# alshai/Big-BWT

Hardware: NVIDIA B200
Metric: pfp_parse_throughput (higher is better)
Workload: dtype u8/u32/u64 integer

## Files before the change

big-bwt_b200/csrc/pfp_api.cu:

```cuda
#include "pfp_common.cuh"
#include "pfp_stages.cuh"
#include <errno.h>
#include <fcntl.h>
#include <stdlib.h>
#include <sys/stat.h>
#include <time.h>
#include <unistd.h>

extern "C" {
int pfp_io_read_file(const char *path, int gz_ok, uint8_t **buf, uint64_t *n, char *err, size_t errlen);
int pfp_io_write_outputs(const char *path, const pfpb200_opts *opts, const pfpb200_outputs *o,
                         char *err, size_t errlen);
}

static double wall_sec() {
    struct timespec ts;
    clock_gettime(CLOCK_MONOTONIC, &ts);
    return (double)ts.tv_sec + 1e-9 * (double)ts.tv_nsec;
}

__global__ void set_u64_k(u64 *p, u64 v) { *p = v; }

__global__ void __launch_bounds__(256) first_invalid_k(const u8 *__restrict__ t, u64 n,
                                                       unsigned long long *__restrict__ first) {
    const u64 stride = (u64)gridDim.x * blockDim.x * 16;
    for (u64 i = ((u64)blockIdx.x * blockDim.x + threadIdx.x) * 16; i < n; i += stride) {
        bool hit = false;
        if (i + 16 <= n && (((uintptr_t)(t + i)) & 15) == 0) {
            uint4 v = __ldg(reinterpret_cast<const uint4 *>(t + i));
            u32 w[4] = {v.x, v.y, v.z, v.w};
#pragma unroll
            for (int k = 0; k < 4; k++) hit |= ((w[k] - 0x03030303u) & ~w[k] & 0x80808080u) != 0;
        } else hit = true;
        if (hit) {
            u64 e = i + 16 < n ? i + 16 : n;
            for (u64 j = i; j < e; j++)
                if (t[j] <= PFP_DOLLAR) { atomicMin(first, (unsigned long long)j); break; }
        }
    }
}

int pfp_first_invalid(pfpb200_ctx *ctx, const u8 *d_text, u64 n, u64 *d_first) {
    if (n == 0) return PFPB200_OK;
    first_invalid_k<<<ctx->sm_count * 8, 256, 0, ctx->stream>>>(d_text, n,
                                                               reinterpret_cast<unsigned long long *>(d_first));
    PFP_LAUNCHED(ctx);
    return PFPB200_OK;
}

extern "C" int pfpb200_abi_version(void) { return PFPB200_ABI_VERSION; }

extern "C" const char *pfpb200_strerror(int code) {
    switch (code) {
        case PFPB200_OK: return "ok";
        case PFPB200_E_ARG: return "invalid argument";
        case PFPB200_E_IO: return "file I/O error";
        case PFPB200_E_CUDA: return "CUDA error (no usable GPU or kernel failure)";
        case PFPB200_E_NOMEM: return "out of memory";
        case PFPB200_E_LIMIT: return "algorithm limit exceeded";
        case PFPB200_E_COLLISION: return "fingerprint collision";
        case PFPB200_E_INTERNAL: return "internal error";
        default: return "unknown error";
    }
}

extern "C" uint32_t pfpb200_launch_count(const pfpb200_ctx *ctx) { return ctx ? ctx->launches : 0; }

extern "C" const char *pfpb200_last_error(const pfpb200_ctx *ctx) { return ctx ? ctx->err : ""; }

static u64 splitmix64(u64 &s) {
    u64 z = (s += 0x9E3779B97F4A7C15ULL);
    z = (z ^ (z >> 30)) * 0xBF58476D1CE4E5B9ULL;
    z = (z ^ (z >> 27)) * 0x94D049BB133111EBULL;
    return z ^ (z >> 31);
}

extern "C" int pfpb200_create(int device, pfpb200_ctx **out) {
    if (!out) return PFPB200_E_ARG;
    *out = nullptr;
    int ndev = 0;
    if (cudaGetDeviceCount(&ndev) != cudaSuccess || device < 0 || device >= ndev) {
        cudaGetLastError();
        return PFPB200_E_CUDA;
    }
    pfpb200_ctx *ctx = new (std::nothrow) pfpb200_ctx();
    if (!ctx) return PFPB200_E_NOMEM;
    ctx->device = device;
    { const char *ev = getenv("PFPB200_LEGACY_K2"); ctx->legacy_k2 = ev && atoi(ev) != 0; }
    { const char *ev = getenv("PFPB200_K1"); ctx->k1_mode = (ev && strcmp(ev, "rolling") == 0) ? 1 : (ev && strcmp(ev, "table") == 0) ? 2 : 0; }
    { const char *ev = getenv("PFPB200_TEST_WEAK_FP"); ctx->weak_fp = (ev && atoi(ev) != 0) ? 1u : 0u; }
    { const char *ev = getenv("PFPB200_NO_SCAN_ALPHA"); ctx->no_scan_alpha = ev && atoi(ev) != 0; }
    { const char *ev = getenv("PFPB200_RANK_FULL_SORT"); ctx->rank_full_sort = ev && atoi(ev) != 0; }
    { const char *ev = getenv("PFPB200_RANK_CHUNK_PASSES"); ctx->rank_chunk_passes = ev && atoi(ev) != 0; }
    { const char *ev = getenv("PFPB200_RANK_WARP_PASSES"); ctx->rank_warp_passes = ev && atoi(ev) != 0; }
    { const char *ev = getenv("PFPB200_POOL_BY_WORD"); ctx->pool_by_word = ev && atoi(ev) != 0; }
    { const char *ev = getenv("PFPB200_FUSE_K3"); ctx->fuse_k3 = ev && atoi(ev) != 0; }
    { const char *ev = getenv("PFPB200_TABLE_SCALE"); if (ev && atof(ev) >= 1.2) ctx->table_scale = atof(ev); }
    { const char *ev = getenv("PFPB200_K1_MIX"); ctx->k1_mix = ev ? atoi(ev) : 0; }
    { const char *ev = getenv("PFPB200_K2_WINDOW"); ctx->k2_window = ev ? atoi(ev) : 0; }
    auto bail = [&](int code) { pfpb200_destroy(ctx); return code; };
    if (cudaSetDevice(device) != cudaSuccess) return bail(PFPB200_E_CUDA);
    cudaDeviceProp prop;
    if (cudaGetDeviceProperties(&prop, device) != cudaSuccess) return bail(PFPB200_E_CUDA);
    ctx->sm_count = prop.multiProcessorCount;
    if (cudaStreamCreateWithFlags(&ctx->own_stream, cudaStreamNonBlocking) != cudaSuccess)
        return bail(PFPB200_E_CUDA);
    ctx->stream = ctx->own_stream;
    if (cudaMalloc(&ctx->d_flags, PFP_FLAG_SLOTS * sizeof(u64)) != cudaSuccess ||
        cudaMallocHost(&ctx->h_flags, PFP_FLAG_SLOTS * sizeof(u64)) != cudaSuccess ||
        cudaMalloc(&ctx->d_keys, NH_KEY_WORDS * sizeof(u32)) != cudaSuccess ||
        cudaMalloc(&ctx->d_alpha, 8 * sizeof(u32)) != cudaSuccess)
        return bail(PFPB200_E_NOMEM);
    u32 hk[NH_KEY_WORDS];
    u64 seed = 0x5bd1e9955bd1e995ULL;
    for (u32 i = 0; i < NH_KEY_WORDS; i++) hk[i] = (u32)(splitmix64(seed) >> 32);
    if (cudaMemcpy(ctx->d_keys, hk, sizeof(hk), cudaMemcpyHostToDevice) != cudaSuccess ||
        cudaMemset(ctx->d_flags, 0, PFP_FLAG_SLOTS * sizeof(u64)) != cudaSuccess)
        return bail(PFPB200_E_CUDA);
    set_u64_k<<<1, 1, 0, ctx->stream>>>(&ctx->d_flags[15], 1);
    if (cudaGetLastError() != cudaSuccess || cudaStreamSynchronize(ctx->stream) != cudaSuccess)
        return bail(PFPB200_E_CUDA);
    if (cudaStreamCreateWithFlags(&ctx->aux_stream, cudaStreamNonBlocking) != cudaSuccess ||
        cudaEventCreateWithFlags(&ctx->ev_aux0, cudaEventDisableTiming) != cudaSuccess ||
        cudaEventCreateWithFlags(&ctx->ev_aux1, cudaEventDisableTiming) != cudaSuccess)
        return bail(PFPB200_E_CUDA);
    if (pfp_scan_init(ctx) || pfp_stream_init(ctx) || pfp_phrase_init(ctx) || pfp_prims_init(ctx) ||
        pfp_rank_init(ctx))
        return bail(PFPB200_E_CUDA);
    *out = ctx;
    return PFPB200_OK;
}

extern "C" void pfpb200_destroy(pfpb200_ctx *ctx) {
    if (!ctx) return;
    cudaSetDevice(ctx->device);
    if (ctx->stream) cudaStreamSynchronize(ctx->stream);
    pfp_release_scratch(ctx);
    pfp_release_held(ctx);
    pfp_arena_destroy(ctx);
    if (ctx->own_stream) { cudaStreamSynchronize(ctx->own_stream); cudaStreamDestroy(ctx->own_stream); }
    if (ctx->d_flags) cudaFree(ctx->d_flags);
    if (ctx->h_flags) cudaFreeHost(ctx->h_flags);
    if (ctx->d_keys) cudaFree(ctx->d_keys);
    if (ctx->dna_table) cudaFree(ctx->dna_table);
    if (ctx->iv_etab) cudaFree(ctx->iv_etab);
    if (ctx->iv_xtab) cudaFree(ctx->iv_xtab);
    if (ctx->d_alpha) cudaFree(ctx->d_alpha);
    pfp_io_destroy(ctx);
    for (int i = 0; i < 5; i++)
        if (ctx->pin_buf[i]) cudaFreeHost(ctx->pin_buf[i]);
    if (ctx->copy_stream) { cudaStreamSynchronize(ctx->copy_stream); cudaStreamDestroy(ctx->copy_stream); }
    if (ctx->aux_stream) { cudaStreamSynchronize(ctx->aux_stream); cudaStreamDestroy(ctx->aux_stream); }
    if (ctx->ev_aux0) cudaEventDestroy(ctx->ev_aux0);
    if (ctx->ev_aux1) cudaEventDestroy(ctx->ev_aux1);
    if (ctx->ev_k2) cudaEventDestroy(ctx->ev_k2);
    if (ctx->ev_copy) cudaEventDestroy(ctx->ev_copy);
    delete ctx;
}

extern "C" int pfpb200_set_stream(pfpb200_ctx *ctx, void *cuda_stream) {
    if (!ctx) return PFPB200_E_ARG;
    cudaStreamSynchronize(ctx->stream);
    pfp_release_scratch(ctx);
    pfp_release_held(ctx);
    ctx->stream = cuda_stream ? (cudaStream_t)cuda_stream : ctx->own_stream;
    return PFPB200_OK;
}

static int check_opts(pfpb200_ctx *ctx, const pfpb200_opts *o) {
    if (!ctx) return PFPB200_E_ARG;
    if (!o) return pfp_fail(ctx, PFPB200_E_ARG, "null options");
    if (o->w < 4) return pfp_fail(ctx, PFPB200_E_ARG, "Windows size must be at least 4");
    if (o->p < 10) return pfp_fail(ctx, PFPB200_E_ARG, "Modulus must be at least 10");
    if (o->w > 65536) return pfp_fail(ctx, PFPB200_E_ARG, "window size too large");
    if (o->nseg < 0) return pfp_fail(ctx, PFPB200_E_ARG, "Number of threads cannot be negative");
    return PFPB200_OK;
}

static int begin_call(pfpb200_ctx *ctx) {
    PFP_CUDA(ctx, cudaSetDevice(ctx->device));
    pfp_release_scratch(ctx);
    pfp_release_held(ctx);
    PFP_TRY(pfp_arena_consolidate(ctx));
    ctx->launches = 0;
    ctx->err[0] = 0;
    PFP_CUDA(ctx, cudaMemsetAsync(ctx->d_flags, 0, PFP_FLAG_SLOTS * sizeof(u64), ctx->stream));
    return PFPB200_OK;
}

struct StageTimer {
    cudaEvent_t ev[10] = {nullptr};
    int n = 0;
    int init() {
        for (int i = 0; i < 10; i++)
            if (cudaEventCreate(&ev[i]) != cudaSuccess) { ev[i] = nullptr; return -1; }
        return 0;
    }
    void mark(cudaStream_t s) { cudaEventRecord(ev[n++], s); }
    float ms(int a, int b) { float t = 0; cudaEventElapsedTime(&t, ev[a], ev[b]); return t; }
    ~StageTimer() {
        for (int i = 0; i < 10; i++)
            if (ev[i]) cudaEventDestroy(ev[i]);
    }
};

static int pfp_pin(pfpb200_ctx *ctx, int slot, void **h, size_t bytes) {
    if (bytes > ctx->pin_cap[slot]) {
        if (ctx->pin_buf[slot]) cudaFreeHost(ctx->pin_buf[slot]);
        ctx->pin_buf[slot] = nullptr;
        ctx->pin_cap[slot] = 0;
        size_t cap = bytes + bytes / 8 + 4096;
        if (cudaMallocHost(&ctx->pin_buf[slot], cap) != cudaSuccess) {
            cudaGetLastError();
            return pfp_fail(ctx, PFPB200_E_NOMEM, "pinned host allocation of %zu bytes failed", cap);
        }
        ctx->pin_cap[slot] = cap;
    }
    *h = ctx->pin_buf[slot];
    return PFPB200_OK;
}

static int parse_device_impl(pfpb200_ctx *ctx, const u8 *d_text, u64 n, const pfpb200_opts *o,
                             pfpb200_outputs *out, pfpb200_stats *st) {
    const u32 w = o->w, p = o->p;
    StageTimer tm;
    if (tm.init()) return pfp_fail(ctx, PFPB200_E_CUDA, "cudaEventCreate failed");
    int rc = PFPB200_OK;
    auto run = [&]() -> int {
        tm.mark(ctx->stream);
        ScanBits sb;
        float ms_scan = 0, ms_emit = 0;
        PFP_TRY(pfp_scan_bits(ctx, d_text, n, 0, 0, n, w, p, false, &sb, &ms_scan));
        const u64 k = sb.total;
        const u64 P = k + 1;
        if (P >= 0xFFFFFFFFull)
            return pfp_fail(ctx, PFPB200_E_LIMIT, "the parse contains %llu words, more than 2^32-2",
                            (unsigned long long)P);
        u64 *ends = nullptr;
        PFP_TRY(pfp_alloc_t(ctx, &ends, P));
        set_u64_k<<<1, 1, 0, ctx->stream>>>(ends + k, n + w - 1);
        PFP_LAUNCHED(ctx);
        tm.mark(ctx->stream);
        PhraseArrays ph{};
        ph.ends = ends;
        PFP_TRY(pfp_alloc_t(ctx, &ph.last, P, true));
        if (o->flags & PFPB200_F_SAI) PFP_TRY(pfp_alloc_t(ctx, &ph.sai, P * PFP_IBYTES, true));
        TextView tv{d_text, n, 0, (i64)n};
        DictArrays D;
        const bool stream = pfp_stream_ok(sb, w) && !ctx->legacy_k2;
        const bool fused = stream && ctx->fuse_k3;
        if (fused) {
            PFP_TRY(pfp_words_fused_stage(ctx, sb, tv, ph, P, -1, w, true, &D));
        } else {
            PFP_TRY(pfp_alloc_t(ctx, &ph.rec, P));
            if (stream) PFP_TRY(pfp_stream_stage(ctx, sb, tv, ph, P, -1, w, true));
            else {
                PFP_TRY(pfp_scan_emit(ctx, sb, ends));
                PFP_TRY(pfp_hash_stage(ctx, tv, ph, P, -1, w));
            }
        }
        PFP_TRY(pfp_scan_bits_free(ctx, &sb));
        tm.mark(ctx->stream);
        if (ctx->early_copy) {
            void *h_last = nullptr, *h_sai = nullptr;
            PFP_TRY(pfp_pin(ctx, 3, &h_last, P));
            if (ph.sai) PFP_TRY(pfp_pin(ctx, 4, &h_sai, P * PFP_IBYTES));
            if (!ctx->copy_stream) {
                PFP_CUDA(ctx, cudaStreamCreateWithFlags(&ctx->copy_stream, cudaStreamNonBlocking));
                PFP_CUDA(ctx, cudaEventCreateWithFlags(&ctx->ev_k2, cudaEventDisableTiming));
                PFP_CUDA(ctx, cudaEventCreateWithFlags(&ctx->ev_copy, cudaEventDisableTiming));
            }
            PFP_CUDA(ctx, cudaEventRecord(ctx->ev_k2, ctx->stream));
            PFP_CUDA(ctx, cudaStreamWaitEvent(ctx->copy_stream, ctx->ev_k2, 0));
            PFP_CUDA(ctx, cudaMemcpyAsync(h_last, ph.last, P, cudaMemcpyDeviceToHost, ctx->copy_stream));
            if (ph.sai)
                PFP_CUDA(ctx, cudaMemcpyAsync(h_sai, ph.sai, P * PFP_IBYTES, cudaMemcpyDeviceToHost, ctx->copy_stream));
            PFP_CUDA(ctx, cudaEventRecord(ctx->ev_copy, ctx->copy_stream));
            ctx->early_done = true;
        }
        if (!fused) {
            PFP_TRY(pfp_dedup_stage(ctx, ph, P, -1, w, &D));
            PFP_TRY(pfp_free_now(ctx, ph.rec));
            PFP_TRY(pfp_pool_stage(ctx, tv, ends, -1, w, &D));
        }
        if (o->flags & PFPB200_F_VERIFY) {
            PFP_TRY(pfp_uid_words(ctx, &D, P));
            PFP_TRY(pfp_verify_stage(ctx, tv, ends, -1, w, P, D));
        }
        tm.mark(ctx->stream);
        u32 *order = nullptr, rounds = 0;
        PFP_TRY(pfp_rank_stage(ctx, D, &order, &rounds, ctx->alpha_valid && !ctx->no_scan_alpha));
        tm.mark(ctx->stream);
        u8 *dict = nullptr;
        u32 *occ = nullptr, *rank_of_uid = nullptr;
        u64 dict_bytes = 0;
        u32 *parse = nullptr;
        PFP_TRY(pfp_alloc_t(ctx, &parse, P, true));
        PFP_TRY(pfp_dict_stage(ctx, D, order, (o->flags & PFPB200_F_COMPRESS) ? w : 0, &dict,
                               &dict_bytes, &occ, &rank_of_uid, D.uid, P, parse));
        tm.mark(ctx->stream);
        tm.mark(ctx->stream);
        PFP_CUDA(ctx, cudaMemcpyAsync(ctx->h_flags, ctx->d_flags, sizeof(u64), cudaMemcpyDeviceToHost, ctx->stream));
        PFP_CUDA(ctx, cudaStreamSynchronize(ctx->stream));
        PFP_CUDA(ctx, cudaGetLastError());
        if (ctx->h_flags[0] & PFP_ERRBIT_COLLISION)
            return pfp_fail(ctx, PFPB200_E_COLLISION, "two different phrases share a fingerprint (found by the verify pass)");
        out->dict = dict; out->dict_bytes = dict_bytes;
        out->occ = occ; out->n_distinct = D.d;
        out->parse = parse; out->n_phrases = P;
        out->last = ph.last;
        out->sai = ph.sai;
        if (st) {
            st->n_text = n; st->n_phrases = P; st->n_distinct = D.d;
            st->sum_word_len = D.sum_len; st->dict_bytes = dict_bytes;
            st->alg_bytes = n + 4 * P + P + ((o->flags & PFPB200_F_SAI) ? 5 * P : 0) + dict_bytes + 4 * D.d;
            st->rank_rounds = rounds;
            st->launches = ctx->launches;
            st->ms_total = tm.ms(0, 6);
            st->ms_scan = ms_scan; st->ms_emit = ms_emit;
            st->ms_hash = tm.ms(1, 2); st->ms_dedup = tm.ms(2, 3); st->ms_rank = tm.ms(3, 4);
            st->ms_dict = tm.ms(4, 5); st->ms_remap = tm.ms(5, 6);
        }
        return PFPB200_OK;
    };
    rc = run();
    if (rc != PFPB200_OK) cudaStreamSynchronize(ctx->stream);
    pfp_release_scratch(ctx);
    return rc;
}

extern "C" int pfpb200_parse_device(pfpb200_ctx *ctx, const uint8_t *d_text, uint64_t n_text,
                                    const pfpb200_opts *opts, pfpb200_outputs *dev_out,
                                    pfpb200_stats *stats) {
    PFP_TRY(check_opts(ctx, opts));
    if (!dev_out || (n_text && !d_text)) return pfp_fail(ctx, PFPB200_E_ARG, "null buffer");
    if (stats) memset(stats, 0, sizeof(*stats));
    memset(dev_out, 0, sizeof(*dev_out));
    PFP_TRY(begin_call(ctx));
    return parse_device_impl(ctx, d_text, n_text, opts, dev_out, stats);
}

extern "C" int pfpb200_memcpy_d2h(pfpb200_ctx *ctx, void *dst_host, const void *src_device,
                                  uint64_t bytes) {
    if (!ctx || (bytes && (!dst_host || !src_device))) return PFPB200_E_ARG;
    if (bytes == 0) return PFPB200_OK;
    PFP_CUDA(ctx, cudaSetDevice(ctx->device));
    PFP_CUDA(ctx, cudaMemcpyAsync(dst_host, src_device, bytes, cudaMemcpyDeviceToHost, ctx->stream));
    PFP_CUDA(ctx, cudaStreamSynchronize(ctx->stream));
    return PFPB200_OK;
}

extern "C" int pfpb200_parse_host(pfpb200_ctx *ctx, const uint8_t *text, uint64_t n_text,
                                  const pfpb200_opts *opts, pfpb200_outputs *host_out,
                                  pfpb200_stats *stats) {
    PFP_TRY(check_opts(ctx, opts));
    if (!host_out || (n_text && !text)) return pfp_fail(ctx, PFPB200_E_ARG, "null buffer");
    if (stats) memset(stats, 0, sizeof(*stats));
    memset(host_out, 0, sizeof(*host_out));
    PFP_TRY(begin_call(ctx));
    PfpEvents evs(4);
    if (!evs.ok) return pfp_fail(ctx, PFPB200_E_CUDA, "cudaEventCreate failed");
    const cudaEvent_t e0 = evs[0], e1 = evs[1], e2 = evs[2], e3 = evs[3];
    u8 *d_text = nullptr;
    PFP_TRY(pfp_alloc(ctx, (void **)&d_text, n_text, true));
    cudaEventRecord(e0, ctx->stream);
    if (n_text) PFP_CUDA(ctx, cudaMemcpyAsync(d_text, text, n_text, cudaMemcpyHostToDevice, ctx->stream));
    u64 n = n_text;
    if (n_text) {
        set_u64_k<<<1, 1, 0, ctx->stream>>>(&ctx->d_flags[14], n_text);
        PFP_LAUNCHED(ctx);
        first_invalid_k<<<ctx->sm_count * 8, 256, 0, ctx->stream>>>(
            d_text, n_text, reinterpret_cast<unsigned long long *>(&ctx->d_flags[14]));
        PFP_LAUNCHED(ctx);
        PFP_CUDA(ctx, cudaMemcpyAsync(&ctx->h_flags[14], &ctx->d_flags[14], sizeof(u64),
                                      cudaMemcpyDeviceToHost, ctx->stream));
    }
    cudaEventRecord(e1, ctx->stream);
    if (n_text) {
        PFP_CUDA(ctx, cudaStreamSynchronize(ctx->stream));
        n = ctx->h_flags[14];
    }
    if (n < n_text && (opts->flags & PFPB200_F_VERBOSE))
        fprintf(stderr, "Invalid char found in input file: no additional chars will be read\n");
    pfpb200_outputs dv;
    memset(&dv, 0, sizeof(dv));
    ctx->early_copy = true;
    ctx->early_done = false;
    int rc = parse_device_impl(ctx, d_text, n, opts, &dv, stats);
    ctx->early_copy = false;
    if (rc != PFPB200_OK) {
        if (ctx->early_done) cudaEventSynchronize(ctx->ev_copy);
        return rc;
    }
    const u64 P = dv.n_phrases, d = dv.n_distinct;
    void *h_dict = nullptr, *h_occ = nullptr, *h_parse = nullptr, *h_last = nullptr, *h_sai = nullptr;
    PFP_TRY(pfp_pin(ctx, 0, &h_dict, dv.dict_bytes));
    PFP_TRY(pfp_pin(ctx, 1, &h_occ, d * 4));
    PFP_TRY(pfp_pin(ctx, 2, &h_parse, P * 4));
    PFP_TRY(pfp_pin(ctx, 3, &h_last, P));
    if (dv.sai) PFP_TRY(pfp_pin(ctx, 4, &h_sai, P * PFP_IBYTES));
    cudaEventRecord(e2, ctx->stream);
    PFP_CUDA(ctx, cudaMemcpyAsync(h_dict, dv.dict, dv.dict_bytes, cudaMemcpyDeviceToHost, ctx->stream));
    PFP_CUDA(ctx, cudaMemcpyAsync(h_occ, dv.occ, d * 4, cudaMemcpyDeviceToHost, ctx->stream));
    PFP_CUDA(ctx, cudaMemcpyAsync(h_parse, dv.parse, P * 4, cudaMemcpyDeviceToHost, ctx->stream));
    if (ctx->early_done) {
        PFP_CUDA(ctx, cudaStreamWaitEvent(ctx->stream, ctx->ev_copy, 0));
    } else {
        PFP_CUDA(ctx, cudaMemcpyAsync(h_last, dv.last, P, cudaMemcpyDeviceToHost, ctx->stream));
        if (dv.sai)
            PFP_CUDA(ctx, cudaMemcpyAsync(h_sai, dv.sai, P * PFP_IBYTES, cudaMemcpyDeviceToHost, ctx->stream));
    }
    cudaEventRecord(e3, ctx->stream);
    PFP_CUDA(ctx, cudaStreamSynchronize(ctx->stream));
    if (stats) {
        cudaEventElapsedTime(&stats->ms_h2d, e0, e1);
        cudaEventElapsedTime(&stats->ms_d2h, e2, e3);
    }
    host_out->dict = (const u8 *)h_dict; host_out->dict_bytes = dv.dict_bytes;
    host_out->occ = (const u32 *)h_occ; host_out->n_distinct = d;
    host_out->parse = (const u32 *)h_parse; host_out->n_phrases = P;
    host_out->last = (const u8 *)h_last;
    host_out->sai = (const u8 *)h_sai;
    pfp_release_held(ctx);
    return PFPB200_OK;
}

static int write_outputs_from_device(pfpb200_ctx *ctx, const char *path, const pfpb200_opts *o,
                                     const pfpb200_outputs &dv) {
    char name[4096];
    auto put = [&](const char *ext, int seg, const void *p, u64 bytes) -> int {
        if (seg < 0) snprintf(name, sizeof(name), "%s.%s", path, ext);
        else snprintf(name, sizeof(name), "%s.%d.%s", path, seg, ext);
        return pfp_device_to_file(ctx, name, p, bytes);
    };
    const u64 P = dv.n_phrases;
    PFP_TRY(put((o->flags & PFPB200_F_COMPRESS) ? "dicz" : "dict", -1, dv.dict, dv.dict_bytes));
    PFP_TRY(put("occ", -1, dv.occ, 4 * dv.n_distinct));
    PFP_TRY(put("parse", -1, dv.parse, 4 * P));
    const int T = o->nseg;
    if (T <= 0) {
        PFP_TRY(put("last", -1, dv.last, P));
        if (dv.sai) PFP_TRY(put("sai", -1, dv.sai, PFP_IBYTES * P));
    } else {
        const u64 per = (P + (u64)T - 1) / (u64)T;
        for (int s = 0; s < T; s++) {
            u64 a = (u64)s * per, b = a + per;
            if (a > P) a = P;
            if (b > P) b = P;
            PFP_TRY(put("last", s, dv.last + a, b - a));
            if (dv.sai) PFP_TRY(put("sai", s, dv.sai + PFP_IBYTES * a, PFP_IBYTES * (b - a)));
        }
    }
    return PFPB200_OK;
}

static int cut_and_parse_device(pfpb200_ctx *ctx, const u8 *d_text, u64 n_text, const pfpb200_opts *opts,
                                pfpb200_outputs *dv, pfpb200_stats *stats) {
    u64 n = n_text;
    if (n_text) {
        set_u64_k<<<1, 1, 0, ctx->stream>>>(&ctx->d_flags[14], n_text);
        PFP_LAUNCHED(ctx);
        PFP_TRY(pfp_first_invalid(ctx, d_text, n_text, &ctx->d_flags[14]));
        PFP_CUDA(ctx, cudaMemcpyAsync(&ctx->h_flags[14], &ctx->d_flags[14], sizeof(u64), cudaMemcpyDeviceToHost,
                                      ctx->stream));
        PFP_CUDA(ctx, cudaStreamSynchronize(ctx->stream));
        n = ctx->h_flags[14];
    }
    if (n < n_text) fprintf(stderr, "Invalid char found in input file: no additional chars will be read\n");
    return parse_device_impl(ctx, d_text, n, opts, dv, stats);
}

static int parse_file_impl(pfpb200_ctx *ctx, const char *path, const pfpb200_opts *opts, pfpb200_stats *stats,
                           bool write_files, pfpb200_outputs *dv_out);

extern "C" int pfpb200_parse_file(pfpb200_ctx *ctx, const char *path, const pfpb200_opts *opts,
                                  pfpb200_stats *stats) {
    const int rc = parse_file_impl(ctx, path, opts, stats, true, nullptr);
    if (ctx && rc == PFPB200_OK) pfp_release_held(ctx);
    return rc;
}

extern "C" int pfpb200_bigbwt_file(pfpb200_ctx *ctx, const char *path, const pfpb200_opts *opts, uint32_t pfbwt_flags,
                                   int keep_files, pfpb200_stats *stats, pfpb200_bwtparse_result *bp_out,
                                   pfpb200_pfbwt_result *res) {
    if (!ctx || !opts || !res) return PFPB200_E_ARG;
    if (opts->flags & PFPB200_F_COMPRESS) return pfp_fail(ctx, PFPB200_E_ARG, "bigbwt: -c stops after the parse, use pfpb200_parse_file");
    pfpb200_opts o = *opts;
    o.flags |= PFPB200_F_SAI;
    o.nseg = 0;
    pfpb200_stats st;
    pfpb200_outputs dv;
    PFP_TRY(parse_file_impl(ctx, path, &o, &st, keep_files != 0, &dv));
    if (stats) *stats = st;
    const double t0 = wall_sec();
    pfpb200_bwtparse_result bp;
    PFP_TRY(pfpb200_bwtparse_device(ctx, dv.parse, dv.n_phrases, dv.last, dv.sai, &bp));
    if (bp_out) *bp_out = bp;
    PFP_TRY(pfpb200_pfbwt_device(ctx, dv.dict, dv.dict_bytes, dv.occ, dv.n_distinct, bp.ilist, bp.bwlast, bp.bwsai,
                                 bp.n_out, o.w, pfbwt_flags, res));
    char name[4096];
    auto put = [&](const char *ext, const void *p, u64 bytes) -> int {
        snprintf(name, sizeof(name), "%s.%s", path, ext);
        return pfp_device_to_file(ctx, name, p, bytes);
    };
    if (keep_files) {
        PFP_TRY(put("ilist", bp.ilist, bp.n_out * 4));
        PFP_TRY(put("bwlast", bp.bwlast, bp.n_out));
        PFP_TRY(put("bwsai", bp.bwsai, bp.n_out * PFP_IBYTES));
    }
    PFP_TRY(put("bwt", res->bwt, res->n_bwt));
    if (pfbwt_flags & PFPB200_PFBWT_SA) PFP_TRY(put("sa", res->sa, res->n_sa * PFP_IBYTES));
    if (pfbwt_flags & PFPB200_PFBWT_SSA) PFP_TRY(put("ssa", res->ssa, res->n_ssa * 2 * PFP_IBYTES));
    if (pfbwt_flags & PFPB200_PFBWT_ESA) PFP_TRY(put("esa", res->esa, res->n_esa * 2 * PFP_IBYTES));
    if (stats) stats->sec_write += (float)(wall_sec() - t0);
    pfp_release_scratch(ctx);
    return PFPB200_OK;
}

static int parse_file_impl(pfpb200_ctx *ctx, const char *path, const pfpb200_opts *opts, pfpb200_stats *stats,
                           bool write_files, pfpb200_outputs *dv_out) {
    PFP_TRY(check_opts(ctx, opts));
    if (!path) return pfp_fail(ctx, PFPB200_E_ARG, "null path");
    if (stats) memset(stats, 0, sizeof(*stats));
    const double t0 = wall_sec();
    const bool fasta = (opts->flags & PFPB200_F_FASTA) != 0;
    int fd = open(path, O_RDONLY);
    if (fd < 0) return pfp_fail(ctx, PFPB200_E_IO, "%s: %s", path, strerror(errno));
    struct stat sb;
    if (fstat(fd, &sb) != 0) { close(fd); return pfp_fail(ctx, PFPB200_E_IO, "%s: %s", path, strerror(errno)); }
    const u64 fsize = (u64)sb.st_size;
    bool gz = false;
    if (fasta && fsize >= 2) {
        unsigned char mg[2] = {0, 0};
        if (pread(fd, mg, 2, 0) == 2) gz = mg[0] == 0x1f && mg[1] == 0x8b;
    }
    PFP_TRY(begin_call(ctx));
    pfpb200_outputs dv;
    memset(&dv, 0, sizeof(dv));
    double t1 = t0;
    int rc = PFPB200_OK;
    auto run = [&]() -> int {
        u8 *d_text = nullptr;
        u64 n_text = 0;
        bool on_device = false;
        if (!gz) {
            u8 *d_file = nullptr;
            PFP_TRY(pfp_alloc(ctx, (void **)&d_file, fsize + 16));
            PFP_TRY(pfp_file_to_device(ctx, fd, 0, fsize, d_file));
            if (!fasta) { d_text = d_file; n_text = fsize; on_device = true; }
            else {
                int supported = 0;
                PFP_TRY(pfp_fasta_device(ctx, d_file, fsize, &d_text, &n_text, &supported, false));
                on_device = supported != 0;
                PFP_CUDA(ctx, cudaStreamSynchronize(ctx->stream));
                PFP_TRY(pfp_free_now(ctx, d_file));
            }
        }
        if (!on_device) {
            uint8_t *text = nullptr;
            uint64_t n = 0;
            int trunc = 0;
            if (pfpb200_read_input(path, opts->flags, &text, &n, &trunc) != PFPB200_OK)
                return pfp_fail(ctx, PFPB200_E_IO, "%s: cannot read", path);
            if (trunc) fprintf(stderr, "Invalid char found in input file: no additional chars will be read\n");
            int r2 = pfp_alloc(ctx, (void **)&d_text, n + 16);
            if (r2 == PFPB200_OK && n && cudaMemcpyAsync(d_text, text, n, cudaMemcpyHostToDevice, ctx->stream) != cudaSuccess)
                r2 = pfp_fail(ctx, PFPB200_E_CUDA, "host-to-device copy of the input failed");
            if (r2 == PFPB200_OK && cudaStreamSynchronize(ctx->stream) != cudaSuccess)
                r2 = pfp_fail(ctx, PFPB200_E_CUDA, "host-to-device copy of the input failed");
            pfpb200_free_host(text);
            PFP_TRY(r2);
            n_text = n;
        }
        PFP_CUDA(ctx, cudaStreamSynchronize(ctx->stream));
        t1 = wall_sec();
        PFP_TRY(cut_and_parse_device(ctx, d_text, n_text, opts, &dv, stats));
        return PFPB200_OK;
    };
    rc = run();
    close(fd);
    if (rc != PFPB200_OK) { pfp_release_scratch(ctx); return rc; }
    const double t2 = wall_sec();
    if (write_files) PFP_TRY(write_outputs_from_device(ctx, path, opts, dv));
    if (stats) {
        stats->sec_read = (float)(t1 - t0);
        stats->sec_write = (float)(wall_sec() - t2);
    }
    pfp_release_scratch(ctx);
    if (dv_out) *dv_out = dv;
    return PFPB200_OK;
}

extern "C" int pfpb200_fasta_extract_device(pfpb200_ctx *ctx, const uint8_t *d_file, uint64_t n,
                                            const uint8_t **d_text, uint64_t *n_text, int *supported) {
    if (!ctx || !d_text || !n_text || !supported || (n && !d_file)) return PFPB200_E_ARG;
    PFP_TRY(begin_call(ctx));
    u8 *out = nullptr;
    int rc = pfp_fasta_device(ctx, d_file, n, &out, n_text, supported, true);
    cudaStreamSynchronize(ctx->stream);
    pfp_release_scratch(ctx);
    *d_text = out;
    return rc;
}

extern "C" int pfpb200_scan_triggers(pfpb200_ctx *ctx, const uint8_t *d_buf, uint64_t n_buf,
                                     uint64_t buf_pos0, uint64_t own_lo, uint64_t own_hi, uint32_t w,
                                     uint32_t p, const uint64_t **d_triggers, uint64_t *n_triggers,
                                     float *ms) {
    pfpb200_opts o = {w, p, 0, 0};
    PFP_TRY(check_opts(ctx, &o));
    if (!d_triggers || !n_triggers) return pfp_fail(ctx, PFPB200_E_ARG, "null output");
    PFP_TRY(begin_call(ctx));
    u64 *out = nullptr, k = 0;
    float a = 0, b = 0;
    int rc = pfp_scan_stage(ctx, d_buf, n_buf, buf_pos0, own_lo, own_hi, w, p, 0, true, &out, &k, &a, &b);
    cudaStreamSynchronize(ctx->stream);
    pfp_release_scratch(ctx);
    if (rc != PFPB200_OK) return rc;
    *d_triggers = out;
    *n_triggers = k;
    if (ms) *ms = a;
    return PFPB200_OK;
}

struct CallTimer {
    PfpEvents ev;
    cudaStream_t s;
    explicit CallTimer(cudaStream_t st) : ev(2), s(st) { if (ev.ok) cudaEventRecord(ev[0], s); }
    float stop() {
        float t = 0;
        if (!ev.ok) { cudaStreamSynchronize(s); return t; }
        cudaEventRecord(ev[1], s);
        cudaEventSynchronize(ev[1]);
        cudaEventElapsedTime(&t, ev[0], ev[1]);
        return t;
    }
};

static void promote_scratch(pfpb200_ctx *ctx) {
    for (void *p : ctx->scratch) ctx->held.push_back(p);
    ctx->scratch.clear();
}

extern "C" int pfpb200_shard_scan(pfpb200_ctx *ctx, const pfpb200_shard *shard, const pfpb200_opts *opts,
                                  uint64_t *n_triggers, uint64_t *first_trigger, uint64_t *last_trigger,
                                  float *ms) {
    PFP_TRY(check_opts(ctx, opts));
    if (!shard || !n_triggers || !first_trigger || !last_trigger) return pfp_fail(ctx, PFPB200_E_ARG, "null argument");
    if (shard->own_lo > shard->own_hi || shard->own_hi > shard->n_global)
        return pfp_fail(ctx, PFPB200_E_ARG, "bad shard range");
    PFP_TRY(begin_call(ctx));
    ctx->sh.desc = *shard;
    ctx->sh.opts = *opts;
    ctx->sh.route_perm = nullptr;
    ctx->sh.route_ooff = nullptr;
    CallTimer tm(ctx->stream);
    u64 *ends = nullptr, k = 0;
    float a = 0;
    ScanBits sb;
    int rc = pfp_scan_bits(ctx, shard->d_buf, shard->n_buf, shard->buf_pos0, shard->own_lo, shard->own_hi,
                           opts->w, opts->p, true, &sb, &a);
    if (rc == PFPB200_OK) {
        k = sb.total;
        rc = pfp_alloc_t(ctx, &ends, k + 1, true);
    }
    const bool stream_k2 = rc == PFPB200_OK && pfp_stream_ok(sb, opts->w) && !ctx->legacy_k2;
    ctx->sh.ends_emitted = !stream_k2;
    if (rc == PFPB200_OK && !stream_k2) rc = pfp_scan_emit(ctx, sb, ends);
    ctx->sh.bits = sb;
    if (rc == PFPB200_OK && k > 0) {
        if (stream_k2) {
            rc = pfp_scan_first_last(ctx, sb, &ctx->d_flags[8]);
            cudaMemcpyAsync(&ctx->h_flags[8], &ctx->d_flags[8], 2 * sizeof(u64), cudaMemcpyDeviceToHost, ctx->stream);
        } else {
            cudaMemcpyAsync(&ctx->h_flags[8], ends, sizeof(u64), cudaMemcpyDeviceToHost, ctx->stream);
            cudaMemcpyAsync(&ctx->h_flags[9], ends + (k - 1), sizeof(u64), cudaMemcpyDeviceToHost, ctx->stream);
        }
    }
    float t = tm.stop();
    pfp_release_scratch(ctx);
    if (rc != PFPB200_OK) return rc;
    PFP_CUDA(ctx, cudaGetLastError());
    ctx->sh.ends = ends;
    ctx->sh.n_trig = k;
    *n_triggers = k;
    *first_trigger = k ? ctx->h_flags[8] : 0;
    *last_trigger = k ? ctx->h_flags[9] : 0;
    if (ms) *ms = t;
    return PFPB200_OK;
}

extern "C" int pfpb200_shard_words(pfpb200_ctx *ctx, int64_t first_start, pfpb200_words *out, float *ms) {
    if (!ctx || !out) return PFPB200_E_ARG;
    memset(out, 0, sizeof(*out));
    PFP_CUDA(ctx, cudaSetDevice(ctx->device));
    const pfpb200_shard &sh = ctx->sh.desc;
    const pfpb200_opts &o = ctx->sh.opts;
    const u32 w = o.w;
    const u64 k = ctx->sh.n_trig;
    const u64 P = k + (sh.is_last ? 1 : 0);
    ctx->sh.P = P;
    ctx->sh.d = 0;
    ctx->sh.uid = nullptr;
    if (ms) *ms = 0;
    if (P == 0) return PFPB200_OK;
    if (P >= 0xFFFFFFFFull) return pfp_fail(ctx, PFPB200_E_LIMIT, "the shard's parse has more than 2^32-2 words");
    CallTimer tm(ctx->stream);
    auto run = [&]() -> int {
        u64 *ends = ctx->sh.ends;
        if (sh.is_last) {
            set_u64_k<<<1, 1, 0, ctx->stream>>>(ends + k, sh.n_global + w - 1);
            PFP_LAUNCHED(ctx);
        }
        PhraseArrays ph{};
        ph.ends = ends;
        PFP_TRY(pfp_alloc_t(ctx, &ph.rec, P));
        PFP_TRY(pfp_alloc_t(ctx, &ph.last, P, true));
        if (o.flags & PFPB200_F_SAI) PFP_TRY(pfp_alloc_t(ctx, &ph.sai, P * PFP_IBYTES, true));
        TextView tv{sh.d_buf, sh.n_buf, (i64)sh.buf_pos0, (i64)sh.n_global};
        DictArrays D;
        const bool stream = pfp_stream_ok(ctx->sh.bits, w) && !ctx->legacy_k2;
        const bool fused = stream && ctx->fuse_k3;
        if (fused) {
            PFP_TRY(pfp_words_fused_stage(ctx, ctx->sh.bits, tv, ph, P, first_start, w, !ctx->sh.ends_emitted, &D));
        } else {
            if (stream) PFP_TRY(pfp_stream_stage(ctx, ctx->sh.bits, tv, ph, P, first_start, w, !ctx->sh.ends_emitted));
            else PFP_TRY(pfp_hash_stage(ctx, tv, ph, P, first_start, w));
            PFP_TRY(pfp_dedup_stage(ctx, ph, P, first_start, w, &D));
            PFP_TRY(pfp_uid_words(ctx, &D, P));
        }
        u64 *wfpa = nullptr, *wfpb = nullptr;
        PFP_TRY(pfp_alloc_t(ctx, &wfpa, D.d));
        PFP_TRY(pfp_alloc_t(ctx, &wfpb, D.d));
        PFP_TRY(pfp_gather_word_fp(ctx, D, ph, wfpa, wfpb));
        PFP_TRY(pfp_free_now(ctx, ph.rec));
        if (!fused) PFP_TRY(pfp_pool_stage(ctx, tv, ends, first_start, w, &D));
        PFP_TRY(pfp_free_now(ctx, D.rep));
        if (o.flags & PFPB200_F_VERIFY) PFP_TRY(pfp_verify_stage(ctx, tv, ends, first_start, w, P, D));
        PFP_CUDA(ctx, cudaMemcpyAsync(ctx->h_flags, ctx->d_flags, sizeof(u64), cudaMemcpyDeviceToHost, ctx->stream));
        PFP_CUDA(ctx, cudaStreamSynchronize(ctx->stream));
        PFP_CUDA(ctx, cudaGetLastError());
        if (ctx->h_flags[0] & PFP_ERRBIT_COLLISION)
            return pfp_fail(ctx, PFPB200_E_COLLISION, "two different phrases share a fingerprint (found by the verify pass)");
        ctx->sh.d = D.d;
        ctx->sh.uid = D.uid;
        ctx->sh.wfpa = wfpa; ctx->sh.wfpb = wfpb; ctx->sh.pool = D.pool; ctx->sh.uoff = D.uoff;
        ctx->sh.pool_words = D.pool_words;
        ctx->sh.ulen = D.ulen; ctx->sh.count = D.count; ctx->sh.uwords = D.uwords;
        out->n_words = D.d; out->n_phrases = P; out->pool_words = D.pool_words;
        out->fpa = wfpa; out->fpb = wfpb; out->len = D.ulen; out->count = D.count;
        out->uwords = D.uwords; out->pool = D.pool; out->last = ph.last; out->sai = ph.sai;
        return PFPB200_OK;
    };
    int rc = run();
    float t = tm.stop();
    if (rc != PFPB200_OK) { pfp_release_scratch(ctx); return rc; }
    promote_scratch(ctx);
    if (ms) *ms = t;
    return PFPB200_OK;
}

extern "C" int pfpb200_dict_merge(pfpb200_ctx *ctx, uint64_t n_in, const uint64_t *fpa, const uint64_t *fpb,
                                  const uint32_t *len, const uint32_t *count, const uint32_t *uwords,
                                  const uint64_t *pool, uint64_t pool_words, uint32_t w, uint32_t flags,
                                  pfpb200_merged *out, float *ms) {
    if (!ctx || !out) return PFPB200_E_ARG;
    memset(out, 0, sizeof(*out));
    PFP_CUDA(ctx, cudaSetDevice(ctx->device));
    PFP_CUDA(ctx, cudaMemsetAsync(ctx->d_flags, 0, PFP_FLAG_SLOTS * sizeof(u64), ctx->stream));
    CallTimer tm(ctx->stream);
    auto run = [&]() -> int {
        if (n_in == 0) {
            u8 *dict = nullptr;
            PFP_TRY(pfp_alloc_t(ctx, &dict, 1, true));
            PFP_CUDA(ctx, cudaMemsetAsync(dict, 0, 1, ctx->stream));
            out->dict = dict; out->dict_bytes = 1;
            return PFPB200_OK;
        }
        DictArrays D;
        u32 *uid_of_entry = nullptr;
        StageTimer tm;
        const bool trace = getenv("PFPB200_TRACE") != nullptr && tm.init() == 0;
        if (trace) tm.mark(ctx->stream);
        PFP_TRY(pfp_merge_stage(ctx, n_in, fpa, fpb, len, count, uwords, pool, pool_words,
                                (flags & PFPB200_F_VERIFY) != 0, &D, &uid_of_entry));
        if (trace) tm.mark(ctx->stream);
        u32 *order = nullptr, rounds = 0;
        PFP_TRY(pfp_rank_stage(ctx, D, &order, &rounds));
        if (trace) tm.mark(ctx->stream);
        u8 *dict = nullptr;
        u32 *occ = nullptr, *rank_of_uid = nullptr, *rank_of_entry = nullptr;
        u64 dict_bytes = 0;
        PFP_TRY(pfp_dict_stage(ctx, D, order, (flags & PFPB200_F_COMPRESS) ? w : 0, &dict, &dict_bytes, &occ,
                               &rank_of_uid));
        PFP_TRY(pfp_alloc_t(ctx, &rank_of_entry, n_in, true));
        PFP_TRY(pfp_remap_stage(ctx, uid_of_entry, rank_of_uid, n_in, rank_of_entry));
        if (trace) tm.mark(ctx->stream);
        PFP_CUDA(ctx, cudaStreamSynchronize(ctx->stream));
        PFP_CUDA(ctx, cudaGetLastError());
        if (trace) {
            fprintf(stderr, "[pfpb200 merge] n_in %llu -> d %llu: dedup %.3f ms, rank %.3f ms (%u rounds), dict+remap %.3f ms\n",
                    (unsigned long long)n_in, (unsigned long long)D.d, tm.ms(0, 1), tm.ms(1, 2), rounds, tm.ms(2, 3));
        }
        out->n_distinct = D.d; out->dict_bytes = dict_bytes; out->sum_word_len = D.sum_len;
        out->dict = dict; out->occ = occ; out->rank_of_entry = rank_of_entry;
        return PFPB200_OK;
    };
    int rc = run();
    float t = tm.stop();
    pfp_release_scratch(ctx);
    if (ms) *ms = t;
    return rc;
}

extern "C" int pfp_unpack_words(pfpb200_ctx *ctx, const pfpb200_word *in, u64 n, u64 *fpa, u64 *fpb,
                                u32 *len, u32 *count, u32 *uwords);

extern "C" int pfpb200_dict_merge_begin(pfpb200_ctx *ctx, uint64_t n_in, const pfpb200_word *words, float *ms) {
    if (!ctx || (n_in && !words)) return PFPB200_E_ARG;
    if (ms) *ms = 0;
    PFP_CUDA(ctx, cudaSetDevice(ctx->device));
    PFP_CUDA(ctx, cudaMemsetAsync(ctx->d_flags, 0, PFP_FLAG_SLOTS * sizeof(u64), ctx->stream));
    ctx->mg.n_in = n_in;
    ctx->mg.d = 0;
    if (n_in == 0) return PFPB200_OK;
    CallTimer tm(ctx->stream);
    auto run = [&]() -> int {
        u64 *fpa = nullptr, *fpb = nullptr;
        u32 *len = nullptr, *count = nullptr, *uwords = nullptr;
        PFP_TRY(pfp_alloc_t(ctx, &fpa, n_in));
        PFP_TRY(pfp_alloc_t(ctx, &fpb, n_in));
        PFP_TRY(pfp_alloc_t(ctx, &len, n_in));
        PFP_TRY(pfp_alloc_t(ctx, &count, n_in));
        PFP_TRY(pfp_alloc_t(ctx, &uwords, n_in));
        PFP_TRY(pfp_unpack_words(ctx, words, n_in, fpa, fpb, len, count, uwords));
        DictArrays D;
        u32 *uid_of_entry = nullptr;
        PFP_TRY(pfp_merge_stage(ctx, n_in, fpa, fpb, len, count, uwords, nullptr, 0, false, &D, &uid_of_entry));
        PFP_TRY(pfp_free_now(ctx, fpa));
        PFP_TRY(pfp_free_now(ctx, fpb));
        PFP_TRY(pfp_free_now(ctx, count));
        ctx->mg.d = D.d; ctx->mg.sum_len = D.sum_len; ctx->mg.max_len = D.max_len;
        ctx->mg.uid_of_entry = uid_of_entry; ctx->mg.rep = D.rep; ctx->mg.count = D.count;
        ctx->mg.ulen = D.ulen; ctx->mg.uwords = D.uwords; ctx->mg.uoff = D.uoff;
        ctx->mg.len_in = len; ctx->mg.uwords_in = uwords;
        return PFPB200_OK;
    };
    int rc = run();
    float t = tm.stop();
    if (rc != PFPB200_OK) { pfp_release_scratch(ctx); ctx->mg.n_in = 0; return rc; }
    promote_scratch(ctx);
    if (ms) *ms = t;
    return PFPB200_OK;
}

extern "C" int pfpb200_dict_merge_finish(pfpb200_ctx *ctx, const uint64_t *pool, uint64_t pool_words, uint32_t w,
                                         uint32_t flags, pfpb200_merged *out, float *ms) {
    if (!ctx || !out) return PFPB200_E_ARG;
    memset(out, 0, sizeof(*out));
    if (ms) *ms = 0;
    PFP_CUDA(ctx, cudaSetDevice(ctx->device));
    CallTimer tm(ctx->stream);
    const u64 n_in = ctx->mg.n_in;
    auto run = [&]() -> int {
        if (n_in == 0) {
            u8 *dict = nullptr;
            PFP_TRY(pfp_alloc_t(ctx, &dict, 1, true));
            PFP_CUDA(ctx, cudaMemsetAsync(dict, 0, 1, ctx->stream));
            out->dict = dict; out->dict_bytes = 1;
            return PFPB200_OK;
        }
        if (!pool) return pfp_fail(ctx, PFPB200_E_ARG, "dict_merge_finish: null pool");
        DictArrays D;
        D.d = ctx->mg.d; D.sum_len = ctx->mg.sum_len; D.max_len = ctx->mg.max_len;
        D.uid = ctx->mg.uid_of_entry; D.rep = ctx->mg.rep; D.count = ctx->mg.count; D.ulen = ctx->mg.ulen;
        D.uwords = ctx->mg.uwords; D.uoff = ctx->mg.uoff;
        D.pool = const_cast<u64 *>(pool); D.pool_words = pool_words;
        if (flags & PFPB200_F_VERIFY)
            PFP_TRY(pfp_merge_verify(ctx, n_in, ctx->mg.uid_of_entry, D.rep, ctx->mg.len_in, ctx->mg.uwords_in, pool));
        u32 *order = nullptr, rounds = 0;
        PFP_TRY(pfp_rank_stage(ctx, D, &order, &rounds));
        u8 *dict = nullptr;
        u32 *occ = nullptr, *rank_of_uid = nullptr, *rank_of_entry = nullptr;
        u64 dict_bytes = 0;
        PFP_TRY(pfp_alloc_t(ctx, &rank_of_entry, n_in, true));
        PFP_TRY(pfp_dict_stage(ctx, D, order, (flags & PFPB200_F_COMPRESS) ? w : 0, &dict, &dict_bytes, &occ,
                               &rank_of_uid, ctx->mg.uid_of_entry, n_in, rank_of_entry));
        PFP_CUDA(ctx, cudaStreamSynchronize(ctx->stream));
        PFP_CUDA(ctx, cudaGetLastError());
        out->n_distinct = D.d; out->dict_bytes = dict_bytes; out->sum_word_len = D.sum_len;
        out->dict = dict; out->occ = occ; out->rank_of_entry = rank_of_entry;
        return PFPB200_OK;
    };
    int rc = run();
    float t = tm.stop();
    pfp_release_scratch(ctx);
    ctx->mg.n_in = 0;
    if (ms) *ms = t;
    return rc;
}

extern "C" int pfpb200_dict_merge_words(pfpb200_ctx *ctx, uint64_t n_in, const pfpb200_word *words,
                                        const uint64_t *pool, uint64_t pool_words, uint32_t w,
                                        uint32_t flags, pfpb200_merged *out, float *ms) {
    if (!ctx || !out || (n_in && !words)) return PFPB200_E_ARG;
    float a = 0, b = 0;
    PFP_TRY(pfpb200_dict_merge_begin(ctx, n_in, words, &a));
    int rc = pfpb200_dict_merge_finish(ctx, pool, pool_words, w, flags, out, &b);
    if (ms) *ms = a + b;
    return rc;
}

extern "C" int pfpb200_shard_remap(pfpb200_ctx *ctx, const uint32_t *d_rank_of_word, const uint32_t **d_parse,
                                   float *ms) {
    if (!ctx || !d_parse) return PFPB200_E_ARG;
    *d_parse = nullptr;
    if (ms) *ms = 0;
    const u64 P = ctx->sh.P;
    if (P == 0) return PFPB200_OK;
    if (!d_rank_of_word || !ctx->sh.uid) return pfp_fail(ctx, PFPB200_E_ARG, "shard_remap before shard_words");
    PFP_CUDA(ctx, cudaSetDevice(ctx->device));
    CallTimer tm(ctx->stream);
    u32 *parse = nullptr;
    PFP_TRY(pfp_alloc_t(ctx, &parse, P, true));
    PFP_TRY(pfp_remap_stage(ctx, ctx->sh.uid, d_rank_of_word, P, parse));
    float t = tm.stop();
    PFP_CUDA(ctx, cudaGetLastError());
    *d_parse = parse;
    if (ms) *ms = t;
    return PFPB200_OK;
}

struct Splitters { u64 s[PFPB200_MAX_RANKS]; u32 n; };

extern "C" int pfp_route_impl(pfpb200_ctx *ctx, const Splitters &sp, u32 n_ranks, pfpb200_routed *out);
extern "C" int pfp_first_keys_impl(pfpb200_ctx *ctx, u64 **keys);

extern "C" int pfpb200_shard_first_keys(pfpb200_ctx *ctx, const uint64_t **d_keys) {
    if (!ctx || !d_keys) return PFPB200_E_ARG;
    *d_keys = nullptr;
    if (ctx->sh.d == 0) return PFPB200_OK;
    PFP_CUDA(ctx, cudaSetDevice(ctx->device));
    u64 *keys = nullptr;
    int rc = pfp_first_keys_impl(ctx, &keys);
    if (rc != PFPB200_OK) return rc;
    PFP_CUDA(ctx, cudaStreamSynchronize(ctx->stream));
    *d_keys = keys;
    return PFPB200_OK;
}

extern "C" int pfpb200_shard_route(pfpb200_ctx *ctx, const uint64_t *splitters, uint32_t n_ranks,
                                   pfpb200_routed *out, float *ms) {
    if (!ctx || !out || n_ranks < 1 || n_ranks > PFPB200_MAX_RANKS || (n_ranks > 1 && !splitters))
        return PFPB200_E_ARG;
    memset(out, 0, sizeof(*out));
    if (ms) *ms = 0;
    if (ctx->sh.d == 0) return PFPB200_OK;
    PFP_CUDA(ctx, cudaSetDevice(ctx->device));
    Splitters sp;
    sp.n = n_ranks - 1;
    for (u32 i = 0; i < sp.n; i++) {
        sp.s[i] = splitters[i];
        if (i && sp.s[i] < sp.s[i - 1]) return pfp_fail(ctx, PFPB200_E_ARG, "splitters not ascending");
    }
    CallTimer tm(ctx->stream);
    int rc = pfp_route_impl(ctx, sp, n_ranks, out);
    float t = tm.stop();
    if (rc != PFPB200_OK) { pfp_release_scratch(ctx); return rc; }
    promote_scratch(ctx);
    if (ms) *ms = t;
    return PFPB200_OK;
}

extern "C" int pfp_route_plan_impl(pfpb200_ctx *ctx, const Splitters &sp, u32 n_ranks, u64 *words_to, u64 *pool_to,
                                   const u32 **perm_out);
extern "C" int pfp_route_push_impl(pfpb200_ctx *ctx, u32 n_ranks, const u64 *word_dst, const u64 *pool_dst);

extern "C" int pfpb200_shard_route_plan(pfpb200_ctx *ctx, const uint64_t *splitters, uint32_t n_ranks,
                                        uint64_t *words_to, uint64_t *pool_to, const uint32_t **d_perm,
                                        float *ms) {
    if (!ctx || !words_to || !pool_to || !d_perm || n_ranks < 1 || n_ranks > PFPB200_MAX_RANKS ||
        (n_ranks > 1 && !splitters))
        return PFPB200_E_ARG;
    for (u32 q = 0; q < PFPB200_MAX_RANKS; q++) words_to[q] = pool_to[q] = 0;
    *d_perm = nullptr;
    if (ms) *ms = 0;
    if (ctx->sh.d == 0) return PFPB200_OK;
    PFP_CUDA(ctx, cudaSetDevice(ctx->device));
    Splitters sp;
    sp.n = n_ranks - 1;
    for (u32 i = 0; i < sp.n; i++) {
        sp.s[i] = splitters[i];
        if (i && sp.s[i] < sp.s[i - 1]) return pfp_fail(ctx, PFPB200_E_ARG, "splitters not ascending");
    }
    CallTimer tm(ctx->stream);
    int rc = pfp_route_plan_impl(ctx, sp, n_ranks, words_to, pool_to, d_perm);
    float t = tm.stop();
    if (rc != PFPB200_OK) { pfp_release_scratch(ctx); return rc; }
    promote_scratch(ctx);
    if (ms) *ms = t;
    return PFPB200_OK;
}

extern "C" int pfpb200_shard_route_push(pfpb200_ctx *ctx, uint32_t n_ranks, const uint64_t *word_dst,
                                        const uint64_t *pool_dst, float *ms) {
    if (!ctx || !word_dst || !pool_dst || n_ranks < 1 || n_ranks > PFPB200_MAX_RANKS) return PFPB200_E_ARG;
    if (ms) *ms = 0;
    if (ctx->sh.d == 0) return PFPB200_OK;
    if (!ctx->sh.route_perm) return pfp_fail(ctx, PFPB200_E_ARG, "shard_route_push before shard_route_plan");
    PFP_CUDA(ctx, cudaSetDevice(ctx->device));
    CallTimer tm(ctx->stream);
    int rc = pfp_route_push_impl(ctx, n_ranks, word_dst, pool_dst);
    float t = tm.stop();
    if (ms) *ms = t;
    return rc;
}
```

big-bwt_b200/csrc/pfp_common.cuh:

```cuda
#pragma once
#include <cuda_runtime.h>
#include <stdint.h>
#include <stdio.h>
#include <string.h>
#include <vector>
#include "pfp_arith.h"
#include "../../include/pfpb200.h"

typedef uint64_t u64;
typedef uint32_t u32;
typedef uint16_t u16;
typedef uint8_t u8;
typedef int64_t i64;

struct PfpBlock { char *p; size_t n; };
struct PfpArena {
    std::vector<PfpBlock> slabs;
    std::vector<PfpBlock> free_list;
    std::vector<PfpBlock> used;
    size_t in_use = 0, peak = 0, total = 0;
};

constexpr int PFP_TILE_T = 256;
constexpr int PFP_TILE_RUN = 128;
constexpr int PFP_TILE = PFP_TILE_T * PFP_TILE_RUN;
struct ScanBits {
    const uint4 *A;
    u64 q_end;
    u64 pos_bias;
    u32 ntiles;
    uint4 *mask;
    u32 *tile_cnt;
    u64 *tile_off;
    u64 total;
    u32 max_tile_cnt;
};

constexpr int PFP_IO_THREADS = 4;
constexpr size_t PFP_IO_CHUNK = (size_t)8 << 20;
struct PfpIo {
    bool ready = false;
    void *slot[PFP_IO_THREADS][2] = {{nullptr}};
    cudaEvent_t ev[PFP_IO_THREADS][2] = {{nullptr}};
    cudaStream_t stream[PFP_IO_THREADS] = {nullptr};
};

struct pfpb200_ctx {
    int device = 0;
    PfpIo io;
    PfpArena arena;
    int sm_count = 148;
    cudaStream_t own_stream = nullptr;
    cudaStream_t stream = nullptr;
    u32 launches = 0;
    int k1_mode = 0;
    u32 *d_alpha = nullptr;
    bool alpha_valid = false;
    u32 *dna_table = nullptr;
    u32 dna_w = 0, dna_p = 0;
    void *iv_etab = nullptr;
    void *iv_xtab = nullptr;
    u32 iv_w = 0, iv_p = 0, iv_cthr = 0;
    int iv_skip = 0;
    bool no_scan_alpha = false;
    bool rank_full_sort = false;
    bool rank_chunk_passes = false;
    bool rank_warp_passes = false;
    bool pool_by_word = false;
    bool fuse_k3 = false;
    double pool_ratio = 0.0;
    bool legacy_k2 = false;
    double table_scale = 2.0;
    u32 weak_fp = 0;
    int k1_mix = 0;
    int k2_window = 0;
    double dedup_ratio = 0.0;
    char err[512] = {0};
    std::vector<void *> scratch;
    std::vector<void *> held;
    void *bp_out[3] = {nullptr, nullptr, nullptr};
    void *up_out = nullptr;
    void *pb_out[4] = {nullptr, nullptr, nullptr, nullptr};
    void *pin_buf[5] = {nullptr, nullptr, nullptr, nullptr, nullptr};
    size_t pin_cap[5] = {0, 0, 0, 0, 0};
    cudaStream_t aux_stream = nullptr;
    cudaEvent_t ev_aux0 = nullptr, ev_aux1 = nullptr;
    cudaStream_t copy_stream = nullptr;
    cudaEvent_t ev_k2 = nullptr, ev_copy = nullptr;
    bool early_copy = false;
    bool early_done = false;
    u32 *d_keys = nullptr;
    u64 *d_flags = nullptr;
    u64 *h_flags = nullptr;
    struct {
        u64 n_in = 0, d = 0, sum_len = 0;
        u32 max_len = 0;
        u32 *uid_of_entry = nullptr, *rep = nullptr, *count = nullptr, *ulen = nullptr, *uwords = nullptr;
        u64 *uoff = nullptr;
        const u32 *len_in = nullptr, *uwords_in = nullptr;
    } mg;
    struct {
        pfpb200_shard desc;
        pfpb200_opts opts;
        u64 *ends = nullptr;
        bool ends_emitted = true;
        ScanBits bits;
        u64 n_trig = 0, P = 0, d = 0;
        u32 *uid = nullptr;
        u64 *wfpa = nullptr, *wfpb = nullptr, *pool = nullptr, *uoff = nullptr, pool_words = 0;
        u32 *ulen = nullptr, *count = nullptr, *uwords = nullptr;
        u32 *route_perm = nullptr;
        u64 *route_ooff = nullptr;
        u64 route_words_to[PFPB200_MAX_RANKS] = {0}, route_pool_to[PFPB200_MAX_RANKS] = {0};
    } sh;
};

#define PFP_FLAG_SLOTS 16
#define PFP_ERRBIT_COLLISION 1ull
#define PFP_ERRBIT_LIMIT 2ull
#define PFP_ERRBIT_INTERNAL 4ull
#define PFP_ERRBIT_TABLE_FULL 8ull
#define PFP_ERRBIT_POOL_FULL 16ull

int pfp_fail(pfpb200_ctx *ctx, int code, const char *fmt, ...);

#define PFP_CUDA(ctx, call)                                                                 \
    do {                                                                                    \
        cudaError_t e_ = (call);                                                            \
        if (e_ != cudaSuccess)                                                              \
            return pfp_fail((ctx), e_ == cudaErrorMemoryAllocation ? PFPB200_E_NOMEM        \
                                                                   : PFPB200_E_CUDA,        \
                            "%s:%d %s: %s", __FILE__, __LINE__, #call, cudaGetErrorString(e_)); \
    } while (0)

#define PFP_TRY(expr)                 \
    do {                              \
        int rc_ = (expr);             \
        if (rc_ != PFPB200_OK) return rc_; \
    } while (0)

#define PFP_LAUNCHED(ctx)                                                                   \
    do {                                                                                    \
        (ctx)->launches++;                                                                  \
        cudaError_t e_ = cudaGetLastError();                                                \
        if (e_ != cudaSuccess)                                                              \
            return pfp_fail((ctx), PFPB200_E_CUDA, "%s:%d launch: %s", __FILE__, __LINE__,  \
                            cudaGetErrorString(e_));                                        \
    } while (0)

int pfp_alloc(pfpb200_ctx *ctx, void **p, size_t bytes, bool held = false);
int pfp_free_now(pfpb200_ctx *ctx, void *p);
void pfp_release_scratch(pfpb200_ctx *ctx);
void pfp_release_held(pfpb200_ctx *ctx);
void pfp_arena_destroy(pfpb200_ctx *ctx);
int pfp_arena_consolidate(pfpb200_ctx *ctx);
void pfp_arena_reserve(pfpb200_ctx *ctx, size_t bytes);

template <typename T>
static inline int pfp_alloc_t(pfpb200_ctx *ctx, T **p, size_t count, bool held = false) {
    return pfp_alloc(ctx, (void **)p, (count ? count : 1) * sizeof(T), held);
}

int pfp_scan_init(pfpb200_ctx *ctx);
int pfp_stream_init(pfpb200_ctx *ctx);
int pfp_phrase_init(pfpb200_ctx *ctx);
int pfp_prims_init(pfpb200_ctx *ctx);
int pfp_rank_init(pfpb200_ctx *ctx);

struct PfpEvents {
    cudaEvent_t ev[4] = {nullptr, nullptr, nullptr, nullptr};
    bool ok = true;
    explicit PfpEvents(int n) {
        for (int i = 0; i < n && i < 4; i++)
            if (cudaEventCreate(&ev[i]) != cudaSuccess) { ev[i] = nullptr; ok = false; }
    }
    ~PfpEvents() {
        for (int i = 0; i < 4; i++)
            if (ev[i]) cudaEventDestroy(ev[i]);
    }
    PfpEvents(const PfpEvents &) = delete;
    PfpEvents &operator=(const PfpEvents &) = delete;
    cudaEvent_t operator[](int i) const { return ev[i]; }
};

static inline u32 pfp_blocks(u64 n, u32 per_block) { return (u32)((n + per_block - 1) / per_block); }

int pfp_exclusive_scan_u32(pfpb200_ctx *ctx, const u32 *in, u32 *out, u64 n, u32 *d_total);
int pfp_exclusive_scan_u32_u64(pfpb200_ctx *ctx, const u32 *in, u64 *out, u64 n, u64 *d_total);
int pfp_exclusive_scan_u8_u32(pfpb200_ctx *ctx, const u8 *in, u32 *out, u64 n, u32 *d_total);

int pfp_radix_sort_pairs(pfpb200_ctx *ctx, u64 *k0, u32 *v0, u64 *k1, u32 *v1, u64 n,
                         int begin_bit, int end_bit, u64 **res_k, u32 **res_v);

__device__ __forceinline__ u32 lane_id() { return threadIdx.x & 31; }
__device__ __forceinline__ u32 lanemask_lt() {
    u32 m;
    asm("mov.u32 %0, %%lanemask_lt;" : "=r"(m));
    return m;
}
__device__ __forceinline__ u32 warp_incl_scan(u32 v) {
#pragma unroll
    for (int o = 1; o < 32; o <<= 1) {
        u32 t = __shfl_up_sync(0xffffffffu, v, o);
        if (lane_id() >= (u32)o) v += t;
    }
    return v;
}
__device__ __forceinline__ u32 block_excl_scan_256(u32 v, u32 *total, u32 *sm ) {
    u32 inc = warp_incl_scan(v);
    u32 w = threadIdx.x >> 5;
    __syncthreads();
    if (lane_id() == 31) sm[w] = inc;
    __syncthreads();
    if (threadIdx.x < 32) {
        u32 x = threadIdx.x < 8 ? sm[threadIdx.x] : 0;
        u32 xi = warp_incl_scan(x);
        if (threadIdx.x < 8) sm[threadIdx.x] = xi - x;
        if (threadIdx.x == 7) sm[8] = xi;
    }
    __syncthreads();
    *total = sm[8];
    return inc - v + sm[w];
}
```

big-bwt_b200/csrc/pfp_phrase.cu:

```cuda
#include "pfp_common.cuh"
#include "pfp_stages.cuh"
#include "pfp_fp.cuh"
#include "pfp_table.cuh"
#include <stdlib.h>

__device__ __forceinline__ void load_chunk(const TextView &tv, i64 s0, u64 len, u64 o, bool special,
                                           u32 x[4]) {
    const u32 nbv = (u32)((len - o) < 16 ? (len - o) : 16);
    if (!special) {
        const i64 loc = s0 + (i64)o - tv.pos0;
        const u8 *p = tv.T + loc;
        const u32 bs = (u32)((uintptr_t)p & 3);
        const u32 *p4 = reinterpret_cast<const u32 *>(p - bs);
        u32 W[5];
        if ((u64)loc + 20 <= tv.n_buf) {
#pragma unroll
            for (int j = 0; j < 5; j++) W[j] = __ldg(p4 + j);
        } else {
            const u32 need = bs + nbv;
#pragma unroll
            for (int j = 0; j < 5; j++) W[j] = (4u * j < need) ? __ldg(p4 + j) : 0u;
        }
#pragma unroll
        for (int j = 0; j < 4; j++) x[j] = __funnelshift_r(W[j], W[j + 1], 8 * bs);
    } else {
#pragma unroll
        for (int j = 0; j < 4; j++) {
            u32 v = 0;
            for (int b = 0; b < 4; b++) {
                u32 k = 4 * j + b;
                if (k < nbv) v |= (u32)tv_byte(tv, s0 + (i64)o + k) << (8 * b);
            }
            x[j] = v;
        }
    }
    if (nbv < 16) {
#pragma unroll
        for (int j = 0; j < 4; j++) {
            u32 lo = 4u * j;
            u32 nb = nbv > lo ? nbv - lo : 0;
            if (nb < 4) x[j] &= (nb == 0) ? 0u : ((1u << (8 * nb)) - 1u);
        }
    }
}

struct ChunkRaw { u32 W[5]; u32 bs; };

__device__ __forceinline__ void chunk_fetch(const u8 *p, ChunkRaw &r) {
    r.bs = (u32)((uintptr_t)p & 3);
    const u32 *p4 = reinterpret_cast<const u32 *>(p - r.bs);
#pragma unroll
    for (int j = 0; j < 5; j++) r.W[j] = __ldg(p4 + j);
}

__device__ __forceinline__ void chunk_finish(const ChunkRaw &r, u32 rem, u32 x[4]) {
#pragma unroll
    for (int j = 0; j < 4; j++) {
        u32 v = __funnelshift_r(r.W[j], r.W[j + 1], 8 * r.bs);
        int nb = (int)rem - 4 * j;
        nb = nb < 0 ? 0 : (nb > 4 ? 4 : nb);
        x[j] = v & __funnelshift_rc(0xFFFFFFFFu, 0u, 8u * (4u - (u32)nb));
    }
}

__device__ __forceinline__ void nh_chunk(const u32 *__restrict__ sk, u32 c, const u32 x[4], u64 &pa,
                                         u64 &pb) {
    const uint4 k0 = *reinterpret_cast<const uint4 *>(sk + 4 * c);
    const uint4 k1 = *reinterpret_cast<const uint4 *>(sk + 4 * c + 4);
    pa += (u64)(x[0] + k0.x) * (u64)(x[1] + k0.y) + (u64)(x[2] + k0.z) * (u64)(x[3] + k0.w);
    pb += (u64)(x[0] + k1.x) * (u64)(x[1] + k1.y) + (u64)(x[2] + k1.z) * (u64)(x[3] + k1.w);
}

__global__ void phrase_records_k(TextView tv, const u64 *__restrict__ ends, u64 j0, u64 P, u32 w,
                                 u8 *__restrict__ last, u8 *__restrict__ sai) {
    u64 j = j0 + (u64)blockIdx.x * blockDim.x + threadIdx.x;
    if (j >= P) return;
    i64 e = (i64)ends[j];
    last[j] = tv_byte(tv, e - (i64)w);
    if (sai) {
        u64 pos = (u64)(e + 1);
        u8 *d = sai + j * PFP_IBYTES;
#pragma unroll
        for (int b = 0; b < PFP_IBYTES; b++) d[b] = (u8)(pos >> (8 * b));
    }
}

constexpr int PH_T = 256;
constexpr int PH_WARPS = PH_T / 32;
constexpr int PH_PER_BLOCK = PH_T;
constexpr int PH_WIN = 6144;


__global__ void __launch_bounds__(PH_T) phrase_hash_k(TextView tv, PhraseArrays ph, u64 P,
                                                      i64 first_start, u32 w,
                                                      const u32 *__restrict__ keytab,
                                                      u32 *__restrict__ long_list,
                                                      u32 *__restrict__ long_count, u32 long_cap,
                                                      u64 *__restrict__ flags, int use_window) {
    __shared__ __align__(16) u32 sk[NH_KEY_WORDS];
    __shared__ const u8 *s_ptr[PH_WARPS][32];
    __shared__ u32 s_len[PH_WARPS][32];
    __shared__ u32 s_pre[PH_WARPS][33];
    __shared__ unsigned long long s_acc[PH_WARPS][32][2];
    extern __shared__ __align__(16) unsigned char ph_win[];
    for (int i = threadIdx.x; i < NH_KEY_WORDS; i += PH_T) sk[i] = keytab[i];
    __syncthreads();
    const u32 lane = threadIdx.x & 31, wp = threadIdx.x >> 5;
    unsigned char *win = ph_win + wp * PH_WIN;
    const u8 *gend = tv.T + tv.n_buf;
    for (u64 j0 = ((u64)blockIdx.x * PH_WARPS + wp) * 32; j0 < P; j0 += (u64)gridDim.x * PH_PER_BLOCK) {
        const u64 j = j0 + lane;
        const bool valid = j < P;
        i64 e = valid ? (i64)ph.ends[j] : 0;
        i64 prev = __shfl_up_sync(0xffffffffu, e, 1);
        if (lane == 0) prev = (j0 > 0) ? (i64)ph.ends[j0 - 1] : 0;
        const i64 s0 = (j == 0) ? first_start : prev - (i64)w + 1;
        const u64 len = valid ? (u64)(e - s0 + 1) : 0;
        const bool slow = valid && (len > NH_SEG_BYTES || s0 < tv.pos0 || e >= tv.n_global ||
                                    (u64)(e - tv.pos0) + 24 > tv.n_buf);
        if (slow) {
            if (len > 0xFFFFFFFFull) atomicOr((unsigned long long *)&flags[0], PFP_ERRBIT_LIMIT);
            else {
                const u32 li = atomicAdd(long_count, 1u);
                if (li < long_cap) long_list[li] = (u32)j;
                else atomicOr((unsigned long long *)&flags[0], PFP_ERRBIT_INTERNAL);
            }
        }
        const u32 mylen = slow ? 0u : (u32)len;
        const u32 nch = (mylen + 15) >> 4;
        const u32 incl = warp_incl_scan(nch);
        const u32 T = __shfl_sync(0xffffffffu, incl, 31);
        i64 wlo = mylen ? s0 - tv.pos0 : (i64)0x7fffffffffffffffLL;
        i64 whi = mylen ? e - tv.pos0 + 1 : -1;
#pragma unroll
        for (int o = 16; o > 0; o >>= 1) {
            wlo = min(wlo, __shfl_xor_sync(0xffffffffu, wlo, o));
            whi = max(whi, __shfl_xor_sync(0xffffffffu, whi, o));
        }
        const u8 *myptr = tv.T + (s0 - tv.pos0);
        if (use_window && whi > wlo) {
            const u8 *gbase = reinterpret_cast<const u8 *>(reinterpret_cast<uintptr_t>(tv.T + wlo) & ~(uintptr_t)15);
            const u64 wbytes = (u64)((tv.T + whi) - gbase) + 24;
            if (wbytes <= PH_WIN) {
                for (u32 o = lane * 16; o < wbytes; o += 512) {
                    uint4 v = make_uint4(0u, 0u, 0u, 0u);
                    if (gbase + o < gend) v = __ldg(reinterpret_cast<const uint4 *>(gbase + o));
                    *reinterpret_cast<uint4 *>(win + o) = v;
                }
                myptr = win + (myptr - gbase);
            }
        }
        s_ptr[wp][lane] = myptr;
        s_len[wp][lane] = mylen;
        s_pre[wp][lane] = incl - nch;
        if (lane == 31) s_pre[wp][32] = T;
        s_acc[wp][lane][0] = 0ull;
        s_acc[wp][lane][1] = 0ull;
        __syncwarp();
        const u32 K = (T + 31) >> 5;
        u32 g = lane * K;
        const u32 g1 = (g + K < T) ? g + K : T;
        u64 head_a = 0, head_b = 0, tail_a = 0, tail_b = 0;
        u32 head_q = 0xFFFFFFFFu;
        bool pass = false;
        if (g < g1) {
            u32 lo = 0, hi = 32;
#pragma unroll
            for (int it = 0; it < 5; it++) {
                u32 mid = (lo + hi) >> 1;
                if (s_pre[wp][mid] <= g) lo = mid; else hi = mid;
            }
            u32 q = lo;
            u32 c = g - s_pre[wp][q];
            bool cont = c != 0;
            const u8 *qp = s_ptr[wp][q];
            u32 qlen = s_len[wp][q];
            u32 qnch = (qlen + 15) >> 4;
            u64 pa = 0, pb = 0;
            ChunkRaw cur;
            chunk_fetch(qp + 16u * c, cur);
            for (; g < g1; g++) {
                u32 nq = q, nc = c + 1, nlen = qlen, nnch = qnch;
                const u8 *np = qp;
                const bool ends = nc == qnch;
                if (ends) {
                    nc = 0;
                    do { nq++; } while (nq < 31 && s_len[wp][nq] == 0);
                    np = s_ptr[wp][nq & 31];
                    nlen = s_len[wp][nq & 31];
                    nnch = (nlen + 15) >> 4;
                }
                ChunkRaw nxt;
                if (g + 1 < g1) chunk_fetch(np + 16u * nc, nxt);
                u32 x[4];
                chunk_finish(cur, qlen - 16u * c, x);
                nh_chunk(sk, c, x, pa, pb);
                if (ends) {
                    if (cont) { head_a = pa; head_b = pb; head_q = q; cont = false; }
                    else { s_acc[wp][q][0] = pa; s_acc[wp][q][1] = pb; }
                    pa = pb = 0;
                }
                q = nq; c = nc; qp = np; qlen = nlen; qnch = nnch;
                cur = nxt;
            }
            if (c != 0) { tail_a = pa; tail_b = pb; pass = cont; }
        }
#pragma unroll
        for (int o = 1; o < 32; o <<= 1) {
            u64 ta = __shfl_up_sync(0xffffffffu, tail_a, o);
            u64 tb = __shfl_up_sync(0xffffffffu, tail_b, o);
            int tp = __shfl_up_sync(0xffffffffu, (int)pass, o);
            if (lane >= (u32)o && pass) { tail_a += ta; tail_b += tb; pass = tp != 0; }
        }
        u64 ca = __shfl_up_sync(0xffffffffu, tail_a, 1);
        u64 cb = __shfl_up_sync(0xffffffffu, tail_b, 1);
        if (head_q != 0xFFFFFFFFu) {
            s_acc[wp][head_q][0] = head_a + (lane ? ca : 0ull);
            s_acc[wp][head_q][1] = head_b + (lane ? cb : 0ull);
        }
        __syncwarp();
        if (valid && !slow) store_rec(ph.rec, j, s_acc[wp][lane][0], s_acc[wp][lane][1]);
        __syncwarp();
    }
}

__global__ void __launch_bounds__(PH_T) phrase_hash_long_k(TextView tv, PhraseArrays ph,
                                                           i64 first_start, u32 w,
                                                           const u32 *__restrict__ keytab,
                                                           const u32 *__restrict__ long_list,
                                                           const u32 *__restrict__ long_count, u32 long_cap,
                                                           u64 *__restrict__ flags,
                                                           PhraseFp *__restrict__ rec_compact ) {
    __shared__ __align__(16) u32 sk[NH_KEY_WORDS];
    for (int i = threadIdx.x; i < NH_KEY_WORDS; i += PH_T) sk[i] = keytab[i];
    __syncthreads();
    const u32 lane = threadIdx.x & 31;
    const u32 nlong = min(*long_count, long_cap);
    for (u32 q = blockIdx.x * PH_WARPS + (threadIdx.x >> 5); q < nlong; q += gridDim.x * PH_WARPS) {
        const u64 j = long_list[q];
        const i64 e = (i64)ph.ends[j];
        const i64 s0 = (j == 0) ? first_start : (i64)ph.ends[j - 1] - (i64)w + 1;
        const u64 len = (u64)(e - s0 + 1);
        const bool special = (s0 < 0) || (e >= tv.n_global);
        const u64 nch = (len + 15) >> 4;
        u64 fa = 0, fb = 0, pa = 0, pb = 0, wa = 1, wb = 1;
        u64 seg = 0;
        for (u64 c = lane; c < nch; c += 32) {
            const u64 sg = c >> 9;
            if (sg != seg) {
                fa += wa * pa; fb += wb * pb;
                pa = pb = 0;
                for (; seg < sg; seg++) { wa *= NH_FOLD_A; wb *= NH_FOLD_B; }
            }
            u32 x[4];
            load_chunk(tv, s0, len, 16ull * c, special, x);
            nh_chunk(sk, (u32)(c & 511u), x, pa, pb);
        }
        fa += wa * pa; fb += wb * pb;
#pragma unroll
        for (int o = 16; o > 0; o >>= 1) {
            fa += __shfl_xor_sync(0xffffffffu, fa, o);
            fb += __shfl_xor_sync(0xffffffffu, fb, o);
        }
        if (lane == 0) {
            if (len > 0xFFFFFFFFull) atomicOr((unsigned long long *)&flags[0], PFP_ERRBIT_LIMIT);
            if (rec_compact) store_rec(rec_compact, q, fa, fb);
            else store_rec(ph.rec, j, fa, fb);
        }
    }
}

__global__ void table_init_k(DictSlot *__restrict__ tab, u64 cap) {
    u64 i = (u64)blockIdx.x * blockDim.x + threadIdx.x;
    if (i < cap) *reinterpret_cast<uint4 *>(tab + i) = make_uint4(0u, 0u, 0u, 0u);
}

int pfp_table_init(pfpb200_ctx *ctx, DictSlot *tab, u64 cap) {
    table_init_k<<<pfp_blocks(cap, 256), 256, 0, ctx->stream>>>(tab, cap);
    PFP_LAUNCHED(ctx);
    return PFPB200_OK;
}

constexpr int TI_T = 256;

__global__ void __launch_bounds__(TI_T, 8) table_insert_k(const PhraseFp *__restrict__ rec, u64 P,
                                                         DictSlot *__restrict__ tab, u64 cap,
                                                         const u32 *__restrict__ weight,
                                                         u32 weak ,
                                                         u32 *__restrict__ uid, u64 *__restrict__ flags) {
    const u32 lane = threadIdx.x & 31;
    for (u64 b0 = (u64)blockIdx.x * TI_T; b0 < P; b0 += (u64)gridDim.x * TI_T) {
        const u64 j = b0 + threadIdx.x;
        PhraseFp r;
        r.fpa = 0; r.fpb = 0;
        u64 k = 0;
        if (j < P) {
            const uint4 a = __ldcs(reinterpret_cast<const uint4 *>(rec + j));
            r.fpa = ((u64)a.y << 32) | a.x; r.fpb = ((u64)a.w << 32) | a.z;
            if (weak) { r.fpa &= 3ull; r.fpb = 0; }
            k = sort_key_of(r.fpa, r.fpb);
        }
        const u32 chk = j < P ? check_of(r) : 0u;
        const u32 peers = __match_any_sync(0xffffffffu, k);
        const int leader = __ffs(peers) - 1;
        const bool lead = j < P && (int)lane == leader;
        u32 res = 0;
        if (lead) {
            const u64 s0 = __umul64hi(k, cap);
            const Probe pr = table_probe(tab, cap, s0, __ldcg(reinterpret_cast<const uint4 *>(tab + s0)), k);
            if (pr.placed) {
                res = (u32)pr.slot | (pr.creator ? UID_CREATOR : 0u);
                u32 seen = pr.seen_chk;
                if (seen == 0u) seen = atomicCAS(&tab[pr.slot].chk, 0u, chk);
                if (seen != 0u && seen != chk) atomicOr((unsigned long long *)&flags[0], PFP_ERRBIT_COLLISION);
                if (!weight) atomicAdd(&tab[pr.slot].val, (u32)__popc(peers));
            } else {
                atomicOr((unsigned long long *)&flags[0], PFP_ERRBIT_TABLE_FULL);
            }
        }
        const u32 slot = __shfl_sync(0xffffffffu, res, leader) & ~UID_CREATOR;
        const u32 lchk = __shfl_sync(0xffffffffu, chk, leader);
        if (j < P) {
            if (chk != lchk) atomicOr((unsigned long long *)&flags[0], PFP_ERRBIT_COLLISION);
            __stcs(uid + j, lead ? res : slot);
            if (weight) {
                const u32 c = weight[j];
                const u32 old = atomicAdd(&tab[slot].val, c);
                if (old + c < old) atomicOr((unsigned long long *)&flags[0], PFP_ERRBIT_LIMIT);
            }
        }
    }
}

constexpr int TC_T = 256;
constexpr int TC_I = 4;
constexpr int TC_TILE = TC_T * TC_I;

__device__ __forceinline__ void load_uids(const u32 *__restrict__ uid, u64 n, u64 j, u32 v[TC_I]) {
    if (j + TC_I <= n) {
        const uint4 a = __ldcs(reinterpret_cast<const uint4 *>(uid + j));
        v[0] = a.x; v[1] = a.y; v[2] = a.z; v[3] = a.w;
    } else {
#pragma unroll
        for (int i = 0; i < TC_I; i++) v[i] = j + i < n ? uid[j + i] : 0u;
    }
}

__global__ void __launch_bounds__(TC_T) table_creators_k(const u32 *__restrict__ uid, u64 n,
                                                         u32 *__restrict__ tile_count) {
    __shared__ u32 sm[9];
    u32 v[TC_I];
    load_uids(uid, n, (u64)blockIdx.x * TC_TILE + (u64)threadIdx.x * TC_I, v);
    u32 c = 0;
#pragma unroll
    for (int i = 0; i < TC_I; i++) c += v[i] >> 31;
    u32 total;
    block_excl_scan_256(c, &total, sm);
    if (threadIdx.x == 0) tile_count[blockIdx.x] = total;
}

__global__ void __launch_bounds__(TC_T, 6) table_compact_k(u32 *__restrict__ uid, u64 n,
                                                        const u32 *__restrict__ tile_base,
                                                        const DictSlot *__restrict__ tab,
                                                        const u32 *__restrict__ len_in,
                                                        const u64 *__restrict__ ends, i64 first_start, u32 w,
                                                        u32 *__restrict__ slot_of_word,
                                                        u32 *__restrict__ rep, u32 *__restrict__ count,
                                                        u32 *__restrict__ ulen, u32 *__restrict__ uwords,
                                                        i64 *__restrict__ ustart ,
                                                        u64 *__restrict__ flags) {
    __shared__ u32 sm[9];
    __shared__ u32 s_max;
    __shared__ unsigned long long s_sum;
    if (threadIdx.x == 0) { s_max = 0; s_sum = 0; }
    const u64 j0 = (u64)blockIdx.x * TC_TILE + (u64)threadIdx.x * TC_I;
    u32 v[TC_I];
    load_uids(uid, n, j0, v);
    u32 c = 0;
#pragma unroll
    for (int i = 0; i < TC_I; i++) c += v[i] >> 31;
    u32 cnt[TC_I], len[TC_I];
    i64 st[TC_I];
#pragma unroll
    for (int i = 0; i < TC_I; i++) {
        const u64 j = j0 + i;
        const bool cr = (v[i] & UID_CREATOR) != 0;
        cnt[i] = cr ? tab[v[i] & ~UID_CREATOR].val : 0u;
        if (len_in) {
            len[i] = cr ? len_in[j] : 0u;
            st[i] = 0;
        } else {
            st[i] = cr ? (j ? (i64)ends[j - 1] - (i64)w + 1 : first_start) : 0;
            len[i] = cr ? (u32)((i64)ends[j] - st[i] + 1) : 0u;
        }
    }
    u32 total;
    u32 u = block_excl_scan_256(c, &total, sm) + tile_base[blockIdx.x];
    u32 mx = 0;
    u64 sum = 0;
#pragma unroll
    for (int i = 0; i < TC_I; i++) {
        if (!(v[i] & UID_CREATOR)) continue;
        slot_of_word[u] = v[i] & ~UID_CREATOR;
        uid[j0 + i] = u | UID_CREATOR;
        rep[u] = (u32)(j0 + i); count[u] = cnt[i]; ulen[u] = len[i]; uwords[u] = (len[i] + 7) >> 3;
        if (ustart) ustart[u] = st[i];
        mx = max(mx, len[i]);
        sum += len[i];
        u++;
    }
    mx = __reduce_max_sync(0xffffffffu, mx);
#pragma unroll
    for (int o = 16; o > 0; o >>= 1) sum += __shfl_xor_sync(0xffffffffu, sum, o);
    if ((threadIdx.x & 31) == 0 && sum) { atomicMax(&s_max, mx); atomicAdd(&s_sum, (unsigned long long)sum); }
    __syncthreads();
    if (threadIdx.x == 0 && s_sum) {
        atomicMax((unsigned long long *)&flags[2], (unsigned long long)s_max);
        atomicAdd((unsigned long long *)&flags[3], s_sum);
    }
}

__global__ void word_of_slot_k(const u32 *__restrict__ slot_of_word, u64 d, const u64 *__restrict__ d_ptr,
                               u32 *__restrict__ word_of_slot) {
    const u64 u = (u64)blockIdx.x * blockDim.x + threadIdx.x;
    if (u < (d_ptr ? *d_ptr : d)) word_of_slot[slot_of_word[u]] = (u32)u;
}

__device__ __forceinline__ u32 word_of(u32 v, const u32 *__restrict__ word_of_slot) {
    return (v & UID_CREATOR) ? v & ~UID_CREATOR : word_of_slot[v];
}

__global__ void uid_words_k(u32 *__restrict__ uid, u64 n, const u32 *__restrict__ word_of_slot) {
    const u64 q = (u64)blockIdx.x * blockDim.x + threadIdx.x;
    const u64 j = 4 * q;
    if (j + 4 <= n) {
        uint4 v = __ldcs(reinterpret_cast<const uint4 *>(uid) + q);
        v.x = word_of(v.x, word_of_slot); v.y = word_of(v.y, word_of_slot);
        v.z = word_of(v.z, word_of_slot); v.w = word_of(v.w, word_of_slot);
        __stcs(reinterpret_cast<uint4 *>(uid) + q, v);
    } else {
        for (u64 i = j; i < n; i++) uid[i] = word_of(uid[i], word_of_slot);
    }
}

static int uid_words(pfpb200_ctx *ctx, DictArrays *D, u64 n, u64 d_max, const u64 *d_ptr) {
    if (n && d_max) {
        u32 *word_of_slot = nullptr;
        PFP_TRY(pfp_alloc_t(ctx, &word_of_slot, D->slots));
        word_of_slot_k<<<pfp_blocks(d_max, 256), 256, 0, ctx->stream>>>(D->slot_of_word, d_max, d_ptr, word_of_slot);
        PFP_LAUNCHED(ctx);
        uid_words_k<<<pfp_blocks((n + 3) / 4, 256), 256, 0, ctx->stream>>>(D->uid, n, word_of_slot);
        PFP_LAUNCHED(ctx);
        PFP_TRY(pfp_free_now(ctx, word_of_slot));
    }
    PFP_TRY(pfp_free_now(ctx, D->slot_of_word));
    D->slot_of_word = nullptr;
    return PFPB200_OK;
}

int pfp_uid_words(pfpb200_ctx *ctx, DictArrays *D, u64 n) {
    return D->slot_of_word ? uid_words(ctx, D, n, D->d, nullptr) : PFPB200_OK;
}

static int table_words(pfpb200_ctx *ctx, const PhraseFp *rec, u64 n, DictSlot *tab, u64 cap,
                       const u32 *weight, const u32 *len_in, const u64 *ends, i64 first_start, u32 w,
                       u32 *uid, const DictArrays &D) {
    table_init_k<<<pfp_blocks(cap, 256), 256, 0, ctx->stream>>>(tab, cap);
    PFP_LAUNCHED(ctx);
    PFP_CUDA(ctx, cudaMemsetAsync(&ctx->d_flags[1], 0, 3 * sizeof(u64), ctx->stream));
    if (n == 0) return PFPB200_OK;
    int per_sm = 0;
    PFP_CUDA(ctx, cudaOccupancyMaxActiveBlocksPerMultiprocessor(&per_sm, table_insert_k, TI_T, 0));
    const u64 want = (n + TI_T - 1) / TI_T;
    const u64 resident = (u64)ctx->sm_count * (per_sm > 0 ? per_sm : 1);
    table_insert_k<<<(u32)(want < resident ? want : resident), TI_T, 0, ctx->stream>>>(
        rec, n, tab, cap, weight, ctx->weak_fp, uid, ctx->d_flags);
    PFP_LAUNCHED(ctx);
    const u32 nt = pfp_blocks(n, TC_TILE);
    u32 *tile = nullptr;
    PFP_TRY(pfp_alloc_t(ctx, &tile, nt));
    table_creators_k<<<nt, TC_T, 0, ctx->stream>>>(uid, n, tile);
    PFP_LAUNCHED(ctx);
    PFP_TRY(pfp_exclusive_scan_u32(ctx, tile, tile, nt, reinterpret_cast<u32 *>(&ctx->d_flags[1])));
    table_compact_k<<<nt, TC_T, 0, ctx->stream>>>(uid, n, tile, tab, len_in, ends, first_start, w, D.slot_of_word,
                                                  D.rep, D.count, D.ulen, D.uwords, D.ustart, ctx->d_flags);
    PFP_LAUNCHED(ctx);
    PFP_TRY(pfp_free_now(ctx, tile));
    return PFPB200_OK;
}

__global__ void table_pending_k(const DictSlot *__restrict__ tab, u64 P, u32 *__restrict__ uid,
                                u32 *__restrict__ count) {
    u64 j = (u64)blockIdx.x * blockDim.x + threadIdx.x;
    if (j >= P) return;
    const u32 v = uid[j];
    if (!(v & UID_PENDING)) return;
    const u32 u = tab[v & ~UID_PENDING].val - 1;
    uid[j] = u;
    atomicAdd(&count[u], 1u);
}

constexpr int PC_GROUP = 8;
constexpr int PC_PER_BLOCK = PH_T / PC_GROUP;

__device__ __forceinline__ u64 phrase_word8(const TextView &tv, i64 s0, u64 len, u64 k, bool special) {
    const u64 o = 8 * k;
    const u32 nbv = (u32)((len - o) < 8 ? (len - o) : 8);
    u64 v = 0;
    if (!special) {
        const u8 *p = tv.T + (s0 + (i64)o - tv.pos0);
        const u32 bs = (u32)((uintptr_t)p & 7);
        const u64 *p8 = reinterpret_cast<const u64 *>(p - bs);
        const u64 lo = __ldg(p8);
        if (bs) {
            const u64 hi = (bs + nbv > 8) ? __ldg(p8 + 1) : 0ull;
            v = (lo >> (8 * bs)) | (hi << (64 - 8 * bs));
        } else v = lo;
    } else {
        for (u32 b = 0; b < nbv; b++) v |= (u64)tv_byte(tv, s0 + (i64)o + b) << (8 * b);
    }
    if (nbv < 8) v &= (1ull << (8 * nbv)) - 1ull;
    return v;
}

__global__ void __launch_bounds__(PH_T) pool_copy_k(TextView tv, const u64 *__restrict__ ends,
                                                    i64 first_start, u32 w,
                                                    const u32 *__restrict__ rep,
                                                    const u32 *__restrict__ ulen,
                                                    const u64 *__restrict__ uoff, u64 d,
                                                    u64 *__restrict__ pool,
                                                    const u32 *__restrict__ ulist ,
                                                    const u32 *__restrict__ ucount, u64 pool_cap,
                                                    const i64 *__restrict__ ustart ) {
    const u32 li = threadIdx.x & (PC_GROUP - 1);
    if (ulist) d = *ucount;
    for (u64 x = (u64)blockIdx.x * PC_PER_BLOCK + (threadIdx.x / PC_GROUP); x < d;
         x += (u64)gridDim.x * PC_PER_BLOCK) {
        const u64 u = ulist ? ulist[x] : x;
        const u64 len = ulen[u];
        i64 s0, e;
        if (ustart) {
            s0 = ustart[u];
            e = s0 + (i64)len - 1;
        } else {
            const u64 j = rep[u];
            e = (i64)ends[j];
            s0 = (j == 0) ? first_start : (i64)ends[j - 1] - (i64)w + 1;
        }
        const bool special = (s0 < 0) || (e >= tv.n_global);
        u64 nw = (len + 7) >> 3;
        if (uoff[u] + nw > pool_cap) continue;
        u64 *dst = pool + uoff[u];
        for (u64 k = li; k < nw; k += PC_GROUP) dst[k] = phrase_word8(tv, s0, len, k, special);
    }
}

__global__ void __launch_bounds__(PH_T) pool_copy_span_k(TextView tv, const i64 *__restrict__ ustart,
                                                         const u32 *__restrict__ ulen,
                                                         const u64 *__restrict__ uoff, u64 d,
                                                         u64 *__restrict__ pool) {
    const u32 lane = threadIdx.x & 31;
    for (u64 u0 = ((u64)blockIdx.x * PH_WARPS + (threadIdx.x >> 5)) * 32; u0 < d; u0 += (u64)gridDim.x * PH_WARPS * 32) {
        const u64 u = u0 + lane;
        const bool have = u < d;
        const i64 s0 = have ? ustart[u] : 0;
        const u32 len = have ? ulen[u] : 0u;
        const u64 off = have ? uoff[u] : 0ull;
        const u64 base = __shfl_sync(0xffffffffu, off, 0);
        const u32 nw = (len + 7) >> 3;
        u32 rel = have ? (u32)(off - base) : 0xFFFFFFFFu;
        const u32 endrel = have ? rel + nw : 0u;
        u32 total = endrel;
#pragma unroll
        for (int o = 16; o > 0; o >>= 1) total = max(total, __shfl_xor_sync(0xffffffffu, total, o));
        const bool special = have && (s0 < 0 || s0 + (i64)len > tv.n_global);
        for (u32 k0 = 0; k0 < total; k0 += 32) {
            const u32 k = k0 + lane;
            u32 j = 0;
#pragma unroll
            for (int step = 16; step > 0; step >>= 1) {
                const u32 t = __shfl_sync(0xffffffffu, rel, (j + step) & 31);
                if (j + step < 32 && t <= k) j += step;
            }
            const u32 rj = __shfl_sync(0xffffffffu, rel, j);
            const u32 lj = __shfl_sync(0xffffffffu, len, j);
            const i64 sj = __shfl_sync(0xffffffffu, s0, j);
            const int spj = __shfl_sync(0xffffffffu, (int)special, j);
            if (k < total) pool[base + k] = phrase_word8(tv, sj, lj, k - rj, spj != 0);
        }
    }
}

__global__ void __launch_bounds__(PH_T) verify_phrases_k(TextView tv, const u64 *__restrict__ ends,
                                                         i64 first_start, u32 w, u64 P,
                                                         const u32 *__restrict__ uid,
                                                         const u32 *__restrict__ ulen,
                                                         const u64 *__restrict__ uoff,
                                                         const u64 *__restrict__ pool,
                                                         u64 *__restrict__ flags) {
    const u32 lane = threadIdx.x & 31;
    for (u64 j = (u64)blockIdx.x * PH_WARPS + (threadIdx.x >> 5); j < P; j += (u64)gridDim.x * PH_WARPS) {
        const i64 e = (i64)ends[j];
        const i64 s0 = (j == 0) ? first_start : (i64)ends[j - 1] - (i64)w + 1;
        const u64 len = (u64)(e - s0 + 1);
        const u32 u = uid[j];
        bool bad = len != (u64)ulen[u];
        if (!bad) {
            const bool special = (s0 < 0) || (e >= tv.n_global);
            const u64 *src = pool + uoff[u];
            const u64 nw = (len + 7) >> 3;
            for (u64 k = lane; k < nw; k += 32) bad |= phrase_word8(tv, s0, len, k, special) != src[k];
        }
        if (__any_sync(0xffffffffu, bad) && lane == 0)
            atomicOr((unsigned long long *)&flags[0], PFP_ERRBIT_COLLISION);
    }
}

__global__ void __launch_bounds__(PH_T) verify_entries_k(u64 n, const u32 *__restrict__ uid_of_entry,
                                                         const u32 *__restrict__ rep,
                                                         const u32 *__restrict__ len_in,
                                                         const u64 *__restrict__ in_off,
                                                         const u64 *__restrict__ pool,
                                                         u64 *__restrict__ flags) {
    const u32 lane = threadIdx.x & 31;
    for (u64 i = (u64)blockIdx.x * PH_WARPS + (threadIdx.x >> 5); i < n; i += (u64)gridDim.x * PH_WARPS) {
        const u32 r = rep[uid_of_entry[i]];
        if (r == (u32)i) continue;
        bool bad = len_in[i] != len_in[r];
        if (!bad) {
            const u64 *a = pool + in_off[i], *b = pool + in_off[r];
            const u64 nw = ((u64)len_in[i] + 7) >> 3;
            for (u64 k = lane; k < nw; k += 32) bad |= a[k] != b[k];
        }
        if (__any_sync(0xffffffffu, bad) && lane == 0)
            atomicOr((unsigned long long *)&flags[0], PFP_ERRBIT_COLLISION);
    }
}

__global__ void table_insert_list_k(const PhraseFp *__restrict__ rec_small, const u32 *__restrict__ list,
                                    const u32 *__restrict__ list_count, u32 list_cap,
                                    DictSlot *__restrict__ tab, u64 cap, const u64 *__restrict__ ends,
                                    i64 first_start, u32 w, u32 weak, u32 *__restrict__ uid,
                                    u32 *__restrict__ rep, u32 *__restrict__ ulen, u32 *__restrict__ uwords,
                                    u32 *__restrict__ count, u64 *__restrict__ uoff,
                                    PhraseFp *__restrict__ rec_full, u32 *__restrict__ created,
                                    u32 *__restrict__ created_count, u64 *__restrict__ flags) {
    const u32 i = blockIdx.x * blockDim.x + threadIdx.x;
    if (i >= min(*list_count, list_cap)) return;
    const u64 j = list[i];
    PhraseFp r = rec_small[i];
    if (weak) { r.fpa &= 3ull; r.fpb = 0; }
    const u64 k = sort_key_of(r.fpa, r.fpb);
    const u32 chk = check_of(r);
    const u64 s0 = __umul64hi(k, cap);
    const Probe pr = table_probe(tab, cap, s0, __ldcg(reinterpret_cast<const uint4 *>(tab + s0)), k);
    if (!pr.placed) { atomicOr((unsigned long long *)&flags[0], PFP_ERRBIT_TABLE_FULL); uid[j] = 0; return; }
    u32 seen = pr.seen_chk;
    if (pr.creator) {
        const i64 st = j ? (i64)ends[j - 1] - (i64)w + 1 : first_start;
        const u32 len = (u32)((i64)ends[j] - st + 1);
        const u32 uw = (len + 7) >> 3;
        const u32 u = (u32)atomicAdd((unsigned long long *)&flags[1], 1ull);
        const u64 off = atomicAdd((unsigned long long *)&flags[7], (unsigned long long)uw);
        atomicMax((unsigned long long *)&flags[2], (unsigned long long)len);
        atomicAdd((unsigned long long *)&flags[3], (unsigned long long)len);
        rep[u] = (u32)j; ulen[u] = len; uwords[u] = uw; uoff[u] = off;
        tab[pr.slot].val = u + 1;
        uid[j] = u;
        atomicAdd(&count[u], 1u);
        created[atomicAdd(created_count, 1u)] = u;
        if (rec_full) store_rec(rec_full, j, r.fpa, r.fpb);
    } else if (pr.seen_val) {
        uid[j] = pr.seen_val - 1;
        atomicAdd(&count[pr.seen_val - 1], 1u);
    } else {
        uid[j] = UID_PENDING | (u32)pr.slot;
        atomicOr((unsigned long long *)&flags[6], 1ull);
    }
    if (seen == 0u) seen = atomicCAS(&tab[pr.slot].chk, 0u, chk);
    if (seen != 0u && seen != chk) atomicOr((unsigned long long *)&flags[0], PFP_ERRBIT_COLLISION);
}

int pfp_insert_list(pfpb200_ctx *ctx, const TextView &tv, const PhraseFp *rec_small, const u32 *list,
                    const u32 *list_count, u64 list_cap, void *tab, u64 cap, const u64 *ends, i64 first_start,
                    u32 w, const DictArrays &D, u64 pool_cap, PhraseFp *rec_full) {
    u32 *created = nullptr;
    PFP_TRY(pfp_alloc_t(ctx, &created, (size_t)list_cap + 1));
    u32 *ccount = created + list_cap;
    PFP_CUDA(ctx, cudaMemsetAsync(ccount, 0, sizeof(u32), ctx->stream));
    const u32 lc = (u32)(list_cap < 0xFFFFFFFFull ? list_cap : 0xFFFFFFFFull);
    table_insert_list_k<<<pfp_blocks(list_cap, 128), 128, 0, ctx->stream>>>(
        rec_small, list, list_count, lc, (DictSlot *)tab, cap, ends, first_start, w, ctx->weak_fp, D.uid, D.rep, D.ulen,
        D.uwords, D.count, D.uoff, rec_full, created, ccount, ctx->d_flags);
    PFP_LAUNCHED(ctx);
    u64 want = (list_cap + PC_PER_BLOCK - 1) / PC_PER_BLOCK;
    u64 maxb = (u64)ctx->sm_count * 8;
    pool_copy_k<<<(u32)(want < maxb ? (want ? want : 1) : maxb), PH_T, 0, ctx->stream>>>(
        tv, ends, first_start, w, D.rep, D.ulen, D.uoff, 0, D.pool, created, ccount, pool_cap, nullptr);
    PFP_LAUNCHED(ctx);
    PFP_TRY(pfp_free_now(ctx, created));
    return PFPB200_OK;
}

int pfp_table_pending(pfpb200_ctx *ctx, const void *tab, u64 P, u32 *uid, u32 *count) {
    table_pending_k<<<pfp_blocks(P, 256), 256, 0, ctx->stream>>>((const DictSlot *)tab, P, uid, count);
    PFP_LAUNCHED(ctx);
    return PFPB200_OK;
}

int pfp_hash_list(pfpb200_ctx *ctx, const TextView &tv, const PhraseArrays &ph, i64 first_start, u32 w,
                  const u32 *long_list, const u32 *long_count, u64 max_count, PhraseFp *rec_compact) {
    u64 want = (max_count + PH_WARPS - 1) / PH_WARPS;
    u64 maxb = (u64)ctx->sm_count * 8;
    u32 nlb = (u32)(want < maxb ? want : maxb);
    if (nlb == 0) nlb = 1;
    phrase_hash_long_k<<<nlb, PH_T, 0, ctx->stream>>>(tv, ph, first_start, w, ctx->d_keys, long_list,
                                                      long_count, (u32)(max_count < 0xFFFFFFFFull ? max_count : 0xFFFFFFFFull),
                                                      ctx->d_flags, rec_compact);
    PFP_LAUNCHED(ctx);
    return PFPB200_OK;
}

int pfp_records_range(pfpb200_ctx *ctx, const TextView &tv, const PhraseArrays &ph, u64 j0, u64 P, u32 w) {
    if (j0 >= P) return PFPB200_OK;
    phrase_records_k<<<pfp_blocks(P - j0, 256), 256, 0, ctx->stream>>>(tv, ph.ends, j0, P, w, ph.last, ph.sai);
    PFP_LAUNCHED(ctx);
    return PFPB200_OK;
}

int pfp_phrase_init(pfpb200_ctx *ctx) {
    PFP_CUDA(ctx, cudaFuncSetAttribute(phrase_hash_k, cudaFuncAttributeMaxDynamicSharedMemorySize,
                                       PH_WARPS * PH_WIN));
    return PFPB200_OK;
}

int pfp_hash_stage(pfpb200_ctx *ctx, const TextView &tv, const PhraseArrays &ph, u64 P,
                   i64 first_start, u32 w) {
    u32 *long_list = nullptr, *long_count = nullptr;
    const u64 cap = P + 8;
    PFP_TRY(pfp_alloc_t(ctx, &long_list, (size_t)cap));
    PFP_TRY(pfp_alloc_t(ctx, &long_count, 1));
    PFP_CUDA(ctx, cudaMemsetAsync(long_count, 0, sizeof(u32), ctx->stream));
    phrase_records_k<<<pfp_blocks(P, 256), 256, 0, ctx->stream>>>(tv, ph.ends, 0, P, w, ph.last, ph.sai);
    PFP_LAUNCHED(ctx);
    u64 want = (P + PH_PER_BLOCK - 1) / PH_PER_BLOCK;
    u64 maxb = (u64)ctx->sm_count * 32;
    u32 nb = (u32)(want < maxb ? want : maxb);
    if (nb == 0) nb = 1;
    const int use_window = ctx->k2_window;
    phrase_hash_k<<<nb, PH_T, use_window ? PH_WARPS * PH_WIN : 0, ctx->stream>>>(
        tv, ph, P, first_start, w, ctx->d_keys, long_list, long_count, (u32)cap, ctx->d_flags, use_window);
    PFP_LAUNCHED(ctx);
    PFP_TRY(pfp_hash_list(ctx, tv, ph, first_start, w, long_list, long_count, cap, nullptr));
    PFP_TRY(pfp_free_now(ctx, long_list));
    PFP_TRY(pfp_free_now(ctx, long_count));
    return PFPB200_OK;
}

int pfp_dedup_stage(pfpb200_ctx *ctx, const PhraseArrays &ph, u64 P, i64 first_start, u32 w, DictArrays *D) {
    if (P >= 0x7FFFFFFEull) return pfp_fail(ctx, PFPB200_E_LIMIT, "more than 2^31-2 phrases in one shard");
    DictSlot *tab = nullptr;
    u64 cap = 0, d = 0;
    PFP_TRY(pfp_alloc_t(ctx, &D->uid, P));
    for (int attempt = 0;; attempt++) {
        double want = (double)P * 1.5;
        if (attempt == 0 && ctx->dedup_ratio > 0.0) {
            double guess = ctx->dedup_ratio * (double)P * ctx->table_scale;
            if (guess < want) want = guess;
        }
        cap = (u64)want + 1024;
        if (cap >= 0x7FFFFFFFull) cap = 0x7FFFFFFEull;
        const u64 wcap = cap < P ? cap : P;
        PFP_TRY(pfp_alloc_t(ctx, &tab, cap));
        PFP_TRY(pfp_alloc_t(ctx, &D->slot_of_word, wcap));
        PFP_TRY(pfp_alloc_t(ctx, &D->rep, wcap));
        PFP_TRY(pfp_alloc_t(ctx, &D->count, wcap));
        PFP_TRY(pfp_alloc_t(ctx, &D->ulen, wcap));
        PFP_TRY(pfp_alloc_t(ctx, &D->uwords, wcap));
        PFP_TRY(pfp_alloc_t(ctx, &D->ustart, wcap));
        PFP_TRY(table_words(ctx, ph.rec, P, tab, cap, nullptr, nullptr, ph.ends, first_start, w, D->uid, *D));
        PFP_CUDA(ctx, cudaMemcpyAsync(ctx->h_flags, ctx->d_flags, 4 * sizeof(u64), cudaMemcpyDeviceToHost,
                                      ctx->stream));
        PFP_CUDA(ctx, cudaStreamSynchronize(ctx->stream));
        if (ctx->h_flags[0] & PFP_ERRBIT_LIMIT)
            return pfp_fail(ctx, PFPB200_E_LIMIT, "a phrase is longer than 2^32-1 bytes");
        d = ctx->h_flags[1];
        const bool full = (ctx->h_flags[0] & PFP_ERRBIT_TABLE_FULL) != 0 || (double)d > 0.85 * (double)cap;
        if (!full) break;
        if (attempt > 0) return pfp_fail(ctx, PFPB200_E_INTERNAL, "dictionary table overflow");
        void *fr[] = {tab, D->slot_of_word, D->rep, D->count, D->ulen, D->uwords, D->ustart};
        for (void *q : fr) PFP_TRY(pfp_free_now(ctx, q));
        ctx->dedup_ratio = 0.0;
        const u64 keep = ctx->h_flags[0] & ~(PFP_ERRBIT_TABLE_FULL | PFP_ERRBIT_COLLISION);
        PFP_CUDA(ctx, cudaMemcpyAsync(&ctx->d_flags[0], &keep, sizeof(u64), cudaMemcpyHostToDevice, ctx->stream));
        PFP_CUDA(ctx, cudaStreamSynchronize(ctx->stream));
    }
    D->slots = cap;
    ctx->dedup_ratio = (double)d / (double)P;
    if (d > 0x7FFFFFFEull)
        return pfp_fail(ctx, PFPB200_E_LIMIT, "%llu distinct words exceed the limit 2^31-2",
                        (unsigned long long)d);
    D->d = d;
    D->max_len = (u32)ctx->h_flags[2];
    D->sum_len = ctx->h_flags[3];
    PFP_TRY(pfp_free_now(ctx, tab));
    return PFPB200_OK;
}

int pfp_pool_stage(pfpb200_ctx *ctx, const TextView &tv, const u64 *ends, i64 first_start, u32 w,
                   DictArrays *D) {
    u64 d = D->d;
    PFP_TRY(pfp_alloc_t(ctx, &D->uoff, d));
    PFP_TRY(pfp_exclusive_scan_u32_u64(ctx, D->uwords, D->uoff, d, &ctx->d_flags[1]));
    PFP_CUDA(ctx, cudaMemcpyAsync(ctx->h_flags, ctx->d_flags, 4 * sizeof(u64), cudaMemcpyDeviceToHost,
                                  ctx->stream));
    PFP_CUDA(ctx, cudaStreamSynchronize(ctx->stream));
    if (ctx->h_flags[0] & PFP_ERRBIT_COLLISION)
        return pfp_fail(ctx, PFPB200_E_COLLISION, "fingerprint collision between different phrases");
    D->pool_words = ctx->h_flags[1];
    D->max_len = (u32)ctx->h_flags[2];
    D->sum_len = ctx->h_flags[3];
    PFP_TRY(pfp_alloc_t(ctx, &D->pool, (size_t)D->pool_words));
    u64 want = (d + PC_PER_BLOCK - 1) / PC_PER_BLOCK;
    u64 maxb = (u64)ctx->sm_count * 32;
    u32 nb = (u32)(want < maxb ? want : maxb);
    if (nb == 0) nb = 1;
    if (D->ustart && !ctx->pool_by_word) {
        u64 wantw = (d + 32ull * PH_WARPS - 1) / (32ull * PH_WARPS);
        pool_copy_span_k<<<(u32)(wantw < maxb ? (wantw ? wantw : 1) : maxb), PH_T, 0, ctx->stream>>>(
            tv, D->ustart, D->ulen, D->uoff, d, D->pool);
    } else {
        pool_copy_k<<<nb, PH_T, 0, ctx->stream>>>(tv, ends, first_start, w, D->rep, D->ulen, D->uoff, d,
                                                  D->pool, nullptr, nullptr, D->pool_words, D->ustart);
    }
    PFP_LAUNCHED(ctx);
    return PFPB200_OK;
}

int pfp_merge_verify(pfpb200_ctx *ctx, u64 n, const u32 *uid_of_entry, const u32 *rep, const u32 *len_in,
                     const u32 *uwords_in, const u64 *pool) {
    if (n == 0) return PFPB200_OK;
    u64 *in_off = nullptr;
    PFP_TRY(pfp_alloc_t(ctx, &in_off, n));
    PFP_TRY(pfp_exclusive_scan_u32_u64(ctx, uwords_in, in_off, n, nullptr));
    u64 want = (n + PH_WARPS - 1) / PH_WARPS;
    u64 maxb = (u64)ctx->sm_count * 32;
    verify_entries_k<<<(u32)(want < maxb ? want : maxb), PH_T, 0, ctx->stream>>>(n, uid_of_entry, rep, len_in, in_off, pool,
                                                                                ctx->d_flags);
    PFP_LAUNCHED(ctx);
    PFP_CUDA(ctx, cudaMemcpyAsync(ctx->h_flags, ctx->d_flags, sizeof(u64), cudaMemcpyDeviceToHost, ctx->stream));
    PFP_CUDA(ctx, cudaStreamSynchronize(ctx->stream));
    PFP_TRY(pfp_free_now(ctx, in_off));
    if (ctx->h_flags[0] & PFP_ERRBIT_COLLISION)
        return pfp_fail(ctx, PFPB200_E_COLLISION, "two different words share a fingerprint (found by the verify pass)");
    return PFPB200_OK;
}

int pfp_verify_stage(pfpb200_ctx *ctx, const TextView &tv, const u64 *ends, i64 first_start, u32 w, u64 P,
                     const DictArrays &D) {
    if (P == 0) return PFPB200_OK;
    u64 want = (P + PH_WARPS - 1) / PH_WARPS;
    u64 maxb = (u64)ctx->sm_count * 32;
    verify_phrases_k<<<(u32)(want < maxb ? want : maxb), PH_T, 0, ctx->stream>>>(
        tv, ends, first_start, w, P, D.uid, D.ulen, D.uoff, D.pool, ctx->d_flags);
    PFP_LAUNCHED(ctx);
    return PFPB200_OK;
}

__global__ void merge_recs_k(const u64 *__restrict__ fpa, const u64 *__restrict__ fpb, u64 n,
                             PhraseFp *__restrict__ rec) {
    u64 i = (u64)blockIdx.x * blockDim.x + threadIdx.x;
    if (i < n) store_rec(rec, i, fpa[i], fpb[i]);
}

__global__ void merge_words_k(const u32 *__restrict__ rep, const u32 *__restrict__ uwords_in,
                              const u64 *__restrict__ in_off, const u64 *__restrict__ d_ptr,
                              u32 *__restrict__ uwords, u64 *__restrict__ uoff) {
    u64 u = (u64)blockIdx.x * blockDim.x + threadIdx.x;
    if (u >= *d_ptr) return;
    const u32 r = rep[u];
    uwords[u] = uwords_in[r];
    uoff[u] = in_off[r];
}

__global__ void gather_word_fp_k(const u32 *__restrict__ rep, const PhraseFp *__restrict__ rec,
                                 u64 d, u64 *__restrict__ wfpa, u64 *__restrict__ wfpb) {
    u64 u = (u64)blockIdx.x * blockDim.x + threadIdx.x;
    if (u >= d) return;
    u32 j = rep[u];
    wfpa[u] = rec[j].fpa;
    wfpb[u] = rec[j].fpb;
}

int pfp_gather_word_fp(pfpb200_ctx *ctx, const DictArrays &D, const PhraseArrays &ph, u64 *wfpa,
                       u64 *wfpb) {
    gather_word_fp_k<<<pfp_blocks(D.d, 256), 256, 0, ctx->stream>>>(D.rep, ph.rec, D.d, wfpa, wfpb);
    PFP_LAUNCHED(ctx);
    return PFPB200_OK;
}

int pfp_merge_stage(pfpb200_ctx *ctx, u64 n, const u64 *fpa, const u64 *fpb, const u32 *len,
                    const u32 *count_in, const u32 *uwords_in, const u64 *pool, u64 pool_words,
                    bool verify, DictArrays *D, u32 **uid_of_entry) {
    const int TB = 256;
    if (n >= 0x7FFFFFFEull / 2) return pfp_fail(ctx, PFPB200_E_LIMIT, "too many words to merge");
    PhraseFp *rec = nullptr;
    DictSlot *tab = nullptr;
    u64 *in_off = nullptr;
    const u64 cap = n + n / 2 + 1024;
    PFP_TRY(pfp_alloc_t(ctx, &rec, n));
    PFP_TRY(pfp_alloc_t(ctx, &tab, cap));
    PFP_TRY(pfp_alloc_t(ctx, &D->slot_of_word, n));
    PFP_TRY(pfp_alloc_t(ctx, &in_off, n));
    PFP_TRY(pfp_alloc_t(ctx, uid_of_entry, n));
    PFP_TRY(pfp_alloc_t(ctx, &D->rep, n));
    PFP_TRY(pfp_alloc_t(ctx, &D->count, n));
    PFP_TRY(pfp_alloc_t(ctx, &D->ulen, n));
    PFP_TRY(pfp_alloc_t(ctx, &D->uwords, n));
    PFP_TRY(pfp_alloc_t(ctx, &D->uoff, n));
    D->uid = *uid_of_entry;
    merge_recs_k<<<pfp_blocks(n, TB), TB, 0, ctx->stream>>>(fpa, fpb, n, rec);
    PFP_LAUNCHED(ctx);
    PFP_TRY(table_words(ctx, rec, n, tab, cap, count_in, len, nullptr, 0, 0, *uid_of_entry, *D));
    D->slots = cap;
    PFP_TRY(uid_words(ctx, D, n, n, reinterpret_cast<const u64 *>(&ctx->d_flags[1])));
    PFP_TRY(pfp_exclusive_scan_u32_u64(ctx, uwords_in, in_off, n, nullptr));
    merge_words_k<<<pfp_blocks(n, TB), TB, 0, ctx->stream>>>(D->rep, uwords_in, in_off,
                                                             reinterpret_cast<const u64 *>(&ctx->d_flags[1]),
                                                             D->uwords, D->uoff);
    PFP_LAUNCHED(ctx);
    if (verify) {
        u64 want = (n + PH_WARPS - 1) / PH_WARPS;
        u64 maxb = (u64)ctx->sm_count * 32;
        verify_entries_k<<<(u32)(want < maxb ? want : maxb), PH_T, 0, ctx->stream>>>(
            n, *uid_of_entry, D->rep, len, in_off, pool, ctx->d_flags);
        PFP_LAUNCHED(ctx);
    }
    PFP_CUDA(ctx, cudaMemcpyAsync(ctx->h_flags, ctx->d_flags, 4 * sizeof(u64), cudaMemcpyDeviceToHost,
                                  ctx->stream));
    PFP_CUDA(ctx, cudaStreamSynchronize(ctx->stream));
    if (ctx->h_flags[0] & PFP_ERRBIT_COLLISION)
        return pfp_fail(ctx, PFPB200_E_COLLISION, "fingerprint collision between different phrases");
    if (ctx->h_flags[0] & PFP_ERRBIT_TABLE_FULL)
        return pfp_fail(ctx, PFPB200_E_INTERNAL, "dictionary table overflow in the merge");
    if (ctx->h_flags[0] & PFP_ERRBIT_LIMIT)
        return pfp_fail(ctx, PFPB200_E_LIMIT, "a word occurs more than 2^32-1 times");
    const u64 d = ctx->h_flags[1];
    if (d > 0x7FFFFFFEull)
        return pfp_fail(ctx, PFPB200_E_LIMIT, "%llu distinct words exceed the limit 2^31-2",
                        (unsigned long long)d);
    D->d = d;
    D->pool = const_cast<u64 *>(pool);
    D->pool_words = pool_words;
    D->max_len = (u32)ctx->h_flags[2];
    D->sum_len = ctx->h_flags[3];
    void *fr[] = {rec, tab, in_off};
    for (void *q : fr) PFP_TRY(pfp_free_now(ctx, q));
    return PFPB200_OK;
}
```

big-bwt_b200/csrc/pfp_stages.cuh:

```cuda
#pragma once
#include "pfp_common.cuh"

struct TextView {
    const u8 *T;
    u64 n_buf;
    i64 pos0;
    i64 n_global;
};

__device__ __forceinline__ u8 tv_byte(const TextView &tv, i64 g) {
    if (g < 0 || g >= tv.n_global) return (u8)PFP_DOLLAR;
    return tv.T[g - tv.pos0];
}

struct __align__(16) PhraseFp {
    u64 fpa;
    u64 fpb;
};

struct PhraseArrays {
    u64 *ends;
    PhraseFp *rec;
    u8 *last;
    u8 *sai;
};

struct __align__(16) WordMeta { u64 off; u32 len; u32 count; };

constexpr u32 UID_CREATOR = 0x80000000u;

struct DictArrays {
    u64 d = 0;
    WordMeta *meta = nullptr;
    u32 *uid = nullptr;
    u32 *slot_of_word = nullptr;
    u64 slots = 0;
    u32 *rep = nullptr;
    i64 *ustart = nullptr;
    u32 *count = nullptr;
    u32 *ulen = nullptr;
    u32 *uwords = nullptr;
    u64 *uoff = nullptr;
    u64 *pool = nullptr;
    u64 pool_words = 0;
    u32 max_len = 0;
    u64 sum_len = 0;
};

constexpr u32 NH_SEG_BYTES = 8192;
constexpr u32 NH_KEY_WORDS = NH_SEG_BYTES / 4 + 8;
constexpr u64 NH_FOLD_A = 0x9E3779B97F4A7C15ULL;
constexpr u64 NH_FOLD_B = 0xD6E8FEB86659FD93ULL;

int pfp_scan_stage(pfpb200_ctx *ctx, const u8 *d_buf, u64 n_buf, u64 buf_pos0, u64 own_lo,
                   u64 own_hi, u32 w, u32 p, u64 extra_slots, bool held, u64 **d_out, u64 *n_out,
                   float *ms_scan, float *ms_emit);
int pfp_scan_bits(pfpb200_ctx *ctx, const u8 *d_buf, u64 n_buf, u64 buf_pos0, u64 own_lo, u64 own_hi,
                  u32 w, u32 p, bool held, ScanBits *sb, float *ms_scan);
int pfp_scan_emit(pfpb200_ctx *ctx, const ScanBits &sb, u64 *out);
int pfp_scan_first_last(pfpb200_ctx *ctx, const ScanBits &sb, u64 *d_out2);
int pfp_scan_bits_free(pfpb200_ctx *ctx, ScanBits *sb);
int pfp_hash_stage(pfpb200_ctx *ctx, const TextView &tv, const PhraseArrays &ph, u64 P,
                   i64 first_start, u32 w);
int pfp_hash_list(pfpb200_ctx *ctx, const TextView &tv, const PhraseArrays &ph, i64 first_start, u32 w,
                  const u32 *long_list, const u32 *long_count, u64 max_count, PhraseFp *rec_compact);
int pfp_insert_list(pfpb200_ctx *ctx, const TextView &tv, const PhraseFp *rec_small, const u32 *list,
                    const u32 *list_count, u64 list_cap, void *tab, u64 cap, const u64 *ends, i64 first_start,
                    u32 w, const DictArrays &D, u64 pool_cap, PhraseFp *rec_full);
int pfp_table_pending(pfpb200_ctx *ctx, const void *tab, u64 P, u32 *uid, u32 *count);
int pfp_words_fused_stage(pfpb200_ctx *ctx, const ScanBits &sb, const TextView &tv, const PhraseArrays &ph,
                          u64 P, i64 first_start, u32 w, bool emit_ends, DictArrays *D);
int pfp_records_range(pfpb200_ctx *ctx, const TextView &tv, const PhraseArrays &ph, u64 j0, u64 P, u32 w);
bool pfp_stream_ok(const ScanBits &sb, u32 w);
int pfp_stream_stage(pfpb200_ctx *ctx, const ScanBits &sb, const TextView &tv, const PhraseArrays &ph,
                     u64 P, i64 first_start, u32 w, bool emit_ends);
int pfp_dedup_stage(pfpb200_ctx *ctx, const PhraseArrays &ph, u64 P, i64 first_start, u32 w, DictArrays *D);
int pfp_uid_words(pfpb200_ctx *ctx, DictArrays *D, u64 n);
int pfp_pool_stage(pfpb200_ctx *ctx, const TextView &tv, const u64 *ends, i64 first_start, u32 w,
                   DictArrays *D);
int pfp_rank_stage(pfpb200_ctx *ctx, DictArrays &D, u32 **order, u32 *rounds, bool alpha_from_scan = false);
int pfp_dict_stage(pfpb200_ctx *ctx, const DictArrays &D, const u32 *order, u32 strip_w,
                   u8 **dict, u64 *dict_bytes, u32 **occ, u32 **rank_of_uid,
                   const u32 *remap_uid = nullptr, u64 remap_n = 0, u32 *remap_out = nullptr);
int pfp_remap_stage(pfpb200_ctx *ctx, const u32 *uid, const u32 *rank_of_uid, u64 P, u32 *parse);

int pfp_first_invalid(pfpb200_ctx *ctx, const u8 *d_text, u64 n, u64 *d_first);

int pfp_file_to_device(pfpb200_ctx *ctx, int fd, u64 off, u64 bytes, u8 *d_dst);
int pfp_device_to_file(pfpb200_ctx *ctx, const char *name, const void *d_src, u64 bytes);
int pfp_device_to_fd(pfpb200_ctx *ctx, int fd, u64 file_off, const void *d_src, u64 bytes, const char *name);
void pfp_io_destroy(pfpb200_ctx *ctx);
int pfp_fasta_device(pfpb200_ctx *ctx, const u8 *d_file, u64 n, u8 **d_text, u64 *n_text, int *supported,
                     bool held);

int pfp_gather_word_fp(pfpb200_ctx *ctx, const DictArrays &D, const PhraseArrays &ph, u64 *wfpa,
                       u64 *wfpb);
int pfp_merge_stage(pfpb200_ctx *ctx, u64 n, const u64 *fpa, const u64 *fpb, const u32 *len,
                    const u32 *count_in, const u32 *uwords_in, const u64 *pool, u64 pool_words,
                    bool verify, DictArrays *D, u32 **uid_of_entry);
int pfp_merge_verify(pfpb200_ctx *ctx, u64 n, const u32 *uid_of_entry, const u32 *rep, const u32 *len_in,
                     const u32 *uwords_in, const u64 *pool);
int pfp_verify_stage(pfpb200_ctx *ctx, const TextView &tv, const u64 *ends, i64 first_start, u32 w, u64 P,
                     const DictArrays &D);
```

big-bwt_b200/csrc/pfp_stream.cu:

```cuda
#include "pfp_common.cuh"
#include "pfp_stages.cuh"
#include "pfp_fp.cuh"
#include "pfp_table.cuh"
#include "pfp_tma.cuh"

constexpr int K2_T = PFP_TILE_T;
constexpr int K2_TILE = PFP_TILE;
constexpr int K2_HALO = 32;
constexpr int K2_EXT = 4096;
constexpr int K2_TEXT = K2_HALO + K2_TILE + K2_EXT + 32;
constexpr int K2_MWORDS = (K2_TILE + K2_EXT) / 32;
constexpr int K2_CAP = 1024;
constexpr int K2_NBIN = 34;
constexpr int K2_LANE_MAX = 32;
constexpr int K2_OFF_M = K2_TEXT;
constexpr int K2_OFF_K = K2_OFF_M + K2_MWORDS * 4;
constexpr int K2_OFF_SE = K2_OFF_K + NH_KEY_WORDS * 4;
constexpr int K2_OFF_PERM = K2_OFF_SE + (K2_CAP + 8) * 2;
constexpr int K2_SMEM = K2_OFF_PERM + K2_CAP * 2;
constexpr int K2_OFF_CQ = K2_SMEM;
constexpr int K2_OFF_CS = K2_OFF_CQ + K2_CAP * 2;
constexpr int K2_SMEM_FUSED = K2_OFF_CS + K2_CAP * 4;
static_assert(K2_OFF_CS % 4 == 0, "alignment of the creator slots");
constexpr u32 K2_NONE = 0xFFFFu;
static_assert(K2_T == 256, "block scan below is written for 256 threads");
static_assert(K2_TEXT % 16 == 0 && K2_MWORDS % 4 == 0 && NH_KEY_WORDS % 4 == 0, "16-byte staging");
static_assert(K2_OFF_SE % 16 == 0 && K2_TILE + K2_EXT < 0xFFFF, "tile-local positions are 16 bit");

struct StreamArgs {
    const uint4 *A;
    u64 q_end;
    u64 pos_bias;
    const uint4 *mask;
    u32 ntiles;
    const u64 *tile_off;
    u32 w;
    u64 *ends_out;
    u8 *last;
    u8 *sai;
    PhraseFp *rec;
    const u32 *keytab;
    u32 *long_list, *long_count;
    u64 n_regular;
    u64 *flags;
    DictSlot *tab;
    u64 cap;
    u32 *uid, *rep, *ulen, *uwords, *count;
    u64 *uoff, *pool;
    u64 pool_cap;
    u32 weak;
};

__device__ __forceinline__ void fused_insert(const StreamArgs &a, u64 j, u32 q, u64 pa, u64 pb, u32 *s_ncre,
                                             u16 *cq, u32 *cs) {
    PhraseFp r;
    r.fpa = pa; r.fpb = pb;
    if (a.weak) { r.fpa &= 3ull; r.fpb = 0; }
    const u64 k = sort_key_of(r.fpa, r.fpb);
    const u32 chk = check_of(r);
    const u64 s0 = __umul64hi(k, a.cap);
    const Probe pr = table_probe(a.tab, a.cap, s0, __ldcg(reinterpret_cast<const uint4 *>(a.tab + s0)), k);
    if (!pr.placed) {
        atomicOr((unsigned long long *)&a.flags[0], PFP_ERRBIT_TABLE_FULL);
        return;
    }
    u32 seen = pr.seen_chk;
    if (pr.creator) {
        const u32 i = atomicAdd(s_ncre, 1u);
        cq[i] = (u16)q;
        cs[i] = (u32)pr.slot;
        if (a.rec) store_rec(a.rec, j, pa, pb);
    } else if (pr.seen_val) {
        __stcs(a.uid + j, pr.seen_val - 1);
        atomicAdd(&a.count[pr.seen_val - 1], 1u);
    } else {
        __stcs(a.uid + j, UID_PENDING | (u32)pr.slot);
        atomicOr((unsigned long long *)&a.flags[6], 1ull);
    }
    if (seen == 0u) seen = atomicCAS(&a.tab[pr.slot].chk, 0u, chk);
    if (seen != 0u && seen != chk) atomicOr((unsigned long long *)&a.flags[0], PFP_ERRBIT_COLLISION);
}

__device__ __noinline__ uint4 k2_partial_chunk(const unsigned char *b, int nb) {
    u32 wds[4] = {0, 0, 0, 0};
    for (int i = 0; i < nb; i++) wds[i >> 2] |= (u32)b[i] << ((i & 3) * 8);
    return make_uint4(wds[0], wds[1], wds[2], wds[3]);
}

__device__ __forceinline__ void mask_tail(u32 &x0, u32 &x1, u32 &x2, u32 &x3, int rem) {
    const int t = 8 * rem;
    x0 &= ~__funnelshift_lc(0u, 0xFFFFFFFFu, (u32)t);
    x1 &= ~__funnelshift_lc(0u, 0xFFFFFFFFu, (u32)max(t - 32, 0));
    x2 &= ~__funnelshift_lc(0u, 0xFFFFFFFFu, (u32)max(t - 64, 0));
    x3 &= ~__funnelshift_lc(0u, 0xFFFFFFFFu, (u32)max(t - 96, 0));
}

__device__ __forceinline__ void nh_add(u64 &pa, u64 &pb, u32 x0, u32 x1, u32 x2, u32 x3, const uint4 &k0,
                                       const uint4 &k1) {
    pa += (u64)(x0 + k0.x) * (u64)(x1 + k0.y);
    pa += (u64)(x2 + k0.z) * (u64)(x3 + k0.w);
    pb += (u64)(x0 + k1.x) * (u64)(x1 + k1.y);
    pb += (u64)(x2 + k1.z) * (u64)(x3 + k1.w);
}

template <bool FUSED>
__global__ void __launch_bounds__(K2_T, 4) phrase_stream_k(const StreamArgs a) {
    extern __shared__ __align__(16) unsigned char smem[];
    u16 *cq = reinterpret_cast<u16 *>(smem + K2_OFF_CQ);
    u32 *cs = reinterpret_cast<u32 *>(smem + K2_OFF_CS);
    __shared__ u32 s_ncre, s_max;
    __shared__ unsigned long long s_sum, s_base_id, s_base_pool;
    u8 *sT = smem;
    u32 *sM = reinterpret_cast<u32 *>(smem + K2_OFF_M);
    u32 *sk = reinterpret_cast<u32 *>(smem + K2_OFF_K);
    u16 *se = reinterpret_cast<u16 *>(smem + K2_OFF_SE);
    u16 *perm = reinterpret_cast<u16 *>(smem + K2_OFF_PERM);
    __shared__ u32 s_scan[9];
    __shared__ u32 s_hist[K2_NBIN], s_cur[K2_NBIN];
    const u32 t = threadIdx.x, lane = t & 31, wp = t >> 5;
    const u64 tile = blockIdx.x;
    const i64 q0 = (i64)(tile * (u64)K2_TILE);
    const u32 w = a.w;

    __shared__ __align__(8) u64 s_bar;
    const i64 qs = q0 - K2_HALO;
    const bool bulk = qs >= 0 && (u64)qs + K2_TEXT <= (a.q_end & ~(u64)15) &&
                      (tile * (u64)K2_T + K2_MWORDS / 4) <= (u64)a.ntiles * K2_T;
    if (bulk) {
        if (t == 0) { mbar_init(&s_bar, 1); mbar_init_fence(); }
        __syncthreads();
        if (t == 0) {
            mbar_expect_tx(&s_bar, (u32)(K2_TEXT + K2_MWORDS * 4 + NH_KEY_WORDS * 4));
            bulk_copy_g2s(sT, a.A + (qs >> 4), K2_TEXT, &s_bar);
            bulk_copy_g2s(sM, a.mask + tile * (u64)K2_T, K2_MWORDS * 4, &s_bar);
            bulk_copy_g2s(sk, a.keytab, NH_KEY_WORDS * 4, &s_bar);
        }
        if (t < K2_NBIN) { s_hist[t] = 0; }
        if (t == 0) { s_ncre = 0; s_max = 0; s_sum = 0; }
        mbar_wait(&s_bar, 0);
    } else {
        for (int i = t; i < NH_KEY_WORDS / 4; i += K2_T)
            reinterpret_cast<uint4 *>(sk)[i] = __ldg(reinterpret_cast<const uint4 *>(a.keytab) + i);
        for (int c = t; c < K2_TEXT / 16; c += K2_T) {
            const i64 qc = qs + 16 * (i64)c;
            uint4 v = make_uint4(0, 0, 0, 0);
            if (qc >= 0 && (u64)qc + 16 <= a.q_end) v = __ldg(a.A + (qc >> 4));
            else if (qc >= 0 && (u64)qc < a.q_end)
                v = k2_partial_chunk(reinterpret_cast<const unsigned char *>(a.A) + qc, (int)(a.q_end - (u64)qc));
            reinterpret_cast<uint4 *>(sT)[c] = v;
        }
        for (int i = t; i < K2_MWORDS / 4; i += K2_T) {
            const u64 gi = tile * (u64)K2_T + (u64)i;
            uint4 v = make_uint4(0, 0, 0, 0);
            if (gi < (u64)a.ntiles * K2_T) v = __ldg(a.mask + gi);
            reinterpret_cast<uint4 *>(sM)[i] = v;
        }
        if (t < K2_NBIN) { s_hist[t] = 0; }
        if (t == 0) { s_ncre = 0; s_max = 0; s_sum = 0; }
    }
    __syncthreads();

    const uint4 mv = reinterpret_cast<const uint4 *>(sM)[t];
    u32 tot;
    const u32 ex = block_excl_scan_256(__popc(mv.x) + __popc(mv.y) + __popc(mv.z) + __popc(mv.w), &tot, s_scan);
    if (tot == 0) return;
    if (tot > (u32)K2_CAP) {
        if (t == 0) atomicOr((unsigned long long *)&a.flags[0], PFP_ERRBIT_INTERNAL);
        return;
    }
    {
        u32 o = ex;
        const u32 mw[4] = {mv.x, mv.y, mv.z, mv.w};
#pragma unroll
        for (int k = 0; k < 4; k++) {
            u32 x = mw[k];
            while (x) {
                const int b = __ffs(x) - 1;
                x &= x - 1;
                se[o++] = (u16)(t * 128 + k * 32 + b);
            }
        }
    }
    if (wp == 0) {
        u32 found = K2_NONE;
        for (int b0 = 0; b0 < K2_EXT / 32 && found == K2_NONE; b0 += 32) {
            const u32 x = sM[K2_TILE / 32 + b0 + lane];
            const u32 nz = __ballot_sync(0xffffffffu, x != 0);
            if (nz) {
                const int fl = __ffs(nz) - 1;
                const u32 xf = __shfl_sync(0xffffffffu, x, fl);
                found = (u32)(K2_TILE + 32 * (b0 + fl) + __ffs(xf) - 1);
            }
        }
        if (lane == 0) se[tot] = (u16)found;
    }
    __syncthreads();

    const u64 tile_first = a.tile_off[tile];
    for (u32 li = t; li < tot; li += K2_T) {
        const int e = se[li];
        const u64 idx = tile_first + li;
        const u64 g = (u64)(q0 + e) + a.pos_bias;
        if (a.ends_out) a.ends_out[idx] = g;
        a.last[idx] = (g < (u64)w) ? (u8)PFP_DOLLAR : sT[K2_HALO + e - (int)w];
        if (a.sai) {
            const u64 pos = g + 1;
            u8 *d = a.sai + idx * PFP_IBYTES;
#pragma unroll
            for (int k = 0; k < PFP_IBYTES; k++) d[k] = (u8)(pos >> (8 * k));
        }
    }

    u32 mybin[K2_CAP / K2_T];
#pragma unroll
    for (int r = 0; r < K2_CAP / K2_T; r++) {
        const u32 q = t + 1 + r * K2_T;
        u32 bin = 0;
        if (q <= tot && tile_first + q < a.n_regular) {
            const u32 e = se[q];
            const u32 len = e - se[q - 1] + w;
            const u32 nch = (len + 15) >> 4;
            if (e == K2_NONE || nch > NH_SEG_BYTES / 16) {
                a.long_list[atomicAdd(a.long_count, 1u)] = (u32)(tile_first + q);
            } else {
                bin = nch > (u32)K2_LANE_MAX ? (u32)K2_NBIN - 1 : nch;
                atomicAdd(&s_hist[bin], 1u);
            }
        }
        mybin[r] = bin;
    }
    __syncthreads();
    if (wp == 0) {
        const u32 rb = K2_NBIN - 1 - lane;
        const u32 h = s_hist[rb];
        const u32 inc = warp_incl_scan(h);
        s_cur[rb] = inc - h;
        const u32 above1 = __shfl_sync(0xffffffffu, inc, 31);
        if (lane == 0) { s_cur[1] = above1; s_scan[0] = above1 + s_hist[1]; }
    }
    __syncthreads();
#pragma unroll
    for (int r = 0; r < K2_CAP / K2_T; r++) {
        if (mybin[r]) perm[atomicAdd(&s_cur[mybin[r]], 1u)] = (u16)(t + 1 + r * K2_T);
    }
    const u32 nvalid = s_scan[0];
    const u32 nwarp = s_hist[K2_NBIN - 1];
    __syncthreads();

    for (u32 i = wp; i < nwarp; i += K2_T / 32) {
        const u32 q = perm[i];
        const int s = (int)se[q - 1] - (int)w + 1;
        const u32 len = (u32)se[q] - (u32)se[q - 1] + w;
        const u32 nch = (len + 15) >> 4;
        u64 pa = 0, pb = 0;
        for (u32 c = lane; c < nch; c += 32) {
            const int ad = s + K2_HALO + 16 * (int)c;
            const u32 *p4 = reinterpret_cast<const u32 *>(sT + (ad & ~3));
            const u32 sh = (u32)(ad & 3) * 8u;
            const u32 W0 = p4[0], W1 = p4[1], W2 = p4[2], W3 = p4[3], W4 = p4[4];
            u32 x0 = __funnelshift_r(W0, W1, sh), x1 = __funnelshift_r(W1, W2, sh);
            u32 x2 = __funnelshift_r(W2, W3, sh), x3 = __funnelshift_r(W3, W4, sh);
            if (c == nch - 1) mask_tail(x0, x1, x2, x3, (int)(len - 16 * c));
            const uint4 k0 = *reinterpret_cast<const uint4 *>(sk + 4 * c);
            const uint4 k1 = *reinterpret_cast<const uint4 *>(sk + 4 * c + 4);
            nh_add(pa, pb, x0, x1, x2, x3, k0, k1);
        }
#pragma unroll
        for (int o = 16; o > 0; o >>= 1) {
            pa += __shfl_xor_sync(0xffffffffu, pa, o);
            pb += __shfl_xor_sync(0xffffffffu, pb, o);
        }
        if (lane == 0) {
            if (FUSED) fused_insert(a, tile_first + q, q, pa, pb, &s_ncre, cq, cs);
            else store_rec(a.rec, tile_first + q, pa, pb);
        }
    }

    for (u32 i = nwarp + t; i < nvalid; i += K2_T) {
        const u32 q = perm[i];
        const int s = (int)se[q - 1] - (int)w + 1;
        const u32 len = (u32)se[q] - (u32)se[q - 1] + w;
        const u32 nch = (len + 15) >> 4;
        const int ad = s + K2_HALO;
        const u32 *p4 = reinterpret_cast<const u32 *>(sT + (ad & ~3));
        const u32 sh = (u32)(ad & 3) * 8u;
        const u32 *kp = sk;
        uint4 k0 = *reinterpret_cast<const uint4 *>(kp);
        u32 W0 = p4[0];
        u64 pa = 0, pb = 0;
        for (u32 c = 1; c < nch; c++) {
            const u32 W1 = p4[1], W2 = p4[2], W3 = p4[3], W4 = p4[4];
            const uint4 k1 = *reinterpret_cast<const uint4 *>(kp + 4);
            nh_add(pa, pb, __funnelshift_r(W0, W1, sh), __funnelshift_r(W1, W2, sh),
                   __funnelshift_r(W2, W3, sh), __funnelshift_r(W3, W4, sh), k0, k1);
            W0 = W4;
            k0 = k1;
            p4 += 4;
            kp += 4;
        }
        {
            const u32 W1 = p4[1], W2 = p4[2], W3 = p4[3], W4 = p4[4];
            const uint4 k1 = *reinterpret_cast<const uint4 *>(kp + 4);
            u32 x0 = __funnelshift_r(W0, W1, sh), x1 = __funnelshift_r(W1, W2, sh);
            u32 x2 = __funnelshift_r(W2, W3, sh), x3 = __funnelshift_r(W3, W4, sh);
            mask_tail(x0, x1, x2, x3, (int)(len - 16 * (nch - 1)));
            nh_add(pa, pb, x0, x1, x2, x3, k0, k1);
        }
        if (FUSED) fused_insert(a, tile_first + q, q, pa, pb, &s_ncre, cq, cs);
        else store_rec(a.rec, tile_first + q, pa, pb);
    }
    if (!FUSED) return;

    __syncthreads();
    const u32 ncre = s_ncre;
    if (ncre == 0) return;
    u32 my_off[K2_CAP / K2_T], my_len[K2_CAP / K2_T];
    u32 run_uw = 0;
    {
        u32 mx = 0, sl = 0;
#pragma unroll
        for (int r = 0; r < K2_CAP / K2_T; r++) {
            my_off[r] = 0; my_len[r] = 0;
            if ((u32)r * K2_T < ncre) {
                const u32 k = t + r * K2_T;
                u32 uw = 0;
                if (k < ncre) {
                    const u32 q = cq[k];
                    const u32 len = (u32)se[q] - (u32)se[q - 1] + w;
                    my_len[r] = len;
                    uw = (len + 7) >> 3;
                    mx = max(mx, len);
                    sl += len;
                }
                u32 tot2;
                const u32 ex2 = block_excl_scan_256(uw, &tot2, s_scan);
                my_off[r] = run_uw + ex2;
                run_uw += tot2;
            }
        }
        if (mx) { atomicMax(&s_max, mx); atomicAdd(&s_sum, (unsigned long long)sl); }
    }
    __syncthreads();
    if (t == 0) {
        s_base_id = atomicAdd((unsigned long long *)&a.flags[1], (unsigned long long)ncre);
        s_base_pool = atomicAdd((unsigned long long *)&a.flags[7], (unsigned long long)run_uw);
        atomicMax((unsigned long long *)&a.flags[2], (unsigned long long)s_max);
        atomicAdd((unsigned long long *)&a.flags[3], s_sum);
    }
    __syncthreads();
    const u32 base_id = (u32)s_base_id;
    const u64 base_pool = s_base_pool;
#pragma unroll
    for (int r = 0; r < K2_CAP / K2_T; r++) {
        const u32 k = t + r * K2_T;
        if (k < ncre) {
            const u32 q = cq[k];
            const u32 u = base_id + k;
            const u64 j = tile_first + q;
            a.rep[u] = (u32)j;
            a.ulen[u] = my_len[r];
            a.uwords[u] = (my_len[r] + 7) >> 3;
            a.uoff[u] = base_pool + my_off[r];
            a.tab[cs[k]].val = u + 1;
            __stcs(a.uid + j, u);
            atomicAdd(&a.count[u], 1u);
            cs[k] = my_off[r];
        }
    }
    __syncthreads();
    if (base_pool + run_uw > a.pool_cap) {
        if (t == 0) atomicOr((unsigned long long *)&a.flags[0], PFP_ERRBIT_POOL_FULL);
        return;
    }
    for (u32 k = wp; k < ncre; k += K2_T / 32) {
        const u32 q = cq[k];
        const int s = (int)se[q - 1] - (int)w + 1 + K2_HALO;
        const u32 len = (u32)se[q] - (u32)se[q - 1] + w;
        const u32 nw = (len + 7) >> 3;
        u64 *dst = a.pool + base_pool + cs[k];
        for (u32 i = lane; i < nw; i += 32) {
            const int ad = s + 8 * (int)i;
            const u32 *p4 = reinterpret_cast<const u32 *>(sT + (ad & ~3));
            const u32 sh = (u32)(ad & 3) * 8u;
            const u32 W0 = p4[0], W1 = p4[1], W2 = p4[2];
            u32 lo = __funnelshift_r(W0, W1, sh), hi = __funnelshift_r(W1, W2, sh);
            const int rem = (int)len - 8 * (int)i;
            if (rem < 8) {
                lo &= ~__funnelshift_lc(0u, 0xFFFFFFFFu, (u32)(8 * rem));
                hi &= ~__funnelshift_lc(0u, 0xFFFFFFFFu, (u32)max(8 * rem - 32, 0));
            }
            dst[i] = ((u64)hi << 32) | lo;
        }
    }
}

__global__ void special_list_k(u32 *list, u32 *count, u64 P, u64 total) {
    u32 n = *count;
    if (P > 0) list[n++] = 0u;
    if (P > total && total > 0) list[n++] = (u32)total;
    *count = n;
}

int pfp_stream_stage(pfpb200_ctx *ctx, const ScanBits &sb, const TextView &tv, const PhraseArrays &ph,
                     u64 P, i64 first_start, u32 w, bool emit_ends) {
    if (!pfp_stream_ok(sb, w)) return pfp_fail(ctx, PFPB200_E_INTERNAL, "stream stage: unsupported shape");
    u32 *list = nullptr;
    const u64 cap = 8ull * sb.ntiles + 8;
    PFP_TRY(pfp_alloc_t(ctx, &list, cap + 1));
    u32 *count = list + cap;
    PFP_CUDA(ctx, cudaMemsetAsync(count, 0, sizeof(u32), ctx->stream));
    if (sb.ntiles > 0 && sb.total > 0) {
        StreamArgs a{};
        a.A = sb.A; a.q_end = sb.q_end; a.pos_bias = sb.pos_bias;
        a.mask = sb.mask; a.ntiles = sb.ntiles; a.tile_off = sb.tile_off;
        a.w = w;
        a.ends_out = emit_ends ? ph.ends : nullptr;
        a.last = ph.last; a.sai = ph.sai; a.rec = ph.rec;
        a.keytab = ctx->d_keys; a.flags = ctx->d_flags;
        a.long_list = list; a.long_count = count;
        a.n_regular = sb.total;
        phrase_stream_k<false><<<sb.ntiles, K2_T, K2_SMEM, ctx->stream>>>(a);
        PFP_LAUNCHED(ctx);
    }
    special_list_k<<<1, 1, 0, ctx->stream>>>(list, count, P, sb.total);
    PFP_LAUNCHED(ctx);
    PFP_TRY(pfp_hash_list(ctx, tv, ph, first_start, w, list, count, cap, nullptr));
    PFP_TRY(pfp_records_range(ctx, tv, ph, sb.total, P, w));
    PFP_TRY(pfp_free_now(ctx, list));
    return PFPB200_OK;
}

int pfp_words_fused_stage(pfpb200_ctx *ctx, const ScanBits &sb, const TextView &tv, const PhraseArrays &ph,
                          u64 P, i64 first_start, u32 w, bool emit_ends, DictArrays *D) {
    if (!pfp_stream_ok(sb, w)) return pfp_fail(ctx, PFPB200_E_INTERNAL, "stream stage: unsupported shape");
    if (P >= 0x7FFFFFFEull) return pfp_fail(ctx, PFPB200_E_LIMIT, "more than 2^31-2 phrases in one shard");
    u32 *list = nullptr;
    const u64 lcap = 8ull * sb.ntiles + 8;
    PFP_TRY(pfp_alloc_t(ctx, &list, lcap + 1));
    u32 *lcount = list + lcap;
    PhraseFp *rec_small = nullptr;
    PFP_TRY(pfp_alloc_t(ctx, &rec_small, lcap));
    PFP_TRY(pfp_alloc_t(ctx, &D->uid, P));
    const u64 text_words = tv.n_buf / 8 + P * ((u64)w / 8 + 2) + 1024;
    u64 need_pool = 0;
    bool safe_table = false;
    for (int attempt = 0;; attempt++) {
        double want = (double)P * 1.5;
        if (!safe_table && ctx->dedup_ratio > 0.0) {
            const double guess = ctx->dedup_ratio * (double)P * ctx->table_scale;
            if (guess < want) want = guess;
        }
        u64 cap = (u64)want + 1024;
        if (cap >= 0x7FFFFFFFull) cap = 0x7FFFFFFEull;
        const u64 wcap = cap < P ? cap : P;
        u64 pool_cap = text_words;
        if (need_pool) pool_cap = need_pool + 1024;
        else if (ctx->pool_ratio > 0.0) pool_cap = (u64)(ctx->pool_ratio * 1.25 * (double)tv.n_buf / 8.0) + (1u << 16);
        else pool_cap = tv.n_buf / 24 + (1u << 16);
        if (pool_cap > text_words) pool_cap = text_words;
        DictSlot *tab = nullptr;
        PFP_TRY(pfp_alloc_t(ctx, &tab, cap));
        PFP_TRY(pfp_alloc_t(ctx, &D->rep, wcap));
        PFP_TRY(pfp_alloc_t(ctx, &D->count, wcap));
        PFP_TRY(pfp_alloc_t(ctx, &D->ulen, wcap));
        PFP_TRY(pfp_alloc_t(ctx, &D->uwords, wcap));
        PFP_TRY(pfp_alloc_t(ctx, &D->uoff, wcap));
        PFP_TRY(pfp_alloc_t(ctx, &D->pool, (size_t)pool_cap));
        PFP_TRY(pfp_table_init(ctx, tab, cap));
        PFP_CUDA(ctx, cudaMemsetAsync(D->count, 0, wcap * sizeof(u32), ctx->stream));
        PFP_CUDA(ctx, cudaMemsetAsync(&ctx->d_flags[1], 0, 3 * sizeof(u64), ctx->stream));
        PFP_CUDA(ctx, cudaMemsetAsync(&ctx->d_flags[6], 0, 2 * sizeof(u64), ctx->stream));
        PFP_CUDA(ctx, cudaMemsetAsync(lcount, 0, sizeof(u32), ctx->stream));
        if (sb.ntiles > 0 && sb.total > 0) {
            StreamArgs a{};
            a.A = sb.A; a.q_end = sb.q_end; a.pos_bias = sb.pos_bias;
            a.mask = sb.mask; a.ntiles = sb.ntiles; a.tile_off = sb.tile_off;
            a.w = w;
            a.ends_out = emit_ends ? ph.ends : nullptr;
            a.last = ph.last; a.sai = ph.sai; a.rec = ph.rec;
            a.keytab = ctx->d_keys; a.flags = ctx->d_flags;
            a.long_list = list; a.long_count = lcount;
            a.n_regular = sb.total;
            a.tab = tab; a.cap = cap;
            a.uid = D->uid; a.rep = D->rep; a.ulen = D->ulen; a.uwords = D->uwords; a.count = D->count;
            a.uoff = D->uoff; a.pool = D->pool; a.pool_cap = pool_cap; a.weak = ctx->weak_fp;
            phrase_stream_k<true><<<sb.ntiles, K2_T, K2_SMEM_FUSED, ctx->stream>>>(a);
            PFP_LAUNCHED(ctx);
        }
        special_list_k<<<1, 1, 0, ctx->stream>>>(list, lcount, P, sb.total);
        PFP_LAUNCHED(ctx);
        PFP_TRY(pfp_hash_list(ctx, tv, ph, first_start, w, list, lcount, lcap, rec_small));
        D->pool_words = pool_cap;
        PFP_TRY(pfp_insert_list(ctx, tv, rec_small, list, lcount, lcap, tab, cap, ph.ends, first_start, w, *D, pool_cap,
                                ph.rec));
        if (attempt == 0) PFP_TRY(pfp_records_range(ctx, tv, ph, sb.total, P, w));
        PFP_CUDA(ctx, cudaMemcpyAsync(ctx->h_flags, ctx->d_flags, 8 * sizeof(u64), cudaMemcpyDeviceToHost, ctx->stream));
        PFP_CUDA(ctx, cudaStreamSynchronize(ctx->stream));
        const u64 fl = ctx->h_flags[0];
        if (fl & PFP_ERRBIT_LIMIT) return pfp_fail(ctx, PFPB200_E_LIMIT, "a phrase is longer than 2^32-1 bytes");
        if (fl & PFP_ERRBIT_INTERNAL) return pfp_fail(ctx, PFPB200_E_INTERNAL, "stream stage: a tile exceeded its trigger capacity");
        const u64 d = ctx->h_flags[1];
        const bool table_full = (fl & PFP_ERRBIT_TABLE_FULL) != 0 || (double)d > 0.85 * (double)cap;
        const bool pool_full = (fl & PFP_ERRBIT_POOL_FULL) != 0 || ctx->h_flags[7] > pool_cap;
        if (!table_full && !pool_full) {
            if (fl & PFP_ERRBIT_COLLISION)
                return pfp_fail(ctx, PFPB200_E_COLLISION, "fingerprint collision between different phrases");
            if (ctx->h_flags[6]) PFP_TRY(pfp_table_pending(ctx, tab, P, D->uid, D->count));
            PFP_TRY(pfp_free_now(ctx, tab));
            ctx->dedup_ratio = (double)d / (double)P;
            ctx->pool_ratio = tv.n_buf ? 8.0 * (double)ctx->h_flags[7] / (double)tv.n_buf : 0.0;
            if (d > 0x7FFFFFFEull)
                return pfp_fail(ctx, PFPB200_E_LIMIT, "%llu distinct words exceed the limit 2^31-2", (unsigned long long)d);
            D->d = d;
            D->pool_words = ctx->h_flags[7];
            D->max_len = (u32)ctx->h_flags[2];
            D->sum_len = ctx->h_flags[3];
            break;
        }
        if (attempt >= 2) return pfp_fail(ctx, PFPB200_E_INTERNAL, "dictionary table / pool overflow after resizing");
        if (table_full) { safe_table = true; need_pool = (ctx->h_flags[7] > pool_cap ? ctx->h_flags[7] : pool_cap) * 3 / 2; }
        else need_pool = ctx->h_flags[7];
        void *fr[] = {tab, D->rep, D->count, D->ulen, D->uwords, D->uoff, D->pool};
        for (void *q : fr) PFP_TRY(pfp_free_now(ctx, q));
        ctx->dedup_ratio = 0.0;
        const u64 keep = fl & ~(PFP_ERRBIT_TABLE_FULL | PFP_ERRBIT_POOL_FULL | PFP_ERRBIT_COLLISION);
        PFP_CUDA(ctx, cudaMemcpyAsync(&ctx->d_flags[0], &keep, sizeof(u64), cudaMemcpyHostToDevice, ctx->stream));
        PFP_CUDA(ctx, cudaStreamSynchronize(ctx->stream));
    }
    PFP_TRY(pfp_free_now(ctx, list));
    PFP_TRY(pfp_free_now(ctx, rec_small));
    return PFPB200_OK;
}

int pfp_stream_init(pfpb200_ctx *ctx) {
    PFP_CUDA(ctx, cudaFuncSetAttribute(phrase_stream_k<false>, cudaFuncAttributeMaxDynamicSharedMemorySize, K2_SMEM));
    PFP_CUDA(ctx, cudaFuncSetAttribute(phrase_stream_k<true>, cudaFuncAttributeMaxDynamicSharedMemorySize, K2_SMEM_FUSED));
    return PFPB200_OK;
}

bool pfp_stream_ok(const ScanBits &sb, u32 w) {
    return w <= (u32)K2_HALO && sb.max_tile_cnt <= (u32)K2_CAP;
}
```

big-bwt_b200/csrc/pfp_table.cuh:

```cuda
#pragma once
#include "pfp_common.cuh"
#include "pfp_stages.cuh"
#include "pfp_fp.cuh"

struct __align__(16) DictSlot { u64 key; u32 val; u32 chk; };
constexpr u32 TABLE_MAX_PROBES = 2048;
constexpr u32 UID_PENDING = 0x80000000u;

__device__ __forceinline__ u32 check_of(const PhraseFp &r) {
    u64 x = (r.fpa + 0x632BE59BD9B4E019ULL) * 0xD1342543DE82EF95ULL;
    x ^= (rotl64(r.fpb, 23) + 0x2545F4914F6CDD1DULL) * 0xAF251AF3B0F025B5ULL;
    x ^= x >> 29;
    u32 c = (u32)(x ^ (x >> 32));
    return c ? c : 1u;
}

int pfp_table_init(pfpb200_ctx *ctx, DictSlot *tab, u64 cap);

struct Probe { u64 slot; bool placed; bool creator; u32 seen_chk; u32 seen_val; };

__device__ __forceinline__ Probe table_probe(DictSlot *__restrict__ tab, u64 cap, u64 slot, uint4 sv, u64 k) {
    Probe r{slot, false, false, 0u, 0u};
    u32 probes = 0;
    for (;;) {
        const u64 key = ((u64)sv.y << 32) | sv.x;
        if (key == k) { r.placed = true; r.seen_val = sv.z; r.seen_chk = sv.w; break; }
        if (key == 0ull) {
            const u64 prev = atomicCAS((unsigned long long *)&tab[r.slot].key, 0ull, (unsigned long long)k);
            if (prev == 0ull) { r.placed = true; r.creator = true; break; }
            if (prev == k) { r.placed = true; break; }
        }
        if (++probes > TABLE_MAX_PROBES) break;
        r.slot = (r.slot + 1 == cap) ? 0 : r.slot + 1;
        sv = __ldcg(reinterpret_cast<const uint4 *>(tab + r.slot));
    }
    return r;
}
```

big-bwt_b200/csrc/pfp_tma.cuh:

```cuda
#pragma once
#include "pfp_common.cuh"

__device__ __forceinline__ u32 smem_addr_u32(const void *p) { return (u32)__cvta_generic_to_shared(p); }

__device__ __forceinline__ void mbar_init(u64 *bar, u32 arrivals) {
    asm volatile("mbarrier.init.shared::cta.b64 [%0], %1;" ::"r"(smem_addr_u32(bar)), "r"(arrivals) : "memory");
}
__device__ __forceinline__ void mbar_init_fence() {
    asm volatile("fence.mbarrier_init.release.cluster;" ::: "memory");
}
__device__ __forceinline__ void mbar_expect_tx(u64 *bar, u32 bytes) {
    asm volatile("mbarrier.arrive.expect_tx.shared::cta.b64 _, [%0], %1;" ::"r"(smem_addr_u32(bar)), "r"(bytes) : "memory");
}
__device__ __forceinline__ void bulk_copy_g2s(void *dst, const void *src, u32 bytes, u64 *bar) {
    asm volatile("cp.async.bulk.shared::cluster.global.mbarrier::complete_tx::bytes [%0], [%1], %2, [%3];"
                 ::"r"(smem_addr_u32(dst)), "l"(src), "r"(bytes), "r"(smem_addr_u32(bar)) : "memory");
}
__device__ __forceinline__ void mbar_wait(u64 *bar, u32 parity) {
    u32 ok;
    do {
        asm volatile("{\n\t.reg .pred p;\n\tmbarrier.try_wait.parity.shared::cta.b64 p, [%1], %2;\n\tselp.u32 %0, 1, 0, p;\n\t}"
                     : "=r"(ok) : "r"(smem_addr_u32(bar)), "r"(parity) : "memory");
    } while (!ok);
}
```

Before: 530.6.

## Make phrase stream kernel persistent with TMA staging and drop fused insert path

Removes the opt-in fused K3 path, which did dictionary table insertion inside the stream kernel, along with its helper kernels. The phrase stream kernel becomes a persistent, templated kernel launched on an occupancy-sized grid. Each block loops over tiles and stages text and trigger masks through bulk async copies into a stage buffer. This is meant to cut per-tile launch and setup overhead and to allow overlap and L2 prefetch, but it adds sequential tile loops per block and more barrier synchronisation.

```diff
diff --git a/big-bwt_b200/csrc/pfp_api.cu b/big-bwt_b200/csrc/pfp_api.cu
--- a/big-bwt_b200/csrc/pfp_api.cu
+++ b/big-bwt_b200/csrc/pfp_api.cu
@@ -94,7 +94,6 @@
     { const char *ev = getenv("PFPB200_RANK_CHUNK_PASSES"); ctx->rank_chunk_passes = ev && atoi(ev) != 0; }
     { const char *ev = getenv("PFPB200_RANK_WARP_PASSES"); ctx->rank_warp_passes = ev && atoi(ev) != 0; }
     { const char *ev = getenv("PFPB200_POOL_BY_WORD"); ctx->pool_by_word = ev && atoi(ev) != 0; }
-    { const char *ev = getenv("PFPB200_FUSE_K3"); ctx->fuse_k3 = ev && atoi(ev) != 0; }
     { const char *ev = getenv("PFPB200_TABLE_SCALE"); if (ev && atof(ev) >= 1.2) ctx->table_scale = atof(ev); }
     { const char *ev = getenv("PFPB200_K1_MIX"); ctx->k1_mix = ev ? atoi(ev) : 0; }
     { const char *ev = getenv("PFPB200_K2_WINDOW"); ctx->k2_window = ev ? atoi(ev) : 0; }
@@ -248,16 +247,11 @@
         TextView tv{d_text, n, 0, (i64)n};
         DictArrays D;
         const bool stream = pfp_stream_ok(sb, w) && !ctx->legacy_k2;
-        const bool fused = stream && ctx->fuse_k3;
-        if (fused) {
-            PFP_TRY(pfp_words_fused_stage(ctx, sb, tv, ph, P, -1, w, true, &D));
-        } else {
-            PFP_TRY(pfp_alloc_t(ctx, &ph.rec, P));
-            if (stream) PFP_TRY(pfp_stream_stage(ctx, sb, tv, ph, P, -1, w, true));
-            else {
-                PFP_TRY(pfp_scan_emit(ctx, sb, ends));
-                PFP_TRY(pfp_hash_stage(ctx, tv, ph, P, -1, w));
-            }
+        PFP_TRY(pfp_alloc_t(ctx, &ph.rec, P));
+        if (stream) PFP_TRY(pfp_stream_stage(ctx, sb, tv, ph, P, -1, w, true));
+        else {
+            PFP_TRY(pfp_scan_emit(ctx, sb, ends));
+            PFP_TRY(pfp_hash_stage(ctx, tv, ph, P, -1, w));
         }
         PFP_TRY(pfp_scan_bits_free(ctx, &sb));
         tm.mark(ctx->stream);
@@ -278,11 +272,9 @@
             PFP_CUDA(ctx, cudaEventRecord(ctx->ev_copy, ctx->copy_stream));
             ctx->early_done = true;
         }
-        if (!fused) {
-            PFP_TRY(pfp_dedup_stage(ctx, ph, P, -1, w, &D));
-            PFP_TRY(pfp_free_now(ctx, ph.rec));
-            PFP_TRY(pfp_pool_stage(ctx, tv, ends, -1, w, &D));
-        }
+        PFP_TRY(pfp_dedup_stage(ctx, ph, P, -1, w, &D));
+        PFP_TRY(pfp_free_now(ctx, ph.rec));
+        PFP_TRY(pfp_pool_stage(ctx, tv, ends, -1, w, &D));
         if (o->flags & PFPB200_F_VERIFY) {
             PFP_TRY(pfp_uid_words(ctx, &D, P));
             PFP_TRY(pfp_verify_stage(ctx, tv, ends, -1, w, P, D));
@@ -720,21 +712,16 @@
         TextView tv{sh.d_buf, sh.n_buf, (i64)sh.buf_pos0, (i64)sh.n_global};
         DictArrays D;
         const bool stream = pfp_stream_ok(ctx->sh.bits, w) && !ctx->legacy_k2;
-        const bool fused = stream && ctx->fuse_k3;
-        if (fused) {
-            PFP_TRY(pfp_words_fused_stage(ctx, ctx->sh.bits, tv, ph, P, first_start, w, !ctx->sh.ends_emitted, &D));
-        } else {
-            if (stream) PFP_TRY(pfp_stream_stage(ctx, ctx->sh.bits, tv, ph, P, first_start, w, !ctx->sh.ends_emitted));
-            else PFP_TRY(pfp_hash_stage(ctx, tv, ph, P, first_start, w));
-            PFP_TRY(pfp_dedup_stage(ctx, ph, P, first_start, w, &D));
-            PFP_TRY(pfp_uid_words(ctx, &D, P));
-        }
+        if (stream) PFP_TRY(pfp_stream_stage(ctx, ctx->sh.bits, tv, ph, P, first_start, w, !ctx->sh.ends_emitted));
+        else PFP_TRY(pfp_hash_stage(ctx, tv, ph, P, first_start, w));
+        PFP_TRY(pfp_dedup_stage(ctx, ph, P, first_start, w, &D));
+        PFP_TRY(pfp_uid_words(ctx, &D, P));
         u64 *wfpa = nullptr, *wfpb = nullptr;
         PFP_TRY(pfp_alloc_t(ctx, &wfpa, D.d));
         PFP_TRY(pfp_alloc_t(ctx, &wfpb, D.d));
         PFP_TRY(pfp_gather_word_fp(ctx, D, ph, wfpa, wfpb));
         PFP_TRY(pfp_free_now(ctx, ph.rec));
-        if (!fused) PFP_TRY(pfp_pool_stage(ctx, tv, ends, first_start, w, &D));
+        PFP_TRY(pfp_pool_stage(ctx, tv, ends, first_start, w, &D));
         PFP_TRY(pfp_free_now(ctx, D.rep));
         if (o.flags & PFPB200_F_VERIFY) PFP_TRY(pfp_verify_stage(ctx, tv, ends, first_start, w, P, D));
         PFP_CUDA(ctx, cudaMemcpyAsync(ctx->h_flags, ctx->d_flags, sizeof(u64), cudaMemcpyDeviceToHost, ctx->stream));
diff --git a/big-bwt_b200/csrc/pfp_common.cuh b/big-bwt_b200/csrc/pfp_common.cuh
--- a/big-bwt_b200/csrc/pfp_common.cuh
+++ b/big-bwt_b200/csrc/pfp_common.cuh
@@ -67,9 +67,8 @@
     bool rank_chunk_passes = false;
     bool rank_warp_passes = false;
     bool pool_by_word = false;
-    bool fuse_k3 = false;
-    double pool_ratio = 0.0;
     bool legacy_k2 = false;
+    u32 k2_grid = 0;
     double table_scale = 2.0;
     u32 weak_fp = 0;
     int k1_mix = 0;
diff --git a/big-bwt_b200/csrc/pfp_phrase.cu b/big-bwt_b200/csrc/pfp_phrase.cu
--- a/big-bwt_b200/csrc/pfp_phrase.cu
+++ b/big-bwt_b200/csrc/pfp_phrase.cu
@@ -489,17 +489,6 @@
     return PFPB200_OK;
 }
 
-__global__ void table_pending_k(const DictSlot *__restrict__ tab, u64 P, u32 *__restrict__ uid,
-                                u32 *__restrict__ count) {
-    u64 j = (u64)blockIdx.x * blockDim.x + threadIdx.x;
-    if (j >= P) return;
-    const u32 v = uid[j];
-    if (!(v & UID_PENDING)) return;
-    const u32 u = tab[v & ~UID_PENDING].val - 1;
-    uid[j] = u;
-    atomicAdd(&count[u], 1u);
-}
-
 constexpr int PC_GROUP = 8;
 constexpr int PC_PER_BLOCK = PH_T / PC_GROUP;
 
@@ -635,77 +624,6 @@
         if (__any_sync(0xffffffffu, bad) && lane == 0)
             atomicOr((unsigned long long *)&flags[0], PFP_ERRBIT_COLLISION);
     }
-}
-
-__global__ void table_insert_list_k(const PhraseFp *__restrict__ rec_small, const u32 *__restrict__ list,
-                                    const u32 *__restrict__ list_count, u32 list_cap,
-                                    DictSlot *__restrict__ tab, u64 cap, const u64 *__restrict__ ends,
-                                    i64 first_start, u32 w, u32 weak, u32 *__restrict__ uid,
-                                    u32 *__restrict__ rep, u32 *__restrict__ ulen, u32 *__restrict__ uwords,
-                                    u32 *__restrict__ count, u64 *__restrict__ uoff,
-                                    PhraseFp *__restrict__ rec_full, u32 *__restrict__ created,
-                                    u32 *__restrict__ created_count, u64 *__restrict__ flags) {
-    const u32 i = blockIdx.x * blockDim.x + threadIdx.x;
-    if (i >= min(*list_count, list_cap)) return;
-    const u64 j = list[i];
-    PhraseFp r = rec_small[i];
-    if (weak) { r.fpa &= 3ull; r.fpb = 0; }
-    const u64 k = sort_key_of(r.fpa, r.fpb);
-    const u32 chk = check_of(r);
-    const u64 s0 = __umul64hi(k, cap);
-    const Probe pr = table_probe(tab, cap, s0, __ldcg(reinterpret_cast<const uint4 *>(tab + s0)), k);
-    if (!pr.placed) { atomicOr((unsigned long long *)&flags[0], PFP_ERRBIT_TABLE_FULL); uid[j] = 0; return; }
-    u32 seen = pr.seen_chk;
-    if (pr.creator) {
-        const i64 st = j ? (i64)ends[j - 1] - (i64)w + 1 : first_start;
-        const u32 len = (u32)((i64)ends[j] - st + 1);
-        const u32 uw = (len + 7) >> 3;
-        const u32 u = (u32)atomicAdd((unsigned long long *)&flags[1], 1ull);
-        const u64 off = atomicAdd((unsigned long long *)&flags[7], (unsigned long long)uw);
-        atomicMax((unsigned long long *)&flags[2], (unsigned long long)len);
-        atomicAdd((unsigned long long *)&flags[3], (unsigned long long)len);
-        rep[u] = (u32)j; ulen[u] = len; uwords[u] = uw; uoff[u] = off;
-        tab[pr.slot].val = u + 1;
-        uid[j] = u;
-        atomicAdd(&count[u], 1u);
-        created[atomicAdd(created_count, 1u)] = u;
-        if (rec_full) store_rec(rec_full, j, r.fpa, r.fpb);
-    } else if (pr.seen_val) {
-        uid[j] = pr.seen_val - 1;
-        atomicAdd(&count[pr.seen_val - 1], 1u);
-    } else {
-        uid[j] = UID_PENDING | (u32)pr.slot;
-        atomicOr((unsigned long long *)&flags[6], 1ull);
-    }
-    if (seen == 0u) seen = atomicCAS(&tab[pr.slot].chk, 0u, chk);
-    if (seen != 0u && seen != chk) atomicOr((unsigned long long *)&flags[0], PFP_ERRBIT_COLLISION);
-}
-
-int pfp_insert_list(pfpb200_ctx *ctx, const TextView &tv, const PhraseFp *rec_small, const u32 *list,
-                    const u32 *list_count, u64 list_cap, void *tab, u64 cap, const u64 *ends, i64 first_start,
-                    u32 w, const DictArrays &D, u64 pool_cap, PhraseFp *rec_full) {
-    u32 *created = nullptr;
-    PFP_TRY(pfp_alloc_t(ctx, &created, (size_t)list_cap + 1));
-    u32 *ccount = created + list_cap;
-    PFP_CUDA(ctx, cudaMemsetAsync(ccount, 0, sizeof(u32), ctx->stream));
-    const u32 lc = (u32)(list_cap < 0xFFFFFFFFull ? list_cap : 0xFFFFFFFFull);
-    table_insert_list_k<<<pfp_blocks(list_cap, 128), 128, 0, ctx->stream>>>(
-        rec_small, list, list_count, lc, (DictSlot *)tab, cap, ends, first_start, w, ctx->weak_fp, D.uid, D.rep, D.ulen,
-        D.uwords, D.count, D.uoff, rec_full, created, ccount, ctx->d_flags);
-    PFP_LAUNCHED(ctx);
-    u64 want = (list_cap + PC_PER_BLOCK - 1) / PC_PER_BLOCK;
-    u64 maxb = (u64)ctx->sm_count * 8;
-    pool_copy_k<<<(u32)(want < maxb ? (want ? want : 1) : maxb), PH_T, 0, ctx->stream>>>(
-        tv, ends, first_start, w, D.rep, D.ulen, D.uoff, 0, D.pool, created, ccount, pool_cap, nullptr);
-    PFP_LAUNCHED(ctx);
-    PFP_TRY(pfp_free_now(ctx, created));
-    return PFPB200_OK;
-}
-
-int pfp_table_pending(pfpb200_ctx *ctx, const void *tab, u64 P, u32 *uid, u32 *count) {
-    table_pending_k<<<pfp_blocks(P, 256), 256, 0, ctx->stream>>>((const DictSlot *)tab, P, uid, count);
-    PFP_LAUNCHED(ctx);
-    return PFPB200_OK;
 }
 
 int pfp_hash_list(pfpb200_ctx *ctx, const TextView &tv, const PhraseArrays &ph, i64 first_start, u32 w,
diff --git a/big-bwt_b200/csrc/pfp_stages.cuh b/big-bwt_b200/csrc/pfp_stages.cuh
--- a/big-bwt_b200/csrc/pfp_stages.cuh
+++ b/big-bwt_b200/csrc/pfp_stages.cuh
@@ -64,12 +64,6 @@
                    i64 first_start, u32 w);
 int pfp_hash_list(pfpb200_ctx *ctx, const TextView &tv, const PhraseArrays &ph, i64 first_start, u32 w,
                   const u32 *long_list, const u32 *long_count, u64 max_count, PhraseFp *rec_compact);
-int pfp_insert_list(pfpb200_ctx *ctx, const TextView &tv, const PhraseFp *rec_small, const u32 *list,
-                    const u32 *list_count, u64 list_cap, void *tab, u64 cap, const u64 *ends, i64 first_start,
-                    u32 w, const DictArrays &D, u64 pool_cap, PhraseFp *rec_full);
-int pfp_table_pending(pfpb200_ctx *ctx, const void *tab, u64 P, u32 *uid, u32 *count);
-int pfp_words_fused_stage(pfpb200_ctx *ctx, const ScanBits &sb, const TextView &tv, const PhraseArrays &ph,
-                          u64 P, i64 first_start, u32 w, bool emit_ends, DictArrays *D);
 int pfp_records_range(pfpb200_ctx *ctx, const TextView &tv, const PhraseArrays &ph, u64 j0, u64 P, u32 w);
 bool pfp_stream_ok(const ScanBits &sb, u32 w);
 int pfp_stream_stage(pfpb200_ctx *ctx, const ScanBits &sb, const TextView &tv, const PhraseArrays &ph,
diff --git a/big-bwt_b200/csrc/pfp_stream.cu b/big-bwt_b200/csrc/pfp_stream.cu
--- a/big-bwt_b200/csrc/pfp_stream.cu
+++ b/big-bwt_b200/csrc/pfp_stream.cu
@@ -1,31 +1,31 @@
 #include "pfp_common.cuh"
 #include "pfp_stages.cuh"
 #include "pfp_fp.cuh"
-#include "pfp_table.cuh"
 #include "pfp_tma.cuh"
 
-constexpr int K2_T = PFP_TILE_T;
 constexpr int K2_TILE = PFP_TILE;
+constexpr int K2_TILE_V4 = K2_TILE / 128;
 constexpr int K2_HALO = 32;
 constexpr int K2_EXT = 4096;
 constexpr int K2_TEXT = K2_HALO + K2_TILE + K2_EXT + 32;
 constexpr int K2_MWORDS = (K2_TILE + K2_EXT) / 32;
+constexpr int K2_STAGE = K2_TEXT + K2_MWORDS * 4;
 constexpr int K2_CAP = 1024;
 constexpr int K2_NBIN = 34;
 constexpr int K2_LANE_MAX = 32;
-constexpr int K2_OFF_M = K2_TEXT;
-constexpr int K2_OFF_K = K2_OFF_M + K2_MWORDS * 4;
+constexpr int K2_OFF_K = 0;
 constexpr int K2_OFF_SE = K2_OFF_K + NH_KEY_WORDS * 4;
 constexpr int K2_OFF_PERM = K2_OFF_SE + (K2_CAP + 8) * 2;
-constexpr int K2_SMEM = K2_OFF_PERM + K2_CAP * 2;
-constexpr int K2_OFF_CQ = K2_SMEM;
-constexpr int K2_OFF_CS = K2_OFF_CQ + K2_CAP * 2;
-constexpr int K2_SMEM_FUSED = K2_OFF_CS + K2_CAP * 4;
-static_assert(K2_OFF_CS % 4 == 0, "alignment of the creator slots");
+constexpr int K2_OFF_ST = K2_OFF_PERM + K2_CAP * 2;
 constexpr u32 K2_NONE = 0xFFFFu;
-static_assert(K2_T == 256, "block scan below is written for 256 threads");
 static_assert(K2_TEXT % 16 == 0 && K2_MWORDS % 4 == 0 && NH_KEY_WORDS % 4 == 0, "16-byte staging");
-static_assert(K2_OFF_SE % 16 == 0 && K2_TILE + K2_EXT < 0xFFFF, "tile-local positions are 16 bit");
+static_assert(K2_OFF_SE % 16 == 0 && K2_OFF_ST % 16 == 0 && K2_STAGE % 16 == 0, "16-byte staging");
+static_assert(K2_TILE + K2_EXT < 0xFFFF, "tile-local positions are 16 bit");
+static_assert(K2_TILE / 32 == 1024, "trigger-bit words of a tile");
+
+constexpr int K2_T = 256;
+constexpr int K2_NST = 1;
+constexpr int K2_SMEM = K2_OFF_ST + K2_NST * K2_STAGE;
 
 struct StreamArgs {
     const uint4 *A;
@@ -43,43 +43,7 @@
     u32 *long_list, *long_count;
     u64 n_regular;
     u64 *flags;
-    DictSlot *tab;
-    u64 cap;
-    u32 *uid, *rep, *ulen, *uwords, *count;
-    u64 *uoff, *pool;
-    u64 pool_cap;
-    u32 weak;
 };
-
-__device__ __forceinline__ void fused_insert(const StreamArgs &a, u64 j, u32 q, u64 pa, u64 pb, u32 *s_ncre,
-                                             u16 *cq, u32 *cs) {
-    PhraseFp r;
-    r.fpa = pa; r.fpb = pb;
-    if (a.weak) { r.fpa &= 3ull; r.fpb = 0; }
-    const u64 k = sort_key_of(r.fpa, r.fpb);
-    const u32 chk = check_of(r);
-    const u64 s0 = __umul64hi(k, a.cap);
-    const Probe pr = table_probe(a.tab, a.cap, s0, __ldcg(reinterpret_cast<const uint4 *>(a.tab + s0)), k);
-    if (!pr.placed) {
-        atomicOr((unsigned long long *)&a.flags[0], PFP_ERRBIT_TABLE_FULL);
-        return;
-    }
-    u32 seen = pr.seen_chk;
-    if (pr.creator) {
-        const u32 i = atomicAdd(s_ncre, 1u);
-        cq[i] = (u16)q;
-        cs[i] = (u32)pr.slot;
-        if (a.rec) store_rec(a.rec, j, pa, pb);
-    } else if (pr.seen_val) {
-        __stcs(a.uid + j, pr.seen_val - 1);
-        atomicAdd(&a.count[pr.seen_val - 1], 1u);
-    } else {
-        __stcs(a.uid + j, UID_PENDING | (u32)pr.slot);
-        atomicOr((unsigned long long *)&a.flags[6], 1ull);
-    }
-    if (seen == 0u) seen = atomicCAS(&a.tab[pr.slot].chk, 0u, chk);
-    if (seen != 0u && seen != chk) atomicOr((unsigned long long *)&a.flags[0], PFP_ERRBIT_COLLISION);
-}
 
 __device__ __noinline__ uint4 k2_partial_chunk(const unsigned char *b, int nb) {
     u32 wds[4] = {0, 0, 0, 0};
@@ -103,293 +67,258 @@
     pb += (u64)(x2 + k1.z) * (u64)(x3 + k1.w);
 }
 
-template <bool FUSED>
-__global__ void __launch_bounds__(K2_T, 4) phrase_stream_k(const StreamArgs a) {
+template <int T>
+__device__ __forceinline__ u32 k2_block_scan(u32 v, u32 *total, u32 *sm ) {
+    constexpr int NW = T / 32;
+    const u32 inc = warp_incl_scan(v);
+    const u32 w = threadIdx.x >> 5;
+    __syncthreads();
+    if (lane_id() == 31) sm[w] = inc;
+    __syncthreads();
+    if (threadIdx.x < 32) {
+        const u32 x = threadIdx.x < (u32)NW ? sm[threadIdx.x] : 0;
+        const u32 xi = warp_incl_scan(x);
+        if (threadIdx.x < (u32)NW) sm[threadIdx.x] = xi - x;
+        if (threadIdx.x == (u32)NW - 1) sm[32] = xi;
+    }
+    __syncthreads();
+    *total = sm[32];
+    return inc - v + sm[w];
+}
+
+__device__ __forceinline__ bool k2_bulk(const StreamArgs &a, u64 tile) {
+    const i64 qs = (i64)(tile * (u64)K2_TILE) - K2_HALO;
+    return qs >= 0 && (u64)qs + K2_TEXT <= (a.q_end & ~(u64)15) &&
+           (tile * (u64)K2_TILE_V4 + K2_MWORDS / 4) <= (u64)a.ntiles * K2_TILE_V4;
+}
+
+__device__ __forceinline__ void k2_issue(const StreamArgs &a, u64 tile, unsigned char *stage, u64 *bar) {
+    fence_proxy_async_smem();
+    mbar_expect_tx(bar, (u32)K2_STAGE);
+    bulk_copy_g2s(stage, a.A + ((tile * (u64)K2_TILE - K2_HALO) >> 4), K2_TEXT, bar);
+    bulk_copy_g2s(stage + K2_TEXT, a.mask + tile * (u64)K2_TILE_V4, K2_MWORDS * 4, bar);
+}
+
+template <int T, int NST>
+__global__ void __launch_bounds__(T, NST == 1 ? 4 : NST == 2 ? 2 : 1) phrase_stream_k(const StreamArgs a) {
+    constexpr int WPT = 1024 / T;
+    static_assert(WPT == 2 || WPT == 4, "256 or 512 threads");
     extern __shared__ __align__(16) unsigned char smem[];
-    u16 *cq = reinterpret_cast<u16 *>(smem + K2_OFF_CQ);
-    u32 *cs = reinterpret_cast<u32 *>(smem + K2_OFF_CS);
-    __shared__ u32 s_ncre, s_max;
-    __shared__ unsigned long long s_sum, s_base_id, s_base_pool;
-    u8 *sT = smem;
-    u32 *sM = reinterpret_cast<u32 *>(smem + K2_OFF_M);
     u32 *sk = reinterpret_cast<u32 *>(smem + K2_OFF_K);
     u16 *se = reinterpret_cast<u16 *>(smem + K2_OFF_SE);
     u16 *perm = reinterpret_cast<u16 *>(smem + K2_OFF_PERM);
-    __shared__ u32 s_scan[9];
+    __shared__ __align__(8) u64 s_bar[NST];
+    __shared__ u32 s_scan[33];
     __shared__ u32 s_hist[K2_NBIN], s_cur[K2_NBIN];
     const u32 t = threadIdx.x, lane = t & 31, wp = t >> 5;
-    const u64 tile = blockIdx.x;
-    const i64 q0 = (i64)(tile * (u64)K2_TILE);
     const u32 w = a.w;
-
-    __shared__ __align__(8) u64 s_bar;
-    const i64 qs = q0 - K2_HALO;
-    const bool bulk = qs >= 0 && (u64)qs + K2_TEXT <= (a.q_end & ~(u64)15) &&
-                      (tile * (u64)K2_T + K2_MWORDS / 4) <= (u64)a.ntiles * K2_T;
-    if (bulk) {
-        if (t == 0) { mbar_init(&s_bar, 1); mbar_init_fence(); }
+    const u64 step = gridDim.x;
+
+    if (t == 0) {
+        for (int s = 0; s < NST; s++) mbar_init(&s_bar[s], 1);
+        mbar_init_fence();
+        for (int s = 0; s < NST - 1; s++) {
+            const u64 tl = blockIdx.x + s * step;
+            if (tl < a.ntiles && k2_bulk(a, tl)) k2_issue(a, tl, smem + K2_OFF_ST + s * K2_STAGE, &s_bar[s]);
+        }
+    }
+    for (int i = t; i < NH_KEY_WORDS / 4; i += T)
+        reinterpret_cast<uint4 *>(sk)[i] = __ldg(reinterpret_cast<const uint4 *>(a.keytab) + i);
+
+    u32 parity = 0;
+    int s = 0;
+    for (u64 tile = blockIdx.x; tile < a.ntiles; tile += step, s = (s + 1 == NST) ? 0 : s + 1) {
+        unsigned char *sT = smem + K2_OFF_ST + s * K2_STAGE;
+        const u32 *sM = reinterpret_cast<const u32 *>(sT + K2_TEXT);
+        const i64 q0 = (i64)(tile * (u64)K2_TILE);
+        const i64 qs = q0 - K2_HALO;
+
         __syncthreads();
         if (t == 0) {
-            mbar_expect_tx(&s_bar, (u32)(K2_TEXT + K2_MWORDS * 4 + NH_KEY_WORDS * 4));
-            bulk_copy_g2s(sT, a.A + (qs >> 4), K2_TEXT, &s_bar);
-            bulk_copy_g2s(sM, a.mask + tile * (u64)K2_T, K2_MWORDS * 4, &s_bar);
-            bulk_copy_g2s(sk, a.keytab, NH_KEY_WORDS * 4, &s_bar);
-        }
-        if (t < K2_NBIN) { s_hist[t] = 0; }
-        if (t == 0) { s_ncre = 0; s_max = 0; s_sum = 0; }
-        mbar_wait(&s_bar, 0);
-    } else {
-        for (int i = t; i < NH_KEY_WORDS / 4; i += K2_T)
-            reinterpret_cast<uint4 *>(sk)[i] = __ldg(reinterpret_cast<const uint4 *>(a.keytab) + i);
-        for (int c = t; c < K2_TEXT / 16; c += K2_T) {
-            const i64 qc = qs + 16 * (i64)c;
-            uint4 v = make_uint4(0, 0, 0, 0);
-            if (qc >= 0 && (u64)qc + 16 <= a.q_end) v = __ldg(a.A + (qc >> 4));
-            else if (qc >= 0 && (u64)qc < a.q_end)
-                v = k2_partial_chunk(reinterpret_cast<const unsigned char *>(a.A) + qc, (int)(a.q_end - (u64)qc));
-            reinterpret_cast<uint4 *>(sT)[c] = v;
-        }
-        for (int i = t; i < K2_MWORDS / 4; i += K2_T) {
-            const u64 gi = tile * (u64)K2_T + (u64)i;
-            uint4 v = make_uint4(0, 0, 0, 0);
-            if (gi < (u64)a.ntiles * K2_T) v = __ldg(a.mask + gi);
-            reinterpret_cast<uint4 *>(sM)[i] = v;
-        }
-        if (t < K2_NBIN) { s_hist[t] = 0; }
-        if (t == 0) { s_ncre = 0; s_max = 0; s_sum = 0; }
-    }
-    __syncthreads();
-
-    const uint4 mv = reinterpret_cast<const uint4 *>(sM)[t];
-    u32 tot;
-    const u32 ex = block_excl_scan_256(__popc(mv.x) + __popc(mv.y) + __popc(mv.z) + __popc(mv.w), &tot, s_scan);
-    if (tot == 0) return;
-    if (tot > (u32)K2_CAP) {
-        if (t == 0) atomicOr((unsigned long long *)&a.flags[0], PFP_ERRBIT_INTERNAL);
-        return;
-    }
-    {
-        u32 o = ex;
-        const u32 mw[4] = {mv.x, mv.y, mv.z, mv.w};
-#pragma unroll
-        for (int k = 0; k < 4; k++) {
-            u32 x = mw[k];
-            while (x) {
-                const int b = __ffs(x) - 1;
-                x &= x - 1;
-                se[o++] = (u16)(t * 128 + k * 32 + b);
-            }
-        }
-    }
-    if (wp == 0) {
-        u32 found = K2_NONE;
-        for (int b0 = 0; b0 < K2_EXT / 32 && found == K2_NONE; b0 += 32) {
-            const u32 x = sM[K2_TILE / 32 + b0 + lane];
-            const u32 nz = __ballot_sync(0xffffffffu, x != 0);
-            if (nz) {
-                const int fl = __ffs(nz) - 1;
-                const u32 xf = __shfl_sync(0xffffffffu, x, fl);
-                found = (u32)(K2_TILE + 32 * (b0 + fl) + __ffs(xf) - 1);
-            }
-        }
-        if (lane == 0) se[tot] = (u16)found;
-    }
-    __syncthreads();
-
-    const u64 tile_first = a.tile_off[tile];
-    for (u32 li = t; li < tot; li += K2_T) {
-        const int e = se[li];
-        const u64 idx = tile_first + li;
-        const u64 g = (u64)(q0 + e) + a.pos_bias;
-        if (a.ends_out) a.ends_out[idx] = g;
-        a.last[idx] = (g < (u64)w) ? (u8)PFP_DOLLAR : sT[K2_HALO + e - (int)w];
-        if (a.sai) {
-            const u64 pos = g + 1;
-            u8 *d = a.sai + idx * PFP_IBYTES;
-#pragma unroll
-            for (int k = 0; k < PFP_IBYTES; k++) d[k] = (u8)(pos >> (8 * k));
-        }
-    }
-
-    u32 mybin[K2_CAP / K2_T];
-#pragma unroll
-    for (int r = 0; r < K2_CAP / K2_T; r++) {
-        const u32 q = t + 1 + r * K2_T;
-        u32 bin = 0;
-        if (q <= tot && tile_first + q < a.n_regular) {
-            const u32 e = se[q];
-            const u32 len = e - se[q - 1] + w;
+            const u64 nx = tile + (NST - 1) * step;
+            const int sn = (s + NST - 1) % NST;
+            if (nx < a.ntiles && k2_bulk(a, nx)) k2_issue(a, nx, smem + K2_OFF_ST + sn * K2_STAGE, &s_bar[sn]);
+            const u64 nl = nx + step;
+            if (nl < a.ntiles && k2_bulk(a, nl)) {
+                bulk_prefetch_l2(a.A + ((nl * (u64)K2_TILE - K2_HALO) >> 4), K2_TEXT);
+                bulk_prefetch_l2(a.mask + nl * (u64)K2_TILE_V4, K2_MWORDS * 4);
+            }
+        }
+        if (t < K2_NBIN) s_hist[t] = 0;
+        const u64 tile_first = a.tile_off[tile];
+        if (k2_bulk(a, tile)) {
+            if (t == 0) mbar_wait(&s_bar[s], (parity >> s) & 1u);
+            parity ^= 1u << s;
+        } else {
+            for (int c = t; c < K2_TEXT / 16; c += T) {
+                const i64 qc = qs + 16 * (i64)c;
+                uint4 v = make_uint4(0, 0, 0, 0);
+                if (qc >= 0 && (u64)qc + 16 <= a.q_end) v = __ldg(a.A + (qc >> 4));
+                else if (qc >= 0 && (u64)qc < a.q_end)
+                    v = k2_partial_chunk(reinterpret_cast<const unsigned char *>(a.A) + qc, (int)(a.q_end - (u64)qc));
+                reinterpret_cast<uint4 *>(sT)[c] = v;
+            }
+            for (int i = t; i < K2_MWORDS / 4; i += T) {
+                const u64 gi = tile * (u64)K2_TILE_V4 + (u64)i;
+                uint4 v = make_uint4(0, 0, 0, 0);
+                if (gi < (u64)a.ntiles * K2_TILE_V4) v = __ldg(a.mask + gi);
+                reinterpret_cast<uint4 *>(sT + K2_TEXT)[i] = v;
+            }
+        }
+        __syncthreads();
+
+        u32 mw[WPT];
+        if constexpr (WPT == 4) {
+            const uint4 v = reinterpret_cast<const uint4 *>(sM)[t];
+            mw[0] = v.x; mw[1] = v.y; mw[2] = v.z; mw[3] = v.w;
+        } else {
+            const uint2 v = reinterpret_cast<const uint2 *>(sM)[t];
+            mw[0] = v.x; mw[1] = v.y;
+        }
+        u32 cnt = 0;
+#pragma unroll
+        for (int k = 0; k < WPT; k++) cnt += __popc(mw[k]);
+        u32 tot;
+        const u32 ex = k2_block_scan<T>(cnt, &tot, s_scan);
+        if (tot == 0) continue;
+        if (tot > (u32)K2_CAP) {
+            if (t == 0) atomicOr((unsigned long long *)&a.flags[0], PFP_ERRBIT_INTERNAL);
+            continue;
+        }
+        {
+            u32 o = ex;
+#pragma unroll
+            for (int k = 0; k < WPT; k++) {
+                u32 x = mw[k];
+                while (x) {
+                    const int b = __ffs(x) - 1;
+                    x &= x - 1;
+                    se[o++] = (u16)((t * WPT + k) * 32 + b);
+                }
+            }
+        }
+        if (wp == 0) {
+            u32 found = K2_NONE;
+            for (int b0 = 0; b0 < K2_EXT / 32 && found == K2_NONE; b0 += 32) {
+                const u32 x = sM[K2_TILE / 32 + b0 + lane];
+                const u32 nz = __ballot_sync(0xffffffffu, x != 0);
+                if (nz) {
+                    const int fl = __ffs(nz) - 1;
+                    const u32 xf = __shfl_sync(0xffffffffu, x, fl);
+                    found = (u32)(K2_TILE + 32 * (b0 + fl) + __ffs(xf) - 1);
+                }
+            }
+            if (lane == 0) se[tot] = (u16)found;
+        }
+        __syncthreads();
+
+        for (u32 li = t; li < tot; li += T) {
+            const int e = se[li];
+            const u64 idx = tile_first + li;
+            const u64 g = (u64)(q0 + e) + a.pos_bias;
+            if (a.ends_out) a.ends_out[idx] = g;
+            a.last[idx] = (g < (u64)w) ? (u8)PFP_DOLLAR : sT[K2_HALO + e - (int)w];
+            if (a.sai) {
+                const u64 pos = g + 1;
+                u8 *d = a.sai + idx * PFP_IBYTES;
+#pragma unroll
+                for (int k = 0; k < PFP_IBYTES; k++) d[k] = (u8)(pos >> (8 * k));
+            }
+        }
+
+        u32 mybin[K2_CAP / T];
+#pragma unroll
+        for (int r = 0; r < K2_CAP / T; r++) {
+            const u32 q = t + 1 + r * T;
+            u32 bin = 0;
+            if (q <= tot && tile_first + q < a.n_regular) {
+                const u32 e = se[q];
+                const u32 len = e - se[q - 1] + w;
+                const u32 nch = (len + 15) >> 4;
+                if (e == K2_NONE || nch > NH_SEG_BYTES / 16) {
+                    a.long_list[atomicAdd(a.long_count, 1u)] = (u32)(tile_first + q);
+                } else {
+                    bin = nch > (u32)K2_LANE_MAX ? (u32)K2_NBIN - 1 : nch;
+                    atomicAdd(&s_hist[bin], 1u);
+                }
+            }
+            mybin[r] = bin;
+        }
+        __syncthreads();
+        if (wp == 0) {
+            const u32 rb = K2_NBIN - 1 - lane;
+            const u32 h = s_hist[rb];
+            const u32 inc = warp_incl_scan(h);
+            s_cur[rb] = inc - h;
+            const u32 above1 = __shfl_sync(0xffffffffu, inc, 31);
+            if (lane == 0) { s_cur[1] = above1; s_scan[0] = above1 + s_hist[1]; }
+        }
+        __syncthreads();
+#pragma unroll
+        for (int r = 0; r < K2_CAP / T; r++) {
+            if (mybin[r]) perm[atomicAdd(&s_cur[mybin[r]], 1u)] = (u16)(t + 1 + r * T);
+        }
+        const u32 nvalid = s_scan[0];
+        const u32 nwarp = s_hist[K2_NBIN - 1];
+        __syncthreads();
+
+        for (u32 i = wp; i < nwarp; i += T / 32) {
+            const u32 q = perm[i];
+            const int st = (int)se[q - 1] - (int)w + 1;
+            const u32 len = (u32)se[q] - (u32)se[q - 1] + w;
             const u32 nch = (len + 15) >> 4;
-            if (e == K2_NONE || nch > NH_SEG_BYTES / 16) {
-                a.long_list[atomicAdd(a.long_count, 1u)] = (u32)(tile_first + q);
-            } else {
-                bin = nch > (u32)K2_LANE_MAX ? (u32)K2_NBIN - 1 : nch;
-                atomicAdd(&s_hist[bin], 1u);
-            }
-        }
-        mybin[r] = bin;
-    }
-    __syncthreads();
-    if (wp == 0) {
-        const u32 rb = K2_NBIN - 1 - lane;
-        const u32 h = s_hist[rb];
-        const u32 inc = warp_incl_scan(h);
-        s_cur[rb] = inc - h;
-        const u32 above1 = __shfl_sync(0xffffffffu, inc, 31);
-        if (lane == 0) { s_cur[1] = above1; s_scan[0] = above1 + s_hist[1]; }
-    }
-    __syncthreads();
-#pragma unroll
-    for (int r = 0; r < K2_CAP / K2_T; r++) {
-        if (mybin[r]) perm[atomicAdd(&s_cur[mybin[r]], 1u)] = (u16)(t + 1 + r * K2_T);
-    }
-    const u32 nvalid = s_scan[0];
-    const u32 nwarp = s_hist[K2_NBIN - 1];
-    __syncthreads();
-
-    for (u32 i = wp; i < nwarp; i += K2_T / 32) {
-        const u32 q = perm[i];
-        const int s = (int)se[q - 1] - (int)w + 1;
-        const u32 len = (u32)se[q] - (u32)se[q - 1] + w;
-        const u32 nch = (len + 15) >> 4;
-        u64 pa = 0, pb = 0;
-        for (u32 c = lane; c < nch; c += 32) {
-            const int ad = s + K2_HALO + 16 * (int)c;
+            u64 pa = 0, pb = 0;
+            for (u32 c = lane; c < nch; c += 32) {
+                const int ad = st + K2_HALO + 16 * (int)c;
+                const u32 *p4 = reinterpret_cast<const u32 *>(sT + (ad & ~3));
+                const u32 sh = (u32)(ad & 3) * 8u;
+                const u32 W0 = p4[0], W1 = p4[1], W2 = p4[2], W3 = p4[3], W4 = p4[4];
+                u32 x0 = __funnelshift_r(W0, W1, sh), x1 = __funnelshift_r(W1, W2, sh);
+                u32 x2 = __funnelshift_r(W2, W3, sh), x3 = __funnelshift_r(W3, W4, sh);
+                if (c == nch - 1) mask_tail(x0, x1, x2, x3, (int)(len - 16 * c));
+                const uint4 k0 = *reinterpret_cast<const uint4 *>(sk + 4 * c);
+                const uint4 k1 = *reinterpret_cast<const uint4 *>(sk + 4 * c + 4);
+                nh_add(pa, pb, x0, x1, x2, x3, k0, k1);
+            }
+#pragma unroll
+            for (int o = 16; o > 0; o >>= 1) {
+                pa += __shfl_xor_sync(0xffffffffu, pa, o);
+                pb += __shfl_xor_sync(0xffffffffu, pb, o);
+            }
+            if (lane == 0) store_rec(a.rec, tile_first + q, pa, pb);
+        }
+
+        for (u32 i = nwarp + t; i < nvalid; i += T) {
+            const u32 q = perm[i];
+            const int st = (int)se[q - 1] - (int)w + 1;
+            const u32 len = (u32)se[q] - (u32)se[q - 1] + w;
+            const u32 nch = (len + 15) >> 4;
+            const int ad = st + K2_HALO;
             const u32 *p4 = reinterpret_cast<const u32 *>(sT + (ad & ~3));
             const u32 sh = (u32)(ad & 3) * 8u;
-            const u32 W0 = p4[0], W1 = p4[1], W2 = p4[2], W3 = p4[3], W4 = p4[4];
-            u32 x0 = __funnelshift_r(W0, W1, sh), x1 = __funnelshift_r(W1, W2, sh);
-            u32 x2 = __funnelshift_r(W2, W3, sh), x3 = __funnelshift_r(W3, W4, sh);
-            if (c == nch - 1) mask_tail(x0, x1, x2, x3, (int)(len - 16 * c));
-            const uint4 k0 = *reinterpret_cast<const uint4 *>(sk + 4 * c);
-            const uint4 k1 = *reinterpret_cast<const uint4 *>(sk + 4 * c + 4);
-            nh_add(pa, pb, x0, x1, x2, x3, k0, k1);
-        }
-#pragma unroll
-        for (int o = 16; o > 0; o >>= 1) {
-            pa += __shfl_xor_sync(0xffffffffu, pa, o);
-            pb += __shfl_xor_sync(0xffffffffu, pb, o);
-        }
-        if (lane == 0) {
-            if (FUSED) fused_insert(a, tile_first + q, q, pa, pb, &s_ncre, cq, cs);
-            else store_rec(a.rec, tile_first + q, pa, pb);
-        }
-    }
-
-    for (u32 i = nwarp + t; i < nvalid; i += K2_T) {
-        const u32 q = perm[i];
-        const int s = (int)se[q - 1] - (int)w + 1;
-        const u32 len = (u32)se[q] - (u32)se[q - 1] + w;
-        const u32 nch = (len + 15) >> 4;
-        const int ad = s + K2_HALO;
-        const u32 *p4 = reinterpret_cast<const u32 *>(sT + (ad & ~3));
-        const u32 sh = (u32)(ad & 3) * 8u;
-        const u32 *kp = sk;
-        uint4 k0 = *reinterpret_cast<const uint4 *>(kp);
-        u32 W0 = p4[0];
-        u64 pa = 0, pb = 0;
-        for (u32 c = 1; c < nch; c++) {
-            const u32 W1 = p4[1], W2 = p4[2], W3 = p4[3], W4 = p4[4];
-            const uint4 k1 = *reinterpret_cast<const uint4 *>(kp + 4);
-            nh_add(pa, pb, __funnelshift_r(W0, W1, sh), __funnelshift_r(W1, W2, sh),
-                   __funnelshift_r(W2, W3, sh), __funnelshift_r(W3, W4, sh), k0, k1);
-            W0 = W4;
-            k0 = k1;
-            p4 += 4;
-            kp += 4;
-        }
-        {
-            const u32 W1 = p4[1], W2 = p4[2], W3 = p4[3], W4 = p4[4];
-            const uint4 k1 = *reinterpret_cast<const uint4 *>(kp + 4);
-            u32 x0 = __funnelshift_r(W0, W1, sh), x1 = __funnelshift_r(W1, W2, sh);
-            u32 x2 = __funnelshift_r(W2, W3, sh), x3 = __funnelshift_r(W3, W4, sh);
-            mask_tail(x0, x1, x2, x3, (int)(len - 16 * (nch - 1)));
-            nh_add(pa, pb, x0, x1, x2, x3, k0, k1);
-        }
-        if (FUSED) fused_insert(a, tile_first + q, q, pa, pb, &s_ncre, cq, cs);
-        else store_rec(a.rec, tile_first + q, pa, pb);
-    }
-    if (!FUSED) return;
-
-    __syncthreads();
-    const u32 ncre = s_ncre;
-    if (ncre == 0) return;
-    u32 my_off[K2_CAP / K2_T], my_len[K2_CAP / K2_T];
-    u32 run_uw = 0;
-    {
-        u32 mx = 0, sl = 0;
-#pragma unroll
-        for (int r = 0; r < K2_CAP / K2_T; r++) {
-            my_off[r] = 0; my_len[r] = 0;
-            if ((u32)r * K2_T < ncre) {
-                const u32 k = t + r * K2_T;
-                u32 uw = 0;
-                if (k < ncre) {
-                    const u32 q = cq[k];
-                    const u32 len = (u32)se[q] - (u32)se[q - 1] + w;
-                    my_len[r] = len;
-                    uw = (len + 7) >> 3;
-                    mx = max(mx, len);
-                    sl += len;
-                }
-                u32 tot2;
-                const u32 ex2 = block_excl_scan_256(uw, &tot2, s_scan);
-                my_off[r] = run_uw + ex2;
-                run_uw += tot2;
-            }
-        }
-        if (mx) { atomicMax(&s_max, mx); atomicAdd(&s_sum, (unsigned long long)sl); }
-    }
-    __syncthreads();
-    if (t == 0) {
-        s_base_id = atomicAdd((unsigned long long *)&a.flags[1], (unsigned long long)ncre);
-        s_base_pool = atomicAdd((unsigned long long *)&a.flags[7], (unsigned long long)run_uw);
-        atomicMax((unsigned long long *)&a.flags[2], (unsigned long long)s_max);
-        atomicAdd((unsigned long long *)&a.flags[3], s_sum);
-    }
-    __syncthreads();
-    const u32 base_id = (u32)s_base_id;
-    const u64 base_pool = s_base_pool;
-#pragma unroll
-    for (int r = 0; r < K2_CAP / K2_T; r++) {
-        const u32 k = t + r * K2_T;
-        if (k < ncre) {
-            const u32 q = cq[k];
-            const u32 u = base_id + k;
-            const u64 j = tile_first + q;
-            a.rep[u] = (u32)j;
-            a.ulen[u] = my_len[r];
-            a.uwords[u] = (my_len[r] + 7) >> 3;
-            a.uoff[u] = base_pool + my_off[r];
-            a.tab[cs[k]].val = u + 1;
-            __stcs(a.uid + j, u);
-            atomicAdd(&a.count[u], 1u);
-            cs[k] = my_off[r];
-        }
-    }
-    __syncthreads();
-    if (base_pool + run_uw > a.pool_cap) {
-        if (t == 0) atomicOr((unsigned long long *)&a.flags[0], PFP_ERRBIT_POOL_FULL);
-        return;
-    }
-    for (u32 k = wp; k < ncre; k += K2_T / 32) {
-        const u32 q = cq[k];
-        const int s = (int)se[q - 1] - (int)w + 1 + K2_HALO;
-        const u32 len = (u32)se[q] - (u32)se[q - 1] + w;
-        const u32 nw = (len + 7) >> 3;
-        u64 *dst = a.pool + base_pool + cs[k];
-        for (u32 i = lane; i < nw; i += 32) {
-            const int ad = s + 8 * (int)i;
-            const u32 *p4 = reinterpret_cast<const u32 *>(sT + (ad & ~3));
-            const u32 sh = (u32)(ad & 3) * 8u;
-            const u32 W0 = p4[0], W1 = p4[1], W2 = p4[2];
-            u32 lo = __funnelshift_r(W0, W1, sh), hi = __funnelshift_r(W1, W2, sh);
-            const int rem = (int)len - 8 * (int)i;
-            if (rem < 8) {
-                lo &= ~__funnelshift_lc(0u, 0xFFFFFFFFu, (u32)(8 * rem));
-                hi &= ~__funnelshift_lc(0u, 0xFFFFFFFFu, (u32)max(8 * rem - 32, 0));
-            }
-            dst[i] = ((u64)hi << 32) | lo;
+            const u32 *kp = sk;
+            uint4 k0 = *reinterpret_cast<const uint4 *>(kp);
+            u32 W0 = p4[0];
+            u64 pa = 0, pb = 0;
+            for (u32 c = 1; c < nch; c++) {
+                const u32 W1 = p4[1], W2 = p4[2], W3 = p4[3], W4 = p4[4];
+                const uint4 k1 = *reinterpret_cast<const uint4 *>(kp + 4);
+                nh_add(pa, pb, __funnelshift_r(W0, W1, sh), __funnelshift_r(W1, W2, sh),
+                       __funnelshift_r(W2, W3, sh), __funnelshift_r(W3, W4, sh), k0, k1);
+                W0 = W4;
+                k0 = k1;
+                p4 += 4;
+                kp += 4;
+            }
+            {
+                const u32 W1 = p4[1], W2 = p4[2], W3 = p4[3], W4 = p4[4];
+                const uint4 k1 = *reinterpret_cast<const uint4 *>(kp + 4);
+                u32 x0 = __funnelshift_r(W0, W1, sh), x1 = __funnelshift_r(W1, W2, sh);
+                u32 x2 = __funnelshift_r(W2, W3, sh), x3 = __funnelshift_r(W3, W4, sh);
+                mask_tail(x0, x1, x2, x3, (int)(len - 16 * (nch - 1)));
+                nh_add(pa, pb, x0, x1, x2, x3, k0, k1);
+            }
+            store_rec(a.rec, tile_first + q, pa, pb);
         }
     }
 }
@@ -419,7 +348,8 @@
         a.keytab = ctx->d_keys; a.flags = ctx->d_flags;
         a.long_list = list; a.long_count = count;
         a.n_regular = sb.total;
-        phrase_stream_k<false><<<sb.ntiles, K2_T, K2_SMEM, ctx->stream>>>(a);
+        const u32 grid = sb.ntiles < ctx->k2_grid ? sb.ntiles : ctx->k2_grid;
+        phrase_stream_k<K2_T, K2_NST><<<grid, K2_T, K2_SMEM, ctx->stream>>>(a);
         PFP_LAUNCHED(ctx);
     }
     special_list_k<<<1, 1, 0, ctx->stream>>>(list, count, P, sb.total);
@@ -430,111 +360,12 @@
     return PFPB200_OK;
 }
 
-int pfp_words_fused_stage(pfpb200_ctx *ctx, const ScanBits &sb, const TextView &tv, const PhraseArrays &ph,
-                          u64 P, i64 first_start, u32 w, bool emit_ends, DictArrays *D) {
-    if (!pfp_stream_ok(sb, w)) return pfp_fail(ctx, PFPB200_E_INTERNAL, "stream stage: unsupported shape");
-    if (P >= 0x7FFFFFFEull) return pfp_fail(ctx, PFPB200_E_LIMIT, "more than 2^31-2 phrases in one shard");
-    u32 *list = nullptr;
-    const u64 lcap = 8ull * sb.ntiles + 8;
-    PFP_TRY(pfp_alloc_t(ctx, &list, lcap + 1));
-    u32 *lcount = list + lcap;
-    PhraseFp *rec_small = nullptr;
-    PFP_TRY(pfp_alloc_t(ctx, &rec_small, lcap));
-    PFP_TRY(pfp_alloc_t(ctx, &D->uid, P));
-    const u64 text_words = tv.n_buf / 8 + P * ((u64)w / 8 + 2) + 1024;
-    u64 need_pool = 0;
-    bool safe_table = false;
-    for (int attempt = 0;; attempt++) {
-        double want = (double)P * 1.5;
-        if (!safe_table && ctx->dedup_ratio > 0.0) {
-            const double guess = ctx->dedup_ratio * (double)P * ctx->table_scale;
-            if (guess < want) want = guess;
-        }
-        u64 cap = (u64)want + 1024;
-        if (cap >= 0x7FFFFFFFull) cap = 0x7FFFFFFEull;
-        const u64 wcap = cap < P ? cap : P;
-        u64 pool_cap = text_words;
-        if (need_pool) pool_cap = need_pool + 1024;
-        else if (ctx->pool_ratio > 0.0) pool_cap = (u64)(ctx->pool_ratio * 1.25 * (double)tv.n_buf / 8.0) + (1u << 16);
-        else pool_cap = tv.n_buf / 24 + (1u << 16);
-        if (pool_cap > text_words) pool_cap = text_words;
-        DictSlot *tab = nullptr;
-        PFP_TRY(pfp_alloc_t(ctx, &tab, cap));
-        PFP_TRY(pfp_alloc_t(ctx, &D->rep, wcap));
-        PFP_TRY(pfp_alloc_t(ctx, &D->count, wcap));
-        PFP_TRY(pfp_alloc_t(ctx, &D->ulen, wcap));
-        PFP_TRY(pfp_alloc_t(ctx, &D->uwords, wcap));
-        PFP_TRY(pfp_alloc_t(ctx, &D->uoff, wcap));
-        PFP_TRY(pfp_alloc_t(ctx, &D->pool, (size_t)pool_cap));
-        PFP_TRY(pfp_table_init(ctx, tab, cap));
-        PFP_CUDA(ctx, cudaMemsetAsync(D->count, 0, wcap * sizeof(u32), ctx->stream));
-        PFP_CUDA(ctx, cudaMemsetAsync(&ctx->d_flags[1], 0, 3 * sizeof(u64), ctx->stream));
-        PFP_CUDA(ctx, cudaMemsetAsync(&ctx->d_flags[6], 0, 2 * sizeof(u64), ctx->stream));
-        PFP_CUDA(ctx, cudaMemsetAsync(lcount, 0, sizeof(u32), ctx->stream));
-        if (sb.ntiles > 0 && sb.total > 0) {
-            StreamArgs a{};
-            a.A = sb.A; a.q_end = sb.q_end; a.pos_bias = sb.pos_bias;
-            a.mask = sb.mask; a.ntiles = sb.ntiles; a.tile_off = sb.tile_off;
-            a.w = w;
-            a.ends_out = emit_ends ? ph.ends : nullptr;
-            a.last = ph.last; a.sai = ph.sai; a.rec = ph.rec;
-            a.keytab = ctx->d_keys; a.flags = ctx->d_flags;
-            a.long_list = list; a.long_count = lcount;
-            a.n_regular = sb.total;
-            a.tab = tab; a.cap = cap;
-            a.uid = D->uid; a.rep = D->rep; a.ulen = D->ulen; a.uwords = D->uwords; a.count = D->count;
-            a.uoff = D->uoff; a.pool = D->pool; a.pool_cap = pool_cap; a.weak = ctx->weak_fp;
-            phrase_stream_k<true><<<sb.ntiles, K2_T, K2_SMEM_FUSED, ctx->stream>>>(a);
-            PFP_LAUNCHED(ctx);
-        }
-        special_list_k<<<1, 1, 0, ctx->stream>>>(list, lcount, P, sb.total);
-        PFP_LAUNCHED(ctx);
-        PFP_TRY(pfp_hash_list(ctx, tv, ph, first_start, w, list, lcount, lcap, rec_small));
-        D->pool_words = pool_cap;
-        PFP_TRY(pfp_insert_list(ctx, tv, rec_small, list, lcount, lcap, tab, cap, ph.ends, first_start, w, *D, pool_cap,
-                                ph.rec));
-        if (attempt == 0) PFP_TRY(pfp_records_range(ctx, tv, ph, sb.total, P, w));
-        PFP_CUDA(ctx, cudaMemcpyAsync(ctx->h_flags, ctx->d_flags, 8 * sizeof(u64), cudaMemcpyDeviceToHost, ctx->stream));
-        PFP_CUDA(ctx, cudaStreamSynchronize(ctx->stream));
-        const u64 fl = ctx->h_flags[0];
-        if (fl & PFP_ERRBIT_LIMIT) return pfp_fail(ctx, PFPB200_E_LIMIT, "a phrase is longer than 2^32-1 bytes");
-        if (fl & PFP_ERRBIT_INTERNAL) return pfp_fail(ctx, PFPB200_E_INTERNAL, "stream stage: a tile exceeded its trigger capacity");
-        const u64 d = ctx->h_flags[1];
-        const bool table_full = (fl & PFP_ERRBIT_TABLE_FULL) != 0 || (double)d > 0.85 * (double)cap;
-        const bool pool_full = (fl & PFP_ERRBIT_POOL_FULL) != 0 || ctx->h_flags[7] > pool_cap;
-        if (!table_full && !pool_full) {
-            if (fl & PFP_ERRBIT_COLLISION)
-                return pfp_fail(ctx, PFPB200_E_COLLISION, "fingerprint collision between different phrases");
-            if (ctx->h_flags[6]) PFP_TRY(pfp_table_pending(ctx, tab, P, D->uid, D->count));
-            PFP_TRY(pfp_free_now(ctx, tab));
-            ctx->dedup_ratio = (double)d / (double)P;
-            ctx->pool_ratio = tv.n_buf ? 8.0 * (double)ctx->h_flags[7] / (double)tv.n_buf : 0.0;
-            if (d > 0x7FFFFFFEull)
-                return pfp_fail(ctx, PFPB200_E_LIMIT, "%llu distinct words exceed the limit 2^31-2", (unsigned long long)d);
-            D->d = d;
-            D->pool_words = ctx->h_flags[7];
-            D->max_len = (u32)ctx->h_flags[2];
-            D->sum_len = ctx->h_flags[3];
-            break;
-        }
-        if (attempt >= 2) return pfp_fail(ctx, PFPB200_E_INTERNAL, "dictionary table / pool overflow after resizing");
-        if (table_full) { safe_table = true; need_pool = (ctx->h_flags[7] > pool_cap ? ctx->h_flags[7] : pool_cap) * 3 / 2; }
-        else need_pool = ctx->h_flags[7];
-        void *fr[] = {tab, D->rep, D->count, D->ulen, D->uwords, D->uoff, D->pool};
-        for (void *q : fr) PFP_TRY(pfp_free_now(ctx, q));
-        ctx->dedup_ratio = 0.0;
-        const u64 keep = fl & ~(PFP_ERRBIT_TABLE_FULL | PFP_ERRBIT_POOL_FULL | PFP_ERRBIT_COLLISION);
-        PFP_CUDA(ctx, cudaMemcpyAsync(&ctx->d_flags[0], &keep, sizeof(u64), cudaMemcpyHostToDevice, ctx->stream));
-        PFP_CUDA(ctx, cudaStreamSynchronize(ctx->stream));
-    }
-    PFP_TRY(pfp_free_now(ctx, list));
-    PFP_TRY(pfp_free_now(ctx, rec_small));
-    return PFPB200_OK;
-}
-
 int pfp_stream_init(pfpb200_ctx *ctx) {
-    PFP_CUDA(ctx, cudaFuncSetAttribute(phrase_stream_k<false>, cudaFuncAttributeMaxDynamicSharedMemorySize, K2_SMEM));
-    PFP_CUDA(ctx, cudaFuncSetAttribute(phrase_stream_k<true>, cudaFuncAttributeMaxDynamicSharedMemorySize, K2_SMEM_FUSED));
+    PFP_CUDA(ctx, cudaFuncSetAttribute(phrase_stream_k<K2_T, K2_NST>, cudaFuncAttributeMaxDynamicSharedMemorySize, K2_SMEM));
+    int per_sm = 0;
+    PFP_CUDA(ctx, cudaOccupancyMaxActiveBlocksPerMultiprocessor(&per_sm, phrase_stream_k<K2_T, K2_NST>, K2_T, K2_SMEM));
+    if (per_sm < 1) return pfp_fail(ctx, PFPB200_E_CUDA, "stream stage: the kernel does not fit on an SM");
+    ctx->k2_grid = (u32)per_sm * (u32)ctx->sm_count;
     return PFPB200_OK;
 }
 
diff --git a/big-bwt_b200/csrc/pfp_table.cuh b/big-bwt_b200/csrc/pfp_table.cuh
--- a/big-bwt_b200/csrc/pfp_table.cuh
+++ b/big-bwt_b200/csrc/pfp_table.cuh
@@ -5,7 +5,6 @@
 
 struct __align__(16) DictSlot { u64 key; u32 val; u32 chk; };
 constexpr u32 TABLE_MAX_PROBES = 2048;
-constexpr u32 UID_PENDING = 0x80000000u;
 
 __device__ __forceinline__ u32 check_of(const PhraseFp &r) {
     u64 x = (r.fpa + 0x632BE59BD9B4E019ULL) * 0xD1342543DE82EF95ULL;
diff --git a/big-bwt_b200/csrc/pfp_tma.cuh b/big-bwt_b200/csrc/pfp_tma.cuh
--- a/big-bwt_b200/csrc/pfp_tma.cuh
+++ b/big-bwt_b200/csrc/pfp_tma.cuh
@@ -9,12 +9,18 @@
 __device__ __forceinline__ void mbar_init_fence() {
     asm volatile("fence.mbarrier_init.release.cluster;" ::: "memory");
 }
+__device__ __forceinline__ void fence_proxy_async_smem() {
+    asm volatile("fence.proxy.async.shared::cta;" ::: "memory");
+}
 __device__ __forceinline__ void mbar_expect_tx(u64 *bar, u32 bytes) {
     asm volatile("mbarrier.arrive.expect_tx.shared::cta.b64 _, [%0], %1;" ::"r"(smem_addr_u32(bar)), "r"(bytes) : "memory");
 }
 __device__ __forceinline__ void bulk_copy_g2s(void *dst, const void *src, u32 bytes, u64 *bar) {
     asm volatile("cp.async.bulk.shared::cluster.global.mbarrier::complete_tx::bytes [%0], [%1], %2, [%3];"
                  ::"r"(smem_addr_u32(dst)), "l"(src), "r"(bytes), "r"(smem_addr_u32(bar)) : "memory");
+}
+__device__ __forceinline__ void bulk_prefetch_l2(const void *src, u32 bytes) {
+    asm volatile("cp.async.bulk.prefetch.L2.global [%0], %1;" ::"l"(src), "r"(bytes) : "memory");
 }
 __device__ __forceinline__ void mbar_wait(u64 *bar, u32 parity) {
     u32 ok;
```

Result: no change. 532.1 (median of 6 runs) (+0.3%).
